# FishYuLi/BalancedGroupSoftmax

Measured on AMD Instinct MI355X. Metric: img/s fwd+bwd R50-FPN+BAGS 1333x800, 512 RoI (BASELINE metric: img/s/GPU fwd+bwd R50-FPN+BAGS 1333x800, 512 RoI; GroupSoftmax us/RoI), higher is better.
Workload: dtype f32 (conv/linear products on the bf16 MFMA from exact 3-way bf16 splits, fp32 accumulate: fp32-faithful)

## Files before the change

balancedgroupsoftmax_amd/backbone.py:

```python
import contextlib

import torch
import torch.nn as nn

from . import functional as BF
from .ops import OFFSET_PITCH, DeformConv
from .registry import BACKBONES, NECKS


def _trainable(*modules):
    return torch.is_grad_enabled() and any(
        p.requires_grad for m in modules if m is not None for p in m.parameters())


def _fold_conv_bn(conv, bn, pad_cin_to=None):
    w = conv.weight
    cbias = getattr(conv, 'bias', None)
    if w.is_cuda:
        ctx = contextlib.nullcontext() if _trainable(conv, bn) else torch.no_grad()
        with ctx:
            if bn is not None:
                return BF.fold_conv_bn(w, cbias, bn.weight, bn.bias, bn.running_mean,
                                       bn.running_var, bn.eps, cin_padded=pad_cin_to)
            return BF.fold_conv_bn(w, cbias, cin_padded=pad_cin_to)
    ctx = contextlib.nullcontext() if _trainable(conv, bn) else torch.no_grad()
    with ctx:
        w = conv.weight.float()
        cout = w.shape[0]
        if bn is not None:
            scale = bn.weight.float() / torch.sqrt(bn.running_var.float() + bn.eps)
            shift = bn.bias.float() - bn.running_mean.float() * scale
            w = w * scale.view(-1, 1, 1, 1)
            b = shift if cbias is None else shift + cbias.float() * scale
        else:
            b = cbias.float() if cbias is not None else w.new_zeros(cout)
        w = w.permute(0, 2, 3, 1)
        if pad_cin_to is not None and w.shape[3] < pad_cin_to:
            w = torch.nn.functional.pad(w, (0, pad_cin_to - w.shape[3]))
        return w.contiguous(), b.contiguous()


def _tensor_slots(mods):
    slots, dicts, moddicts = [], [], []
    stack = list(mods)[::-1]
    while stack:
        m = stack.pop()
        for d in (m._parameters, m._buffers):
            dicts.append(d)
            for k in d:
                slots.append((d, k))
        dicts.append(m._modules)
        moddicts.append(m._modules)
        stack.extend(m._modules.values())
    return slots, dicts, moddicts


class _FoldCache(object):

    def __init__(self):
        self.key = None
        self.data = None
        self.mods = None
        self.slots = None
        self.count = -1
        self.fence = None

    def _list(self, mods):
        self.mods = tuple(id(m) for m in mods)
        self.slots, self.dicts, self.moddicts = _tensor_slots(mods)
        self.count = sum(len(d) for d in self.dicts)
        self.subs = self._sub_ids()
        self.key = None

    def _sub_ids(self):
        return [id(v) for d in self.moddicts for v in d.values()]

    def get(self, module, build):
        mods = module if isinstance(module, tuple) else (module,)
        if self.slots is None or self.mods != tuple(id(m) for m in mods) or \
                self.count != sum(len(d) for d in self.dicts) or self.subs != self._sub_ids():
            self._list(mods)
        try:
            tensors = [d[k] for d, k in self.slots]
        except KeyError:
            self._list(mods)
            tensors = [d[k] for d, k in self.slots]
        grad = torch.is_grad_enabled()
        key = []
        for t in tensors:
            if t is None:
                continue
            if grad and t.requires_grad:
                return build()
            key.append((id(t), t._version, t.data_ptr()))
        if key != self.key:
            self.data = build()
            self.key = key
            self.fence = BF.CacheFence() if any(t is not None and t.is_cuda for t in tensors) else None
        elif self.fence is not None:
            self.fence.wait()
            if self.fence.event is None:
                self.fence = None
        return self.data


def cached_fold(conv, bn=None, pad_cin_to=None):
    cache = conv.__dict__.get('_bgs_fold_cache')
    if cache is None:
        cache = conv.__dict__['_bgs_fold_cache'] = _FoldCache()
    mods = (conv, bn) if bn is not None else (conv,)
    return cache.get(mods, lambda: _fold_conv_bn(conv, bn, pad_cin_to=pad_cin_to))


class Bottleneck(nn.Module):
    expansion = 4

    def __init__(self, inplanes, planes, stride=1, downsample=False, groups=1, base_width=4, dcn=None):
        super().__init__()
        width = planes if groups == 1 else (planes * base_width // 64) * groups
        self.groups, self.width = groups, width
        self.conv1 = nn.Conv2d(inplanes, width, 1, stride=1, bias=False)
        self.bn1 = nn.BatchNorm2d(width)
        self.with_dcn = dcn is not None and not dcn.get('fallback_on_stride', False)
        if dcn is not None and dcn.get('modulated', False):
            raise NotImplementedError('modulated')
        if self.with_dcn:
            self.dcn_groups = dcn.get('groups', 1)
            self.conv2_offset = nn.Conv2d(width, dcn.get('deformable_groups', 1) * 18, 3, stride=stride,
                                          padding=1)
            self.conv2 = DeformConv(width, width, kernel_size=3, stride=stride, padding=1, dilation=1,
                                    groups=self.dcn_groups,
                                    deformable_groups=dcn.get('deformable_groups', 1), bias=False)
        else:
            self.conv2 = nn.Conv2d(width, width, 3, stride=stride, padding=1, groups=groups, bias=False)
        self.bn2 = nn.BatchNorm2d(width)
        self.conv3 = nn.Conv2d(width, planes * 4, 1, bias=False)
        self.bn3 = nn.BatchNorm2d(planes * 4)
        self.stride = stride
        self.downsample = None
        if downsample:
            self.downsample = nn.Sequential(
                nn.Conv2d(inplanes, planes * 4, 1, stride=stride, bias=False),
                nn.BatchNorm2d(planes * 4))
        self._cache = _FoldCache()

    def folded(self):
        return self._cache.get(self, self._build_fold)

    def _build_fold(self):
        f = dict(c1=_fold_conv_bn(self.conv1, self.bn1), c2=_fold_conv_bn(self.conv2, self.bn2),
                 c3=_fold_conv_bn(self.conv3, self.bn3))
        if self.downsample is not None:
            f['ds'] = _fold_conv_bn(self.downsample[0], self.downsample[1])
        if self.with_dcn:
            ow, ob = _fold_conv_bn(self.conv2_offset, None)
            padc = OFFSET_PITCH - ow.shape[0]
            f['off'] = (torch.nn.functional.pad(ow, (0, 0, 0, 0, 0, 0, 0, padc)).contiguous(),
                        torch.nn.functional.pad(ob, (0, padc)).contiguous())
        return f

    def run_bf16_storage(self, x, f):
        if self.with_dcn:
            raise NotImplementedError('Bottleneck.run_bf16_storage: a dcn block has no bf16-storage kernel '
                                      '(the deformable conv is fp32 only)')
        identity, fk = x, None
        if 'ds' in f:
            if x.is_cuda and BF.shortcut_fork_enabled():
                with BF.forked(x.device) as fk:
                    identity = BF.conv2d_nhwc(x, f['ds'][0], f['ds'][1], stride=self.stride)
            else:
                identity = BF.conv2d_nhwc(x, f['ds'][0], f['ds'][1], stride=self.stride)
        out = BF.conv2d_nhwc(x, f['c1'][0], f['c1'][1], relu=True)
        if self.groups > 1:
            out = BF.grouped_conv3x3_nhwc(out, f['c2'][0], f['c2'][1], self.groups, stride=self.stride,
                                          relu=True)
        else:
            out = BF.conv2d_nhwc(out, f['c2'][0], f['c2'][1], stride=self.stride, pad=1, relu=True)
        if fk is not None:
            fk.join()
        return BF.conv2d_nhwc(out, f['c3'][0], f['c3'][1], relu=True, residual=identity)

    def run(self, x, f, next_c1=None, h=None):
        if h is not None and (x.dtype == torch.bfloat16 or self.groups > 1 or self.with_dcn or
                              (torch.is_grad_enabled() and x.requires_grad)):
            raise RuntimeError('Bottleneck.run: a precomputed conv1 output is for the frozen fp32 block only')
        if x.dtype == torch.bfloat16:
            return self.run_bf16_storage(x, f)
        tagged = bool(getattr(x, '_bgs_consumers_mask', False))
        fuse = BF.fork_fusion_enabled() and torch.is_grad_enabled() and x.requires_grad
        if tagged and not fuse:
            raise RuntimeError("Bottleneck.run: x is a relu='consumers' block output but fork fusion is off")
        out_relu = 'consumers' if BF.fork_fusion_enabled() else True
        xin = x
        identity = x
        fk = None
        sc_tail = ('ds' in f and not fuse and self.groups == 1 and not self.with_dcn and x.is_cuda and
                   not (torch.is_grad_enabled() and any(t.requires_grad for k in ('c1', 'c2', 'c3', 'ds') for t in f[k]
                                                        if t is not None)) and
                   BF.fused_c3_shortcut_eligible(x, tuple(x.shape[:3]) + (f['c1'][0].shape[0],), f['c2'][0], f['c3'][0],
                                                 self.stride, f['ds'][0], f['ds'][1], self.stride))
        if sc_tail:
            identity = None
        elif 'ds' in f and not fuse and x.is_cuda and BF.shortcut_fork_enabled() and \
                not (torch.is_grad_enabled() and any(t.requires_grad for t in f['ds'] if t is not None)):
            with BF.forked(x.device) as fk:
                identity = BF.conv2d_nhwc(x, f['ds'][0], f['ds'][1], stride=self.stride)
        elif 'ds' in f:
            if fuse:
                identity, xin = BF.conv2d_autograd(x, f['ds'][0], f['ds'][1], stride=self.stride,
                                                   mask_input=tagged, passthrough=True)
            else:
                identity = BF.conv2d_autograd(x, f['ds'][0], f['ds'][1], stride=self.stride)
        first_pt = fuse and 'ds' not in f
        first_mask = tagged and 'ds' not in f
        if self.groups > 1 or self.with_dcn:
            out = BF.conv2d_autograd(xin, f['c1'][0], f['c1'][1], relu=True, mask_input=first_mask,
                                     passthrough=first_pt)
            if first_pt:
                out, identity = out
            if self.with_dcn:
                off = BF.conv2d_autograd(out, f['off'][0], f['off'][1], stride=self.stride, pad=1)
                out = BF.deform_conv3x3_nhwc(out, off, f['c2'][0], f['c2'][1], self.dcn_groups,
                                             stride=self.stride, relu=True)
            else:
                out = BF.grouped_conv3x3_nhwc(out, f['c2'][0], f['c2'][1], self.groups,
                                              stride=self.stride, relu=True)
            if fk is not None:
                fk.join()
            return BF.conv2d_autograd(out, f['c3'][0], f['c3'][1], relu=out_relu, residual=identity)
        if h is not None:
            out = h
        else:
            out = BF.conv2d_autograd(xin, f['c1'][0], f['c1'][1], relu='consumers', mask_input=first_mask,
                                     passthrough=first_pt)
            if first_pt:
                out, identity = out
        if sc_tail:
            if BF.fused_c3_eligible(out, f['c2'][0], f['c3'][0], self.stride, None):
                nc = next_c1 if next_c1 is not None and next_c1[0].shape[0] == 64 and BF.fused_c3_next_eligible(
                    out, f['c2'][0], f['c3'][0], self.stride, None, next_c1[0], next_c1[1]) else (None, None)
                return BF.conv3x3_c3_sc_fused_nhwc(out, f['c2'][0], f['c2'][1], f['c3'][0], f['c3'][1], x, f['ds'][0],
                                                   f['ds'][1], nc[0], nc[1], relu3=True)
            identity = BF.conv2d_nhwc(x, f['ds'][0], f['ds'][1], stride=self.stride)
        if not fuse and BF.fused_c3_eligible(out, f['c2'][0], f['c3'][0], self.stride, identity):
            if fk is not None:
                fk.join()
            if next_c1 is not None and BF.fused_c3_next_eligible(out, f['c2'][0], f['c3'][0], self.stride, identity,
                                                                 next_c1[0], next_c1[1]):
                return BF.conv3x3_c3_next_fused_nhwc(out, f['c2'][0], f['c2'][1], f['c3'][0], f['c3'][1], next_c1[0],
                                                     next_c1[1], residual=identity, relu3=True)
            return BF.conv3x3_c3_fused_nhwc(out, f['c2'][0], f['c2'][1], f['c3'][0], f['c3'][1], residual=identity,
                                            relu3=True)
        out = BF.conv2d_autograd(out, f['c2'][0], f['c2'][1], stride=self.stride, pad=1,
                                 relu='consumers', mask_input=True)
        if fk is not None:
            fk.join()
        return BF.conv2d_autograd(out, f['c3'][0], f['c3'][1], relu=out_relu, residual=identity,
                                  mask_input=True)


@BACKBONES.register_module
class ResNet(nn.Module):
    arch_settings = {50: (3, 4, 6, 3), 101: (3, 4, 23, 3), 152: (3, 8, 36, 3)}

    def __init__(self, depth, num_stages=4, strides=(1, 2, 2, 2), dilations=(1, 1, 1, 1),
                 out_indices=(0, 1, 2, 3), style='pytorch', frozen_stages=-1, conv_cfg=None,
                 norm_cfg=dict(type='BN', requires_grad=True), norm_eval=True, dcn=None,
                 stage_with_dcn=(False, False, False, False), gcb=None,
                 stage_with_gcb=(False, False, False, False), gen_attention=None,
                 stage_with_gen_attention=((), (), (), ()), with_cp=False,
                 zero_init_residual=True, groups=1, base_width=4):
        super().__init__()
        if depth not in self.arch_settings:
            raise KeyError('invalid depth {} for resnet (bottleneck depths only)'.format(depth))
        if dcn:
            raise NotImplementedError('dcn (deformable convolution, gs_htc_dconv_* config) has no '
                                      'kernel in this build')
        if style != 'pytorch' or tuple(dilations) != (1, 1, 1, 1) or gcb or gen_attention:
            raise NotImplementedError('only the plain pytorch-style trunk of the BAGS configs')
        if norm_cfg.get('type', 'BN') != 'BN' or not norm_eval:
            raise NotImplementedError('BatchNorm in eval mode only (norm_eval=True is what every '
                                      'BAGS config uses); it is folded into the convs')
        self.depth, self.num_stages = depth, num_stages
        self.out_indices, self.frozen_stages, self.norm_eval = out_indices, frozen_stages, norm_eval
        self.conv1 = nn.Conv2d(3, 64, 7, stride=2, padding=3, bias=False)
        self.bn1 = nn.BatchNorm2d(64)
        blocks = self.arch_settings[depth][:num_stages]
        inplanes = 64
        self.res_layers = []
        for i, nb in enumerate(blocks):
            planes = 64 * 2 ** i
            layers = []
            for j in range(nb):
                stride = strides[i] if j == 0 else 1
                layers.append(Bottleneck(inplanes, planes, stride,
                                         downsample=(j == 0 and (stride != 1 or
                                                                 inplanes != planes * 4)),
                                         groups=groups, base_width=base_width))
                inplanes = planes * 4
            name = 'layer{}'.format(i + 1)
            self.add_module(name, nn.Sequential(*layers))
            self.res_layers.append(name)
        self.feat_dim = inplanes
        self._cache = _FoldCache()
        self._stem_split = _FoldCache()
        self._freeze_stages()

    def _freeze_stages(self):
        if self.frozen_stages >= 0:
            for m in (self.conv1, self.bn1):
                for p in m.parameters():
                    p.requires_grad = False
        for i in range(1, self.frozen_stages + 1):
            for p in getattr(self, 'layer{}'.format(i)).parameters():
                p.requires_grad = False

    def init_weights(self, pretrained=None):
        if isinstance(pretrained, str):
            if '://' in pretrained:
                import warnings
                warnings.warn('pretrained=%r is a model-zoo URL and there is no network here: the '
                              'backbone keeps its RANDOM initialisation (frozen stages included). '
                              'Pass a local checkpoint path, or load a state_dict explicitly '
                              '(checkpoint.load_checkpoint / load_from).' % (pretrained,),
                              RuntimeWarning, stacklevel=2)
            else:
                from .checkpoint import load_checkpoint
                load_checkpoint(self, pretrained, strict=False)
                return
        elif pretrained is not None:
            raise TypeError('pretrained must be a str or None')
        for m in self.modules():
            if isinstance(m, nn.Conv2d):
                nn.init.kaiming_normal_(m.weight, mode='fan_out', nonlinearity='relu')
            elif isinstance(m, nn.BatchNorm2d):
                nn.init.constant_(m.weight, 1)
                nn.init.constant_(m.bias, 0)
        for m in self.modules():
            if isinstance(m, Bottleneck):
                nn.init.constant_(m.bn3.weight, 0)
                if hasattr(m, 'conv2_offset'):
                    nn.init.constant_(m.conv2_offset.weight, 0)
                    nn.init.constant_(m.conv2_offset.bias, 0)

    def _build_stem(self):
        return _fold_conv_bn(self.conv1, self.bn1, pad_cin_to=4)

    @staticmethod
    def to_nhwc4(img):
        if img.is_cuda and not (torch.is_grad_enabled() and img.requires_grad):
            return BF.nchw_to_nhwc4(img)
        x = img.float().permute(0, 2, 3, 1)
        return torch.nn.functional.pad(x, (0, 4 - x.shape[3])).contiguous()

    def forward(self, img):
        return self.forward_partial(img, -1, len(self.res_layers) - 1)[1]

    def forward_partial(self, x, first, last, outs=()):
        outs = list(outs)
        if first < 0:
            x = self._forward_stem(x)
            first = 0
        chain = [(i, blk) for i in range(first, last + 1) for blk in getattr(self, self.res_layers[i])]
        h, f = None, None
        for k, (i, blk) in enumerate(chain):
            nxt = chain[k + 1][1] if k + 1 < len(chain) else None
            fn = None
            if nxt is not None and blk.width == 64 and blk.stride == 1 and blk.groups == 1 and not blk.with_dcn \
                    and nxt.groups == 1 and not nxt.with_dcn and not _trainable(nxt):
                fn = nxt.folded()
            r = blk.run(x, f if f is not None else blk.folded(), next_c1=None if fn is None else fn['c1'], h=h)
            x, h = r if isinstance(r, tuple) else (r, None)
            f = fn
            if k + 1 < len(chain) and chain[k + 1][0] == i:
                continue
            if i in self.out_indices:
                outs.append(BF.relu_gate(x))
        return x, tuple(outs)

    def _forward_stem(self, img):
        stem = self._cache.get((self.conv1, self.bn1), self._build_stem)
        frozen_stem = not (torch.is_grad_enabled() and (img.requires_grad or stem[0].requires_grad or
                                                        stem[1].requires_grad))
        if img.is_cuda and frozen_stem and img.shape[1] == 3 and tuple(stem[0].shape[:3]) == (64, 7, 7) \
                and BF.stem_fused_enabled():
            ws = self._stem_split.get((self.conv1, self.bn1),
                                      lambda: BF.stem_fused_split_weights(stem[0].detach()))
            x = BF.stem_fused(img, ws, stem[1].detach())
        else:
            x = self.to_nhwc4(img)
            x = BF.conv2d_autograd(x, stem[0], stem[1], stride=2, pad=3, relu=True)
            storage = (BF.bf16_storage_active() and not x.requires_grad and
                       not _trainable(*[getattr(self, n) for n in self.res_layers]))
            x = BF.maxpool3x3s2_nhwc(x, out_dtype=torch.bfloat16 if storage else torch.float32)
        return x

    def train(self, mode=True):
        super().train(mode)
        self._freeze_stages()
        if mode and self.norm_eval:
            for m in self.modules():
                if isinstance(m, nn.BatchNorm2d):
                    m.eval()
        return self


@BACKBONES.register_module
class ResNeXt(ResNet):

    def __init__(self, groups=1, base_width=4, **kwargs):
        super().__init__(groups=groups, base_width=base_width, **kwargs)
        self.groups, self.base_width = groups, base_width


class ConvModule(nn.Module):

    def __init__(self, cin, cout, k, padding=0):
        super().__init__()
        self.conv = nn.Conv2d(cin, cout, k, padding=padding)
        self.padding = padding


@NECKS.register_module
class FPN(nn.Module):

    def __init__(self, in_channels, out_channels, num_outs, start_level=0, end_level=-1,
                 add_extra_convs=False, extra_convs_on_inputs=True,
                 relu_before_extra_convs=False, no_norm_on_lateral=False, conv_cfg=None,
                 norm_cfg=None, activation=None):
        super().__init__()
        assert isinstance(in_channels, list)
        if add_extra_convs or norm_cfg is not None or activation is not None or start_level != 0 \
                or end_level != -1:
            raise NotImplementedError('FPN variant outside the BAGS configs')
        self.in_channels, self.out_channels, self.num_outs = in_channels, out_channels, num_outs
        self.num_ins = len(in_channels)
        self.lateral_convs = nn.ModuleList(ConvModule(c, out_channels, 1) for c in in_channels)
        self.fpn_convs = nn.ModuleList(ConvModule(out_channels, out_channels, 3, padding=1)
                                       for _ in in_channels)
        self._cache = _FoldCache()

    def init_weights(self):
        for m in self.modules():
            if isinstance(m, nn.Conv2d):
                nn.init.xavier_uniform_(m.weight)
                nn.init.constant_(m.bias, 0)

    def _build_fold(self):
        return dict(lat=[_fold_conv_bn(m.conv, None) for m in self.lateral_convs],
                    out=[_fold_conv_bn(m.conv, None) for m in self.fpn_convs])

    def forward(self, inputs):
        assert len(inputs) == self.num_ins
        f = self._cache.get(self, self._build_fold)
        n = self.num_ins
        if inputs[0].dtype != torch.float32 and torch.is_grad_enabled() and _trainable(self):
            inputs = [t.float() for t in inputs]
        lat = [None] * n
        gate = [bool(getattr(t, '_bgs_consumers_mask', False)) for t in inputs]
        lat[n - 1] = BF.conv2d_autograd(inputs[n - 1], *f['lat'][n - 1], out_dtype=torch.float32,
                                        mask_input=gate[n - 1])
        if n > 1 and lat[n - 1].is_cuda and BF.level_fork_enabled():
            outs, fk = [None] * n, None
            for i in range(n - 1, 0, -1):
                with BF.forked(lat[i].device) as fk:
                    outs[i] = BF.conv2d_autograd(lat[i], *f['out'][i], pad=1)
                    if i == n - 1:
                        extra = []
                        for _ in range(self.num_outs - n):
                            extra.append((extra[-1] if extra else outs[i])[:, ::2, ::2, :].contiguous())
                lat[i - 1] = BF.conv2d_autograd(inputs[i - 1], *f['lat'][i - 1], residual=lat[i],
                                                residual_mode=2, out_dtype=torch.float32, mask_input=gate[i - 1])
            outs[0] = BF.conv2d_autograd(lat[0], *f['out'][0], pad=1)
            fk.join()
            return tuple(outs + extra)
        for i in range(n - 2, -1, -1):
            lat[i] = BF.conv2d_autograd(inputs[i], *f['lat'][i], residual=lat[i + 1],
                                        residual_mode=2, out_dtype=torch.float32, mask_input=gate[i])
        outs = [BF.conv2d_autograd(lat[i], *f['out'][i], pad=1) for i in range(n)]
        for _ in range(self.num_outs - n):
            outs.append(outs[-1][:, ::2, ::2, :].contiguous())
        return tuple(outs)
```

balancedgroupsoftmax_amd/capi.py:

```python
import ctypes
import os

_PKG = os.path.dirname(os.path.abspath(__file__))

c_i64p = ctypes.c_void_p
c_f32p = ctypes.c_void_p
c_ptr = ctypes.c_void_p

BGS_OK = 0
BGS_MAX_BINS = 16


class BgsLibraryError(RuntimeError):
    pass


class BgsCallError(RuntimeError):
    def __init__(self, fn, code, text):
        super().__init__('%s failed with code %d: %s' % (fn, code, text))
        self.code = code


SIGNATURES = {
    'bgs_version': (ctypes.c_int, []),
    'bgs_error_string': (ctypes.c_char_p, [ctypes.c_int]),
    'bgs_selftest_wave_reduce': (ctypes.c_int, [c_f32p, c_f32p, c_ptr]),
    'bgs_selftest_mfma_peak': (ctypes.c_int, [ctypes.c_int, ctypes.c_int, c_f32p, c_ptr]),
    'bgs_selftest_mfma_peak_bf16': (ctypes.c_int, [ctypes.c_int, ctypes.c_int, ctypes.c_int, c_f32p, c_ptr]),
    'bgs_gs_prepare': (ctypes.c_int, [c_i64p, c_i64p, c_f32p, ctypes.c_int, c_f32p, ctypes.c_int,
                                      ctypes.c_int, ctypes.c_int, ctypes.c_double,
                                      ctypes.c_uint64, c_ptr, c_i64p, c_f32p, c_f32p, c_ptr]),
    'bgs_gs_loss_workspace_bytes': (ctypes.c_size_t, [ctypes.c_int, ctypes.c_int]),
    'bgs_gs_loss_fwd_bwd': (ctypes.c_int, [c_f32p, c_ptr, c_i64p, c_f32p, c_f32p,
                                           ctypes.c_int, ctypes.c_int, ctypes.c_int,
                                           c_f32p, c_f32p, c_ptr, c_ptr]),
    'bgs_gs_head_loss_fused': (ctypes.c_int, [c_f32p, c_i64p, c_i64p, c_f32p, c_ptr, ctypes.c_int,
                                              ctypes.c_int, ctypes.c_int, ctypes.c_int,
                                              ctypes.c_double, ctypes.c_uint64, c_ptr, c_f32p,
                                              c_f32p, c_f32p, c_ptr, c_f32p, c_ptr, c_ptr]),
    'bgs_gs_head_step': (ctypes.c_int, [c_f32p, c_i64p, c_i64p, c_ptr, c_f32p, c_ptr, c_ptr, ctypes.c_int,
                                        ctypes.c_int, ctypes.c_int, ctypes.c_int, ctypes.c_double,
                                        ctypes.c_uint64, c_ptr, c_f32p, c_f32p, c_f32p, ctypes.c_int,
                                        ctypes.c_float, ctypes.c_float, c_f32p, c_f32p, c_f32p, c_f32p,
                                        c_f32p, c_ptr, c_f32p, c_ptr, c_ptr]),
    'bgs_gs_head_debug_timestamps': (None, [c_ptr]),
    'bgs_gs_head_tuning': (None, [ctypes.c_int]),
    'bgs_gs_head_variant': (None, [ctypes.c_int]),
    'bgs_gs_head_variant_used': (ctypes.c_int, [ctypes.c_int]),
    'bgs_sgd_clip_workspace_bytes': (ctypes.c_size_t, [c_ptr, ctypes.c_int]),
    'bgs_sgd_clip_step': (ctypes.c_int, [c_ptr, c_ptr, c_ptr, c_ptr, ctypes.c_int] + [ctypes.c_float] * 5
                          + [c_ptr, ctypes.c_size_t, c_ptr, c_ptr]),
    'bgs_gs_class_bin_mask': (ctypes.c_int, [c_i64p, ctypes.c_int, ctypes.c_int, c_ptr, c_ptr]),
    'bgs_gs_head_step_scale_grad': (ctypes.c_int, [c_f32p, c_f32p, c_ptr, c_f32p, c_f32p, ctypes.c_int,
                                                   ctypes.c_int, ctypes.c_int, ctypes.c_int, c_ptr]),
    'bgs_gs_loss_reduce': (ctypes.c_int, [c_ptr, ctypes.c_int, ctypes.c_int, c_f32p, c_ptr]),
    'bgs_gs_scale_grad': (ctypes.c_int, [c_f32p, c_i64p, c_f32p, ctypes.c_int, ctypes.c_int,
                                         ctypes.c_int, c_ptr]),
    'bgs_gs_merge_score': (ctypes.c_int, [c_f32p, c_i64p, c_ptr, ctypes.c_int, ctypes.c_int,
                                          ctypes.c_int, ctypes.c_int, c_f32p, c_ptr]),
    'bgs_bbox_loss_workspace_bytes': (ctypes.c_size_t, [ctypes.c_int]),
    'bgs_bbox_smooth_l1_fwd_bwd': (ctypes.c_int, [c_f32p, c_i64p, c_f32p, c_f32p, ctypes.c_int,
                                                  ctypes.c_int, ctypes.c_float, ctypes.c_float,
                                                  ctypes.c_float, c_f32p, c_f32p, c_ptr, c_ptr]),
    'bgs_fc_reg_gather': (ctypes.c_int, [c_f32p, c_f32p, c_f32p, c_i64p, ctypes.c_int, ctypes.c_int,
                                         ctypes.c_int, c_f32p, c_ptr]),
    'bgs_conv2d_nhwc_f32': (ctypes.c_int, [c_f32p, c_f32p, c_f32p, c_f32p, c_f32p] + [ctypes.c_int] * 11
                            + [c_ptr]),
    'bgs_conv2d_workspace_bytes': (ctypes.c_size_t, [ctypes.c_longlong, ctypes.c_int]),
    'bgs_conv2d_nhwc_f32_ws': (ctypes.c_int, [c_f32p, c_f32p, c_f32p, c_f32p, c_f32p]
                               + [ctypes.c_int] * 11 + [c_ptr, ctypes.c_size_t, c_ptr]),
    'bgs_conv2d_dgrad_nhwc_f32_ws': (ctypes.c_int, [c_f32p, c_f32p, c_f32p, c_f32p, c_f32p]
                                     + [ctypes.c_int] * 10 + [c_ptr, ctypes.c_size_t, c_ptr]),
    'bgs_conv2d_dgrad_nhwc_f32': (ctypes.c_int, [c_f32p, c_f32p, c_f32p, c_f32p, c_f32p]
                                  + [ctypes.c_int] * 10 + [c_ptr]),
    'bgs_conv2d_wgrad_workspace_bytes': (ctypes.c_size_t, [ctypes.c_int] * 9),
    'bgs_conv2d_wgrad_nhwc_f32': (ctypes.c_int, [c_f32p, c_f32p, c_f32p, c_f32p]
                                  + [ctypes.c_int] * 10 + [c_ptr, c_ptr]),
    'bgs_fold_conv_bn_fwd': (ctypes.c_int, [c_f32p] * 6 + [ctypes.c_float] + [ctypes.c_int] * 5
                             + [c_f32p, c_f32p, c_ptr]),
    'bgs_fold_conv_bn_bwd': (ctypes.c_int, [c_f32p] * 7 + [ctypes.c_float] + [ctypes.c_int] * 5
                             + [c_f32p] * 4 + [c_ptr]),
    'bgs_conv2d_wgrad_bfx_workspace_bytes': (ctypes.c_size_t, [ctypes.c_int] * 9),
    'bgs_conv2d_wgrad_nhwc_f32_bfx': (ctypes.c_int, [c_f32p, c_f32p, c_f32p, c_f32p]
                                      + [ctypes.c_int] * 11 + [c_ptr, c_ptr]),
    'bgs_conv2d_wgrad_bfx_enable': (None, [ctypes.c_int]),
    'bgs_conv3x3_halo_nhwc_f32': (ctypes.c_int, [c_f32p, c_f32p, c_f32p, c_f32p] + [ctypes.c_int] * 6
                                  + [c_ptr]),
    'bgs_conv_bfx_weight_bytes': (ctypes.c_size_t, [ctypes.c_int, ctypes.c_int]),
    'bgs_conv_bfx_split_weights': (ctypes.c_int, [c_f32p, c_ptr, ctypes.c_int, ctypes.c_int, c_ptr]),
    'bgs_conv_dgrad_parity_enable': (None, [ctypes.c_int]),
    'bgs_conv_bfx_split_weights_dgrad': (ctypes.c_int, [c_f32p, c_ptr] + [ctypes.c_int] * 4 + [c_ptr]),
    'bgs_conv_bfx_workspace_bytes': (ctypes.c_size_t, [ctypes.c_longlong, ctypes.c_int, ctypes.c_int]),
    'bgs_conv2d_nhwc_f32_bfx_ws': (ctypes.c_int, [c_f32p, c_ptr, c_f32p, c_f32p, c_f32p]
                                   + [ctypes.c_int] * 12 + [c_ptr, ctypes.c_size_t, c_ptr]),
    'bgs_conv2d_dgrad_nhwc_f32_bfx_ws': (ctypes.c_int, [c_f32p, c_ptr, c_f32p, c_f32p, c_f32p]
                                         + [ctypes.c_int] * 11 + [c_ptr, ctypes.c_size_t, c_ptr]),
    'bgs_conv3x3_halo_bfx_workspace_bytes': (ctypes.c_size_t, [ctypes.c_int] * 5),
    'bgs_conv3x3_c3_fused_nhwc_f32_bfx': (ctypes.c_int, [c_f32p, c_ptr, c_f32p, c_ptr, c_f32p, c_f32p, c_f32p]
                                          + [ctypes.c_int] * 6 + [c_ptr]),
    'bgs_conv3x3_c3_fused_eligible': (ctypes.c_int, [ctypes.c_int] * 5),
    'bgs_conv3x3_c3_next_fused_nhwc_f32_bfx': (ctypes.c_int,
                                               [c_f32p, c_ptr, c_f32p, c_ptr, c_f32p, c_f32p, c_f32p, c_ptr, c_f32p,
                                                c_f32p] + [ctypes.c_int] * 7 + [c_ptr]),
    'bgs_conv3x3_c3_next_eligible': (ctypes.c_int, [ctypes.c_int] * 6),
    'bgs_conv3x3_c3_sc_fused_nhwc_f32_bfx': (ctypes.c_int,
                                             [c_f32p, c_ptr, c_f32p, c_ptr, c_f32p, c_f32p, c_ptr, c_f32p, c_f32p, c_ptr,
                                              c_f32p, c_f32p] + [ctypes.c_int] * 8 + [c_ptr]),
    'bgs_conv3x3_c3_sc_eligible': (ctypes.c_int, [ctypes.c_int] * 7),
    'bgs_conv3x3_halo_nhwc_f32_bfx': (ctypes.c_int, [c_f32p, c_ptr, c_f32p, c_f32p]
                                      + [ctypes.c_int] * 7 + [c_ptr, ctypes.c_size_t, c_ptr]),
    'bgs_conv3x3_halo_nhwc_f32_bfx_ex': (ctypes.c_int, [c_f32p, c_ptr, c_f32p, c_f32p, c_f32p]
                                         + [ctypes.c_int] * 7 + [c_ptr, ctypes.c_size_t, c_ptr]),
    'bgs_conv3x3_planes_head_nhwc_f32_bfx': (ctypes.c_int, [c_f32p, c_ptr, c_f32p, c_ptr, c_f32p, c_f32p]
                                             + [ctypes.c_int] * 7 + [c_ptr]),
    'bgs_conv3x3_planes_head_eligible': (ctypes.c_int, [ctypes.c_int] * 6),
    'bgs_gs_loss_tuning': (None, [ctypes.c_int]),
    'bgs_gs_loss_wavepriv_min_rows': (None, [ctypes.c_int]),
    'bgs_gs_merge_tuning': (None, [ctypes.c_int, ctypes.c_int]),
    'bgs_conv_bfx_wide_tuning': (None, [ctypes.c_int] * 3),
    'bgs_conv_bfx_wide_last_launch': (ctypes.c_int, []),
    'bgs_conv1x1_planes_enable': (None, [ctypes.c_int]),
    'bgs_conv1x1_planes_last_launch': (ctypes.c_int, []),
    'bgs_conv3x3_planes_enable': (None, [ctypes.c_int]),
    'bgs_conv3x3_planes_last_launch': (ctypes.c_int, []),
    'bgs_conv1x1_bres_enable': (None, [ctypes.c_int]),
    'bgs_conv1x1_bres_last_launch': (ctypes.c_int, []),
    'bgs_launch_census': (ctypes.c_int, [ctypes.c_int, ctypes.c_int]),
    'bgs_conv_bfx_tuning': (None, [ctypes.c_int] * 2),
    'bgs_conv_bfx_last_launch': (ctypes.c_int, [c_ptr, c_ptr]),
    'bgs_conv_tuning': (None, [ctypes.c_int] * 4),
    'bgs_conv_last_launch': (ctypes.c_int, [c_ptr, c_ptr, c_ptr, c_ptr]),
    'bgs_conv3x3_halo_bfx_tuning': (None, [ctypes.c_int] * 2),
    'bgs_conv3x3_halo_bfx_last_launch': (ctypes.c_int, [c_ptr, c_ptr]),
    'bgs_conv3x3_halo_bfx_last_wide': (ctypes.c_int, [c_ptr, c_ptr]),
    'bgs_conv3x3_halo_bfx_wide': (ctypes.c_int, [ctypes.c_int]),
    'bgs_grouped_conv3x3_nhwc_f32': (ctypes.c_int, [c_f32p, c_f32p, c_f32p, c_f32p] + [ctypes.c_int] * 7
                                     + [c_ptr]),
    'bgs_grouped_conv3x3_nhwc_bf16ops': (ctypes.c_int, [c_f32p, c_f32p, c_f32p, c_f32p] + [ctypes.c_int] * 7
                                         + [c_ptr]),
    'bgs_grouped_conv3x3_dgrad_nhwc_f32': (ctypes.c_int, [c_f32p, c_f32p, c_f32p] + [ctypes.c_int] * 6
                                           + [c_ptr]),
    'bgs_grouped_conv3x3_wgrad_workspace_bytes': (ctypes.c_size_t, [ctypes.c_int] * 6),
    'bgs_grouped_conv3x3_wgrad_nhwc_f32': (ctypes.c_int, [c_f32p, c_f32p, c_f32p, c_f32p]
                                           + [ctypes.c_int] * 7 + [c_ptr, c_ptr]),
    'bgs_deform_conv3x3_nhwc_f32': (ctypes.c_int, [c_f32p] * 5 + [ctypes.c_int] * 9 + [c_ptr]),
    'bgs_deform_conv3x3_dgrad_nhwc_f32': (ctypes.c_int, [c_f32p] * 6 + [ctypes.c_int] * 8 + [c_ptr]),
    'bgs_deform_conv3x3_wgrad_workspace_bytes': (ctypes.c_size_t, [ctypes.c_int] * 6),
    'bgs_deform_conv3x3_wgrad_nhwc_f32': (ctypes.c_int, [c_f32p] * 5 + [ctypes.c_int] * 9 + [c_ptr, c_ptr]),
    'bgs_sigmoid_focal_workspace_bytes': (ctypes.c_size_t, []),
    'bgs_sigmoid_focal_fwd': (ctypes.c_int, [c_f32p, ctypes.c_longlong, c_i64p, ctypes.c_int, ctypes.c_int,
                                             ctypes.c_float, ctypes.c_float, ctypes.c_int, c_f32p, c_ptr]),
    'bgs_sigmoid_focal_bwd': (ctypes.c_int, [c_f32p, ctypes.c_longlong, c_i64p, c_f32p, ctypes.c_int, ctypes.c_int,
                                             ctypes.c_float, ctypes.c_float, ctypes.c_int, c_f32p, c_ptr]),
    'bgs_sigmoid_focal_fwd_bwd': (ctypes.c_int, [c_f32p, ctypes.c_longlong, c_i64p, c_f32p, c_f32p, ctypes.c_int,
                                                 ctypes.c_int, ctypes.c_float, ctypes.c_float, ctypes.c_int, c_f32p,
                                                 ctypes.c_float, c_f32p, c_f32p, c_ptr, c_ptr]),
    'bgs_maxpool3x3s2_bwd_nhwc_f32': (ctypes.c_int, [c_f32p, c_f32p, c_f32p] + [ctypes.c_int] * 4 + [c_ptr]),
    'bgs_maxpool3x3s2_nhwc_f32': (ctypes.c_int, [c_f32p, c_f32p] + [ctypes.c_int] * 4 + [c_ptr]),
    'bgs_nchw_to_nhwc4_f32': (ctypes.c_int, [c_f32p, c_f32p] + [ctypes.c_int] * 4 + [c_ptr]),
    'bgs_conv2d_nhwc_bf16s': (ctypes.c_int, [c_ptr, c_ptr, c_f32p, c_ptr, ctypes.c_int, ctypes.c_int, c_ptr]
                              + [ctypes.c_int] * 11 + [c_ptr]),
    'bgs_grouped_conv3x3_nhwc_bf16s': (ctypes.c_int, [c_ptr, c_f32p, c_f32p, c_ptr] + [ctypes.c_int] * 7
                                       + [c_ptr]),
    'bgs_maxpool3x3s2_nhwc_f32_to_bf16': (ctypes.c_int, [c_f32p, c_ptr] + [ctypes.c_int] * 4 + [c_ptr]),
    'bgs_conv_bf16s_tuning': (None, [ctypes.c_int]),
    'bgs_roi_align_nhwc_fwd': (ctypes.c_int, [c_ptr, c_ptr, c_ptr, c_ptr, ctypes.c_int,
                                              ctypes.c_int, ctypes.c_float, c_f32p, ctypes.c_int,
                                              ctypes.c_int, ctypes.c_int, ctypes.c_int,
                                              ctypes.c_int, c_f32p, c_ptr, c_ptr]),
    'bgs_roi_align_nhwc_bwd': (ctypes.c_int, [c_ptr, c_ptr, c_ptr, c_ptr, ctypes.c_int,
                                              ctypes.c_int, ctypes.c_float, c_f32p, ctypes.c_int,
                                              ctypes.c_int, ctypes.c_int, ctypes.c_int,
                                              ctypes.c_int, c_f32p, c_ptr]),
    'bgs_roi_align_nhwc_fwd_f16': (ctypes.c_int, [c_ptr, c_ptr, c_ptr, c_ptr, ctypes.c_int,
                                                  ctypes.c_int, ctypes.c_float, c_f32p, ctypes.c_int,
                                                  ctypes.c_int, ctypes.c_int, ctypes.c_int,
                                                  ctypes.c_int, c_ptr, c_ptr, c_ptr]),
    'bgs_roi_align_nhwc_bwd_f16': (ctypes.c_int, [c_ptr, c_ptr, c_ptr, c_ptr, ctypes.c_int,
                                                  ctypes.c_int, ctypes.c_float, c_f32p, ctypes.c_int,
                                                  ctypes.c_int, ctypes.c_int, ctypes.c_int,
                                                  ctypes.c_int, c_ptr, c_ptr]),
    'bgs_roi_align_nhwc_fwd_ex': (ctypes.c_int, [c_ptr, c_ptr, c_ptr, c_ptr, ctypes.c_int,
                                                 ctypes.c_int, ctypes.c_float, c_f32p, ctypes.c_int,
                                                 ctypes.c_int, ctypes.c_int, ctypes.c_int,
                                                 ctypes.c_int, ctypes.c_int, ctypes.c_int, c_f32p,
                                                 c_ptr, c_ptr]),
    'bgs_roi_align_nhwc_bwd_ex': (ctypes.c_int, [c_ptr, c_ptr, c_ptr, c_ptr, ctypes.c_int,
                                                 ctypes.c_int, ctypes.c_float, c_f32p, ctypes.c_int,
                                                 ctypes.c_int, ctypes.c_int, ctypes.c_int,
                                                 ctypes.c_int, ctypes.c_int, c_f32p, c_ptr]),
    'bgs_resize_bilinear_nhwc_f32': (ctypes.c_int, [c_f32p, c_f32p] + [ctypes.c_int] * 7 + [c_ptr]),
    'bgs_resize_bilinear_nhwc_bwd_f32': (ctypes.c_int, [c_f32p, c_f32p] + [ctypes.c_int] * 7
                                         + [c_ptr]),
    'bgs_mask_target': (ctypes.c_int, [c_ptr, c_ptr, ctypes.c_int, ctypes.c_int, ctypes.c_int, c_f32p,
                                       ctypes.c_int, c_ptr, c_ptr, ctypes.c_int, ctypes.c_int, c_f32p,
                                       c_ptr]),
    'bgs_stem_fused_weight_bytes': (ctypes.c_size_t, []),
    'bgs_stem_fused_split_weights': (ctypes.c_int, [c_f32p, ctypes.c_int, c_ptr, c_ptr]),
    'bgs_stem_conv7x7s2_relu_maxpool_nchw_f32': (ctypes.c_int, [c_f32p, c_ptr, c_f32p, c_f32p, ctypes.c_int,
                                                                ctypes.c_int, ctypes.c_int, c_ptr]),
    'bgs_mask_paste_u8': (ctypes.c_int, [c_f32p, c_f32p, ctypes.c_int, ctypes.c_int, ctypes.c_int, ctypes.c_float,
                                         ctypes.c_float, ctypes.c_int, ctypes.c_int, c_ptr, c_ptr]),
    'bgs_mask_rle_workspace_bytes': (ctypes.c_size_t, [ctypes.c_int, ctypes.c_int]),
    'bgs_mask_rle_count': (ctypes.c_int, [c_f32p, c_f32p, ctypes.c_int, ctypes.c_int, ctypes.c_int, c_ptr, c_f32p,
                                          ctypes.c_float, ctypes.c_int, ctypes.c_int, c_ptr, ctypes.c_size_t, c_ptr,
                                          c_ptr]),
    'bgs_mask_rle_write': (ctypes.c_int, [c_f32p, c_f32p, ctypes.c_int, ctypes.c_int, ctypes.c_int, c_ptr, c_f32p,
                                          ctypes.c_float, ctypes.c_int, ctypes.c_int, c_ptr, ctypes.c_size_t, c_ptr,
                                          ctypes.c_longlong, c_ptr, c_ptr, c_ptr]),
    'bgs_rle_to_string': (ctypes.c_int, [c_ptr, c_ptr, ctypes.c_int, c_ptr, ctypes.c_longlong, c_ptr]),
    'bgs_rle_from_string': (ctypes.c_int, [c_ptr, c_ptr, ctypes.c_int, c_ptr, ctypes.c_longlong, c_ptr]),
    'bgs_lvis_box_iou': (ctypes.c_int, [c_ptr] * 5 + [ctypes.c_int] + [ctypes.c_longlong] * 3 + [c_ptr, c_ptr]),
    'bgs_lvis_rle_iou': (ctypes.c_int, [c_ptr] * 7 + [ctypes.c_int] + [ctypes.c_longlong] * 3 + [c_ptr, c_ptr]),
    'bgs_lvis_match_workspace_bytes': (ctypes.c_size_t, [ctypes.c_longlong, ctypes.c_int, ctypes.c_int]),
    'bgs_lvis_match': (ctypes.c_int, [c_ptr] * 4 + [ctypes.c_int] + [ctypes.c_longlong] * 2 + [c_ptr] * 4
                       + [c_ptr, ctypes.c_int, c_ptr, ctypes.c_int, c_ptr, ctypes.c_size_t] + [c_ptr] * 4 + [c_ptr]),
    'bgs_lvis_accumulate': (ctypes.c_int, [c_ptr] * 5 + [ctypes.c_int] + [ctypes.c_longlong] * 2
                            + [ctypes.c_int, ctypes.c_int, c_ptr, ctypes.c_int, c_ptr, c_ptr, c_ptr]),
    'bgs_recall_match_lds_bytes': (ctypes.c_size_t, [ctypes.c_int, ctypes.c_int]),
    'bgs_recall_match': (ctypes.c_int, [c_ptr] * 5 + [c_ptr, ctypes.c_int, c_ptr, ctypes.c_int]
                         + [ctypes.c_int, ctypes.c_int, ctypes.c_longlong, ctypes.c_longlong, ctypes.c_int,
                            ctypes.c_int, c_ptr, c_ptr, c_ptr]),
    'bgs_poly_rle_edge_points': (ctypes.c_int, [c_ptr, c_ptr, c_ptr, ctypes.c_longlong, ctypes.c_int, c_ptr, c_ptr]),
    'bgs_poly_rle_crossings': (ctypes.c_int, [c_ptr] * 4 + [ctypes.c_longlong, ctypes.c_int, ctypes.c_int, c_ptr, c_ptr,
                                              ctypes.c_longlong, c_ptr, c_ptr, c_ptr]),
    'bgs_poly_rle_events_from_transitions': (ctypes.c_int, [c_ptr] * 4 + [ctypes.c_int, ctypes.c_longlong, c_ptr,
                                                            c_ptr]),
    'bgs_poly_rle_events_from_runs': (ctypes.c_int, [c_ptr] * 3 + [ctypes.c_int, ctypes.c_longlong, c_ptr, c_ptr]),
    'bgs_poly_rle_resolve': (ctypes.c_int, [c_ptr] * 3 + [ctypes.c_int, ctypes.c_int] + [c_ptr] * 4
                             + [ctypes.c_int, ctypes.c_longlong] + [c_ptr] * 4),
    'bgs_poly_rle_write': (ctypes.c_int, [c_ptr] * 4 + [ctypes.c_int] + [c_ptr] * 4
                           + [ctypes.c_longlong, c_ptr, ctypes.c_longlong, c_ptr, c_ptr]),
    'bgs_mask_gt_logits': (ctypes.c_int, [c_f32p, c_f32p, c_f32p, c_ptr, ctypes.c_int, ctypes.c_int,
                                          ctypes.c_int, ctypes.c_int, c_f32p, c_ptr]),
    'bgs_mask_bce_partials': (ctypes.c_int, [ctypes.c_int]),
    'bgs_mask_bce': (ctypes.c_int, [c_f32p, c_f32p, c_f32p, c_ptr, c_f32p, c_ptr, c_f32p,
                                    ctypes.c_int, ctypes.c_int, ctypes.c_int, ctypes.c_int, c_f32p,
                                    c_f32p, c_f32p, c_f32p, c_ptr]),
    'bgs_topk_workspace_bytes': (ctypes.c_size_t, [ctypes.c_int, ctypes.c_int]),
    'bgs_topk_sorted_f32': (ctypes.c_int, [c_ptr, c_ptr, c_ptr, c_ptr, c_ptr, ctypes.c_int,
                                           ctypes.c_int, c_f32p, c_ptr, c_ptr, c_ptr]),
    'bgs_nms_workspace_bytes': (ctypes.c_size_t, [ctypes.c_int, ctypes.c_int]),
    'bgs_nms_batched': (ctypes.c_int, [c_f32p, c_ptr, ctypes.c_int, ctypes.c_int, ctypes.c_float,
                                       ctypes.c_int, ctypes.c_int, c_ptr, c_ptr, c_ptr, c_ptr]),
    'bgs_nms_merge_select': (ctypes.c_int, [c_f32p, c_ptr, c_ptr] + [ctypes.c_int] * 4 + [c_f32p, c_ptr, c_ptr]),
    'bgs_nms_gather': (ctypes.c_int, [c_f32p, c_ptr, c_ptr, ctypes.c_int, ctypes.c_int, c_f32p, c_f32p, c_ptr]),
    'bgs_soft_nms_batched': (ctypes.c_int, [c_f32p, c_ptr, ctypes.c_int, ctypes.c_int, ctypes.c_float, ctypes.c_int,
                                            ctypes.c_float, ctypes.c_float, c_ptr, c_f32p, c_ptr, c_ptr]),
    'bgs_det_candidates': (ctypes.c_int, [c_f32p, c_f32p, c_ptr, c_f32p] + [ctypes.c_int] * 4
                           + [ctypes.c_float, ctypes.c_int, c_f32p, c_ptr, c_ptr, c_ptr]),
    'bgs_det_select': (ctypes.c_int, [c_f32p, c_ptr, c_ptr, c_f32p, c_ptr] + [ctypes.c_int] * 4
                       + [c_f32p, c_ptr, c_ptr, c_ptr, c_ptr]),
    'bgs_gather_boxes': (ctypes.c_int, [c_f32p, c_ptr, c_f32p, ctypes.c_int, ctypes.c_int, ctypes.c_int, c_f32p,
                                        c_ptr, c_ptr]),
    'bgs_aug_map_boxes': (ctypes.c_int, [c_ptr, c_ptr] + [ctypes.c_int] * 4 + [c_ptr, c_ptr, c_ptr, ctypes.c_int,
                                                                               ctypes.c_int, c_f32p, c_f32p, c_ptr,
                                                                               c_ptr]),
    'bgs_aug_merge_bboxes': (ctypes.c_int, [c_ptr, c_ptr] + [ctypes.c_int] * 4 + [c_ptr, c_ptr, c_ptr, c_ptr, c_f32p,
                                                                                  c_f32p, c_ptr]),
    'bgs_aug_merge_masks': (ctypes.c_int, [c_ptr, c_ptr, ctypes.c_int, ctypes.c_int, ctypes.c_int, c_f32p, c_ptr]),
    'bgs_img_prep_u8': (ctypes.c_int, [c_ptr, c_ptr, ctypes.c_int, ctypes.c_int, c_f32p, ctypes.c_int, c_f32p,
                                       ctypes.c_int, ctypes.c_int, c_ptr]),
    'bgs_gt_mask_prep_u8': (ctypes.c_int, [c_ptr, c_ptr, ctypes.c_int, c_ptr, c_ptr, ctypes.c_longlong, c_ptr,
                                           ctypes.c_int, ctypes.c_int, c_ptr]),
    'bgs_gt_seg_prep_u8': (ctypes.c_int, [c_ptr, c_ptr, ctypes.c_int, c_ptr, ctypes.c_int, ctypes.c_int, c_ptr]),
    'bgs_iou_assign_workspace_bytes': (ctypes.c_size_t, [ctypes.c_int] * 3),
    'bgs_iou_assign': (ctypes.c_int, [c_f32p, ctypes.c_longlong, ctypes.c_int, c_ptr, c_f32p, c_ptr,
                                      ctypes.c_int, ctypes.c_int, ctypes.c_float, ctypes.c_float,
# ... 120 lines not shown
```

balancedgroupsoftmax_amd/csrc/bottleneck_tail_planes.hip:

```cpp
#include <stdlib.h>

#include <initializer_list>

#include "conv_args.h"
#include "bfx_split.h"

using namespace bgs_conv;

namespace {

struct TailArgs {
  const float* x;
  const __bf16* ws2;
  const float* bias2;
  const __bf16* ws3;
  const float* bias3;
  const float* res;
  float* y;
  int N, H, W, relu3;
  int tiles_y, tiles_x, tiles, chunk;
};

struct TailNextArgs {
  TailArgs t;
  const __bf16* ws1n;
  const float* bias1n;
  float* h;
};
template <class A> struct TailScArgs {
  A a;
  const float* x0;
  const __bf16* wssc;
  const float* bias_sc;
};
template <int NEXT, bool SC = false> struct TailArgsOf { typedef TailNextArgs type; };
template <> struct TailArgsOf<0, false> { typedef TailArgs type; };
template <int NEXT> struct TailArgsOf<NEXT, true> { typedef TailScArgs<typename TailArgsOf<NEXT>::type> type; };
__device__ __forceinline__ const TailArgs& tail_base(const TailArgs& a) { return a; }
__device__ __forceinline__ const TailArgs& tail_base(const TailNextArgs& a) { return a.t; }
template <class A> __device__ __forceinline__ const TailArgs& tail_base(const TailScArgs<A>& a) { return tail_base(a.a); }
template <class A> __device__ __forceinline__ const A& tail_inner(const A& a) { return a; }
template <class A> __device__ __forceinline__ const A& tail_inner(const TailScArgs<A>& a) { return a.a; }

constexpr int kOob = 0x7f000000;

__device__ __forceinline__ void load_x0_half(const float* x0, const TailArgs& g, int n, int ty, int tx, int tid, int a,
                                             f32x4& q0, f32x4& q1) {
  const __amdgpu_buffer_rsrc_t x0_rsrc = __builtin_amdgcn_make_buffer_rsrc(
      const_cast<float*>(x0), 0, (int)((size_t)g.N * g.H * g.W * 64 * 4), 0x00020000);
  f32x4 q[2];
#pragma unroll
  for (int j = 0; j < 2; ++j) {
    const int m = a * 32 + (tid >> 4) + 16 * j;
    const int ho = ty * 8 + (m >> 3), wo = tx * 8 + (m & 7);
    const int off = ho < g.H && wo < g.W ? (((n * g.H + ho) * g.W + wo) * 64 + (tid & 15) * 4) * 4 : kOob;
    q[j] = __builtin_bit_cast(f32x4, __builtin_amdgcn_raw_buffer_load_b128(x0_rsrc, off, 0, 0));
  }
  q0 = q[0];
  q1 = q[1];
}

__device__ __forceinline__ void load_sc_filter(const __bf16* wssc, int lane_off, int t, bf16x8 (&dst)[3]) {
  const __amdgpu_buffer_rsrc_t bs_rsrc = __builtin_amdgcn_make_buffer_rsrc(const_cast<__bf16*>(wssc), 0, 3 * 4 * 256 * 32, 0x00020000);
#pragma unroll
  for (int s = 0; s < 3; ++s)
    dst[s] = __builtin_bit_cast(bf16x8, __builtin_amdgcn_raw_buffer_load_b128(bs_rsrc, lane_off, ((s * 4 + (t & 3)) * 256 + 32 * (t >> 2)) * 32, 0));
}

template <int NEXT, bool SC = false>
__global__ __launch_bounds__(kThreads, 3) void bottleneck_tail_planes_kernel(typename TailArgsOf<NEXT, SC>::type ga) {
  static_assert(NEXT == 0 || NEXT == 64 || NEXT == 128, "width of the next block's conv1");
  static_assert(!SC || NEXT != 128, "a block with a stride-1 projection shortcut (layer1.0) is never in front of a 128-wide conv1");
  const TailArgs& g = tail_base(ga);
  const auto& gn = tail_inner(ga);
  constexpr int NS = 3, CM = 64, CO3 = 256, KC2 = 36, KC3 = 4;
  constexpr int PW = 10, PS = 12, PSLOTS = PW * PS;
  constexpr int AQ = PW * PW * 16, AQT = (AQ + kThreads - 1) / kThreads;
  constexpr int KS = PSLOTS * 32, PL = 4 * KS;
  constexpr int KCN = CO3 / 16, KCH = KCN / 2, KSN = 64 * 32 + 32, PLN = KCH * KSN;
  constexpr int LD4 = CO3 + 8;
  constexpr int SC_OFF = 32 * LD4 * 4, KSC = 32 * 32 + 32, PLSC = KC3 * KSC;
  constexpr int LDS_BASE = NEXT ? NS * PLN : NS * PL;
  constexpr int LDS_BYTES = SC && SC_OFF + NS * PLSC > LDS_BASE ? SC_OFF + NS * PLSC : LDS_BASE;
  static_assert(64 * (NEXT + 8) * 4 <= LDS_BYTES, "the h transpose tile overlays the planes");
  static_assert(NS * PL <= LDS_BYTES && 3 * LDS_BYTES <= 160 * 1024, "three workgroups per CU");
  constexpr int LD2 = CM + 4, S2_BYTES = 64 * LD2 * 4;
  constexpr int Y_OFF = 18 * 1024;
  constexpr int P3_CH = 64 * 32, P3_PL = KC3 * P3_CH;
  static_assert(S2_BYTES <= Y_OFF && Y_OFF + NS * P3_PL <= LDS_BYTES && 32 * LD4 * 4 <= LDS_BYTES, "overlays");
  __shared__ __attribute__((aligned(1024))) unsigned char lds[LDS_BYTES];

  const int tid = threadIdx.x, lane = tid & 63;
  const int wave = bgs::uniform(tid >> 6);
  const int wm = wave >> 1, wn = wave & 1;
  const int frow = lane & 31, fk = lane >> 5;
  const int vtile = (int)((blockIdx.x & 7) * g.chunk + (blockIdx.x >> 3));
  if (vtile >= g.tiles) return;
  const int per_img = g.tiles_y * g.tiles_x;
  const int n = vtile / per_img, trem = vtile - n * per_img;
  const int ty = trem / g.tiles_x, tx = trem - ty * g.tiles_x;
  const int h0 = ty * 8 - 1, w0 = tx * 8 - 1;

  const __amdgpu_buffer_rsrc_t x_rsrc = __builtin_amdgcn_make_buffer_rsrc(
      const_cast<float*>(g.x), 0, (int)((size_t)g.N * g.H * g.W * CM * 4), 0x00020000);
  f32x4 ra[AQT];
  int a_dst[AQT];
#pragma unroll
  for (int i = 0; i < AQT; ++i) {
    const int q = tid + kThreads * i;
    const bool use = q < AQ;
    const int pix = use ? q >> 4 : 0, kq = q & 15;
    const int ppy = pix / PW, ppx = pix - ppy * PW;
    const int hi = h0 + ppy, wi = w0 + ppx;
    const bool in = use && hi >= 0 && hi < g.H && wi >= 0 && wi < g.W;
    const int off = in ? (((n * g.H + hi) * g.W + wi) * CM + kq * 4) * 4 : kOob;
    ra[i] = __builtin_bit_cast(f32x4, __builtin_amdgcn_raw_buffer_load_b128(x_rsrc, off, 0, 0));
    const int quad = kq & 3;
    a_dst[i] = use ? (kq >> 2) * KS + (ppy * PS + ppx) * 32 + (((quad >> 1) ^ (ppy & 1)) << 4) + (quad & 1) * 8 : -1;
  }

  f32x4 rx[SC ? 4 : 1];
  if constexpr (SC) load_x0_half(ga.x0, g, n, ty, tx, tid, 0, rx[0], rx[1]);

  const __amdgpu_buffer_rsrc_t b2_rsrc = __builtin_amdgcn_make_buffer_rsrc(
      const_cast<__bf16*>(g.ws2), 0, NS * KC2 * CM * 32, 0x00020000);
  const int b2_lane = ((wn * 32 + frow) * 16 + fk * 8) * 2;
  auto load_b2 = [&](int kc, bf16x8 (&dst)[NS]) {
#pragma unroll
    for (int s = 0; s < NS; ++s)
      dst[s] = __builtin_bit_cast(bf16x8, __builtin_amdgcn_raw_buffer_load_b128(b2_rsrc, b2_lane, (s * KC2 + kc) * CM * 32, 0));
  };
  bf16x8 fbA[NS], fbB[NS];
  load_b2(0, fbA);

#pragma unroll
  for (int i = 0; i < AQT; ++i) {
    if (a_dst[i] < 0) continue;
    u32x2 hh, mm, ll;
    split3(ra[i], hh, mm, ll);
    unsigned char* d = lds + a_dst[i];
    *reinterpret_cast<u32x2*>(d) = hh;
    *reinterpret_cast<u32x2*>(d + PL) = mm;
    *reinterpret_cast<u32x2*>(d + 2 * PL) = ll;
  }
  __syncthreads();

  int a_frag[2];
  {
    const int m = wm * 32 + frow;
    const int py = m >> 3, px = m & 7;
#pragma unroll
    for (int par = 0; par < 2; ++par) a_frag[par] = (py * PS + px) * 32 + ((fk ^ ((py + par) & 1)) << 4);
  }
  f32x16 acc2;
#pragma unroll
  for (int r = 0; r < 16; ++r) acc2[r] = 0.f;
#pragma unroll
  for (int t = 0; t < KC2; ++t) {
    const int c16 = t / 9, tap = t % 9, dy = tap / 3, dx = tap % 3;
    const int t1 = t + 1;
    const int kc_next = t1 < KC2 ? (t1 % 9) * 4 + t1 / 9 : 0;
    if (t & 1) load_b2(kc_next, fbA);
    else load_b2(kc_next, fbB);
    __builtin_amdgcn_sched_barrier(0);
    const bf16x8 (&fb)[NS] = (t & 1) ? fbB : fbA;
    bf16x8 fa[NS];
#pragma unroll
    for (int s = 0; s < NS; ++s)
      fa[s] = *reinterpret_cast<const bf16x8*>(lds + s * PL + c16 * KS + a_frag[dy & 1] + (dy * PS + dx) * 32);
#pragma unroll
    for (int tt = NS - 1; tt >= 0; --tt)
#pragma unroll
      for (int i = 0; i <= tt; ++i) acc2 = __builtin_amdgcn_mfma_f32_32x32x16_bf16(fa[i], fb[tt - i], acc2, 0, 0, 0);
    __builtin_amdgcn_sched_barrier(0);
  }

  const __amdgpu_buffer_rsrc_t b3_rsrc = __builtin_amdgcn_make_buffer_rsrc(
      const_cast<__bf16*>(g.ws3), 0, NS * KC3 * CO3 * 32, 0x00020000);
  const int b3_lane = ((wave * 64 + frow) * 16 + fk * 8) * 2;
  auto load_b3 = [&](int kc, bf16x8 (&dst)[NS][2]) {
#pragma unroll
    for (int s = 0; s < NS; ++s)
#pragma unroll
      for (int b = 0; b < 2; ++b)
        dst[s][b] = __builtin_bit_cast(bf16x8, __builtin_amdgcn_raw_buffer_load_b128(b3_rsrc, b3_lane, ((s * KC3 + kc) * CO3 + 32 * b) * 32, 0));
  };
  bf16x8 f3a[NS][2], f3b[NS][2];
  load_b3(0, f3a);
  bf16x8 fsa[NS], fsb[NS];

  __syncthreads();
  float* scratch = reinterpret_cast<float*>(lds);
#pragma unroll
  for (int r = 0; r < 16; ++r) {
    const int i = wm * 32 + (r & 3) + 8 * (r >> 2) + 4 * (lane >> 5);
    scratch[i * LD2 + wn * 32 + (lane & 31)] = acc2[r];
  }
  __syncthreads();
  {
    const int c4 = (tid & 15) * 4, r0 = tid >> 4;
    f32x4 bias2 = {0.f, 0.f, 0.f, 0.f};
    if (g.bias2) bias2 = *reinterpret_cast<const f32x4*>(g.bias2 + c4);
    const int kc2 = c4 >> 4, kq2 = (c4 & 15) >> 2;
#pragma unroll
    for (int ps = 0; ps < 4; ++ps) {
      const int i = r0 + ps * 16;
      f32x4 v = *reinterpret_cast<const f32x4*>(scratch + i * LD2 + c4);
      v += bias2;
#pragma unroll
      for (int t = 0; t < 4; ++t) v[t] = fmaxf(v[t], 0.f);
      u32x2 hh, mm, ll;
      split3(v, hh, mm, ll);
      unsigned char* d = lds + Y_OFF + kc2 * P3_CH + i * 32 + (((kq2 >> 1) ^ ((i >> 3) & 1)) << 4) + (kq2 & 1) * 8;
      *reinterpret_cast<u32x2*>(d) = hh;
      *reinterpret_cast<u32x2*>(d + P3_PL) = mm;
      *reinterpret_cast<u32x2*>(d + 2 * P3_PL) = ll;
    }
  }
  __syncthreads();

  int a3_frag[2];
#pragma unroll
  for (int a = 0; a < 2; ++a) {
    const int m = a * 32 + frow;
// ... 22 lines not shown
    const bf16x8 (&fb3)[NS][2] = (kc & 1) ? f3b : f3a;
    bf16x8 fa3[NS][2];
#pragma unroll
    for (int s = 0; s < NS; ++s)
#pragma unroll
      for (int a = 0; a < 2; ++a) fa3[s][a] = *reinterpret_cast<const bf16x8*>(lds + a3_frag[a] + kc * P3_CH + s * P3_PL);
#pragma unroll
    for (int tt = NS - 1; tt >= 0; --tt)
#pragma unroll
      for (int i = 0; i <= tt; ++i)
#pragma unroll
        for (int a = 0; a < 2; ++a)
#pragma unroll
          for (int b = 0; b < 2; ++b)
            acc3[a][b] = __builtin_amdgcn_mfma_f32_32x32x16_bf16(fa3[i][a], fb3[tt - i][b], acc3[a][b], 0, 0, 0);
    __builtin_amdgcn_sched_barrier(0);
  }
  __syncthreads();

  const int e4 = (tid & 63) * 4, er0 = tid >> 6;
  f32x4 bias3 = {0.f, 0.f, 0.f, 0.f};
  if (g.bias3) bias3 = *reinterpret_cast<const f32x4*>(g.bias3 + e4);
  const int out_bytes = (int)((size_t)g.N * g.H * g.W * CO3 * 4);
  const __amdgpu_buffer_rsrc_t res_rsrc = __builtin_amdgcn_make_buffer_rsrc(
      const_cast<float*>(g.res ? g.res : g.x), 0, g.res ? out_bytes : 0, 0x00020000);
  const __amdgpu_buffer_rsrc_t y_rsrc = __builtin_amdgcn_make_buffer_rsrc(g.y, 0, out_bytes, 0x00020000);
  f32x4 vn[NEXT ? 2 : 1][NEXT ? 8 : 1];
  if constexpr (SC) {
    const int kcw = (tid & 15) >> 2, kqw = tid & 3;
    auto write_planes = [&](int a) {
#pragma unroll
      for (int j = 0; j < 2; ++j) {
        const int i = (tid >> 4) + 16 * j;
        u32x2 hh, mm, ll;
        split3(rx[2 * a + j], hh, mm, ll);
        unsigned char* d = lds + SC_OFF + kcw * KSC + i * 32 + (((kqw >> 1) ^ ((i >> 3) & 1)) << 4) + (kqw & 1) * 8;
        *reinterpret_cast<u32x2*>(d) = hh;
        *reinterpret_cast<u32x2*>(d + PLSC) = mm;
        *reinterpret_cast<u32x2*>(d + 2 * PLSC) = ll;
      }
    };
    const int as_frag = SC_OFF + frow * 32 + ((fk ^ ((frow >> 3) & 1)) << 4);
    float b3v[2] = {0.f, 0.f}, bsv[2] = {0.f, 0.f};
#pragma unroll
    for (int b = 0; b < 2; ++b) {
      if (g.bias3) b3v[b] = g.bias3[wave * 64 + b * 32 + (lane & 31)];
      if (ga.bias_sc) bsv[b] = ga.bias_sc[wave * 64 + b * 32 + (lane & 31)];
    }
    write_planes(0);
#pragma unroll
    for (int a = 0; a < 2; ++a) {
      __syncthreads();
#pragma unroll
      for (int b = 0; b < 2; ++b) {
        f32x16 accs;
#pragma unroll
        for (int r = 0; r < 16; ++r) accs[r] = 0.f;
#pragma unroll
        for (int kc = 0; kc < KC3; ++kc) {
          const int t = b * KC3 + kc;
          if (t + 1 < 2 * KC3) {
            if (t & 1) load_sc_filter(ga.wssc, b3_lane, t + 1, fsa);
            else load_sc_filter(ga.wssc, b3_lane, t + 1, fsb);
          }
          __builtin_amdgcn_sched_barrier(0);
          const bf16x8 (&fbs)[NS] = (t & 1) ? fsb : fsa;
          bf16x8 fas[NS];
#pragma unroll
          for (int s = 0; s < NS; ++s) fas[s] = *reinterpret_cast<const bf16x8*>(lds + as_frag + kc * KSC + s * PLSC);
#pragma unroll
          for (int tt = NS - 1; tt >= 0; --tt)
#pragma unroll
            for (int i = 0; i <= tt; ++i) accs = __builtin_amdgcn_mfma_f32_32x32x16_bf16(fas[i], fbs[tt - i], accs, 0, 0, 0);
          __builtin_amdgcn_sched_barrier(0);
        }
#pragma unroll
        for (int r = 0; r < 16; ++r) {
          const int i = (r & 3) + 8 * (r >> 2) + 4 * (lane >> 5);
          const float rsc = accs[r] + bsv[b];
          scratch[i * LD4 + wave * 64 + b * 32 + (lane & 31)] = (acc3[a][b][r] + b3v[b]) + rsc;
        }
      }
      __syncthreads();
      if (a == 0) {
        load_sc_filter(ga.wssc, b3_lane, 0, fsa);
        write_planes(1);
      }
#pragma unroll
      for (int ps = 0; ps < 8; ++ps) {
        const int i = er0 + ps * 4;
        const int m = a * 32 + i;
        const int ho = ty * 8 + (m >> 3), wo = tx * 8 + (m & 7);
        f32x4 v = *reinterpret_cast<const f32x4*>(scratch + i * LD4 + e4);
        if (g.relu3) {
#pragma unroll
          for (int t = 0; t < 4; ++t) v[t] = fmaxf(v[t], 0.f);
        }
        if (ho < g.H && wo < g.W)
          __builtin_amdgcn_raw_buffer_store_b128(__builtin_bit_cast(u32x4, v), y_rsrc, (((n * g.H + ho) * g.W + wo) * CO3 + e4) * 4, 0, 0);
        if constexpr (NEXT > 0) vn[a][ps] = v;
      }
    }
    if constexpr (NEXT > 0) __syncthreads();
  } else {
#pragma unroll
  for (int a = 0; a < 2; ++a) {
    f32x4 rs[8];
#pragma unroll
    for (int ps = 0; ps < 8; ++ps) {
      const int m = a * 32 + er0 + ps * 4;
      const int ho = min(ty * 8 + (m >> 3), g.H - 1), wo = min(tx * 8 + (m & 7), g.W - 1);
      rs[ps] = __builtin_bit_cast(f32x4, __builtin_amdgcn_raw_buffer_load_b128(res_rsrc, (((n * g.H + ho) * g.W + wo) * CO3 + e4) * 4, 0, 0));
    }
#pragma unroll
    for (int b = 0; b < 2; ++b)
#pragma unroll
      for (int r = 0; r < 16; ++r) {
        const int i = (r & 3) + 8 * (r >> 2) + 4 * (lane >> 5);
        scratch[i * LD4 + wave * 64 + b * 32 + (lane & 31)] = acc3[a][b][r];
      }
    __syncthreads();
#pragma unroll
    for (int ps = 0; ps < 8; ++ps) {
      const int i = er0 + ps * 4;
      const int m = a * 32 + i;
      const int ho = ty * 8 + (m >> 3), wo = tx * 8 + (m & 7);
      f32x4 v = *reinterpret_cast<const f32x4*>(scratch + i * LD4 + e4);
      v += bias3;
      v += rs[ps];
      if (g.relu3) {
#pragma unroll
        for (int t = 0; t < 4; ++t) v[t] = fmaxf(v[t], 0.f);
      }
      if (ho < g.H && wo < g.W)
        __builtin_amdgcn_raw_buffer_store_b128(__builtin_bit_cast(u32x4, v), y_rsrc, (((n * g.H + ho) * g.W + wo) * CO3 + e4) * 4, 0, 0);
      if constexpr (NEXT > 0) vn[a][ps] = v;
    }
    __syncthreads();
  }
  }

  if constexpr (NEXT > 0) {
    constexpr int LDH = NEXT + 8, NA = NEXT == 128 ? 2 : 1;
    const int a0 = NEXT == 128 ? 0 : (wave >> 1);
    const int tn = NEXT == 128 ? wave : (wave & 1);
    const __amdgpu_buffer_rsrc_t bn_rsrc = __builtin_amdgcn_make_buffer_rsrc(
        const_cast<__bf16*>(gn.ws1n), 0, NS * KCN * NEXT * 32, 0x00020000);
    const int bn_lane = ((tn * 32 + frow) * 16 + fk * 8) * 2;
    auto load_bn = [&](int kc, bf16x8 (&dst)[NS]) {
#pragma unroll
      for (int s = 0; s < NS; ++s)
        dst[s] = __builtin_bit_cast(bf16x8, __builtin_amdgcn_raw_buffer_load_b128(bn_rsrc, bn_lane, (s * KCN + kc) * NEXT * 32, 0));
    };
    bf16x8 fn[3][NS];
    load_bn(0, fn[0]);
    load_bn(1, fn[1]);
    f32x4 vs[2][8];
#pragma unroll
    for (int ps = 0; ps < 8; ++ps) {
      const u32x4 lo = __builtin_bit_cast(u32x4, vn[0][ps]), hi = __builtin_bit_cast(u32x4, vn[1][ps]);
      u32x4 slo, shi;
#pragma unroll
      for (int t = 0; t < 4; ++t) {
        const unsigned a0 = lo[t], a1 = hi[t];
        const auto sw = __builtin_amdgcn_permlane32_swap(a0, a1, false, false);
        slo[t] = sw[0];
        shi[t] = sw[1];
      }
      vs[0][ps] = __builtin_bit_cast(f32x4, slo);
      vs[1][ps] = __builtin_bit_cast(f32x4, shi);
    }
    const int kcl = (lane & 31) >> 2, kqn = lane & 3;
    int an_frag[NA];
#pragma unroll
    for (int a = 0; a < NA; ++a) {
      const int m = (a0 + a) * 32 + frow;
      an_frag[a] = m * 32 + ((fk ^ ((m >> 3) & 1)) << 4);
    }
    f32x16 accn[NA];
#pragma unroll
    for (int a = 0; a < NA; ++a)
#pragma unroll
      for (int r = 0; r < 16; ++r) accn[a][r] = 0.f;
#pragma unroll
    for (int c = 0; c < 2; ++c) {
#pragma unroll
      for (int ps = 0; ps < 8; ++ps) {
        const int i = (lane >> 5) * 32 + er0 + ps * 4;
        u32x2 hh, mm, ll;
        split3(vs[c][ps], hh, mm, ll);
        unsigned char* d = lds + kcl * KSN + i * 32 + (((kqn >> 1) ^ ((i >> 3) & 1)) << 4) + (kqn & 1) * 8;
        *reinterpret_cast<u32x2*>(d) = hh;
        *reinterpret_cast<u32x2*>(d + PLN) = mm;
        *reinterpret_cast<u32x2*>(d + 2 * PLN) = ll;
      }
      __syncthreads();
#pragma unroll
      for (int k8 = 0; k8 < KCH; ++k8) {
        const int kc = c * KCH + k8;
        if (kc + 2 < KCN) load_bn(kc + 2, fn[(kc + 2) % 3]);
        __builtin_amdgcn_sched_barrier(0);
        const bf16x8 (&fbn)[NS] = fn[kc % 3];
        bf16x8 fan[NS][NA];
#pragma unroll
        for (int s = 0; s < NS; ++s)
#pragma unroll
          for (int a = 0; a < NA; ++a) fan[s][a] = *reinterpret_cast<const bf16x8*>(lds + s * PLN + k8 * KSN + an_frag[a]);
#pragma unroll
        for (int tt = NS - 1; tt >= 0; --tt)
#pragma unroll
          for (int i = 0; i <= tt; ++i)
#pragma unroll
            for (int a = 0; a < NA; ++a)
              accn[a] = __builtin_amdgcn_mfma_f32_32x32x16_bf16(fan[i][a], fbn[tt - i], accn[a], 0, 0, 0);
        __builtin_amdgcn_sched_barrier(0);
      }
      __syncthreads();
    }
#pragma unroll
    for (int a = 0; a < NA; ++a)
#pragma unroll
      for (int r = 0; r < 16; ++r) {
        const int i = (a0 + a) * 32 + (r & 3) + 8 * (r >> 2) + 4 * (lane >> 5);
        scratch[i * LDH + tn * 32 + (lane & 31)] = accn[a][r];
      }
    __syncthreads();
    constexpr int TPRN = NEXT / 4, RPPN = kThreads / TPRN, EPN = 64 / RPPN;
    const int n4 = (tid % TPRN) * 4, nr0 = tid / TPRN;
    f32x4 biasn = {0.f, 0.f, 0.f, 0.f};
    if (gn.bias1n) biasn = *reinterpret_cast<const f32x4*>(gn.bias1n + n4);
    const __amdgpu_buffer_rsrc_t h_rsrc =
        __builtin_amdgcn_make_buffer_rsrc(gn.h, 0, (int)((size_t)g.N * g.H * g.W * NEXT * 4), 0x00020000);
#pragma unroll
    for (int ps = 0; ps < EPN; ++ps) {
      const int m = nr0 + ps * RPPN;
      const int ho = ty * 8 + (m >> 3), wo = tx * 8 + (m & 7);
      f32x4 v = *reinterpret_cast<const f32x4*>(scratch + m * LDH + n4);
      v += biasn;
#pragma unroll
      for (int t = 0; t < 4; ++t) v[t] = fmaxf(v[t], 0.f);
      if (ho < g.H && wo < g.W)
        __builtin_amdgcn_raw_buffer_store_b128(__builtin_bit_cast(u32x4, v), h_rsrc, (((n * g.H + ho) * g.W + wo) * NEXT + n4) * 4, 0, 0);
    }
  }
}

}


static int tail_eligible(int N, int H, int W, int Cmid, int Cout3) {
  if (N <= 0 || H <= 0 || W <= 0 || Cmid != 64 || Cout3 != 256) return 0;
  const long long lim = kOob / (256 * 4);
  const long long nh = (long long)N * H;
  return nh < lim && nh * W < lim ? 1 : 0;
}

template <class... P> static bool aligned16(P... ptr) { return ((... | (uintptr_t)ptr) % 16) == 0; }

static TailArgs tail_args(const float* x, const void* w2split, const float* bias2, const void* w3split,
                          const float* bias3, const float* residual, float* y, int N, int H, int W, int relu3) {
  TailArgs g;
  g.x = x;
  g.ws2 = reinterpret_cast<const __bf16*>(w2split);
  g.bias2 = bias2;
  g.ws3 = reinterpret_cast<const __bf16*>(w3split);
  g.bias3 = bias3;
  g.res = residual;
  g.y = y;
  g.N = N; g.H = H; g.W = W; g.relu3 = relu3;
  g.tiles_y = (H + 7) / 8;
  g.tiles_x = (W + 7) / 8;
  g.tiles = N * g.tiles_y * g.tiles_x;
  g.chunk = (g.tiles + 7) / 8;
  return g;
}

static TailNextArgs tail_next_args(const TailArgs& g, const void* w1n_split, const float* bias1n, float* h) {
  TailNextArgs a;
  a.t = g;
  a.ws1n = reinterpret_cast<const __bf16*>(w1n_split);
  a.bias1n = bias1n;
  a.h = h;
  return a;
}

template <int NEXT, bool SC>
static int tail_launch(const typename TailArgsOf<NEXT, SC>::type& a, int chunk, bgs_stream_t stream,
                       std::initializer_list<int> own_slots = {}) {
  hipLaunchKernelGGL((bottleneck_tail_planes_kernel<NEXT, SC>), dim3((unsigned)(8 * chunk)), dim3(kThreads), 0,
                     (hipStream_t)stream, a);
  bgs_internal_census_bump(BGS_CENSUS_FUSED_C3);
  for (int slot : own_slots) bgs_internal_census_bump(slot);
  return hipGetLastError() == hipSuccess ? BGS_OK : BGS_ERR_LAUNCH;
}

extern "C" int bgs_conv3x3_c3_fused_eligible(int N, int H, int W, int Cmid, int Cout3) {
  return tail_eligible(N, H, W, Cmid, Cout3);
}

extern "C" int bgs_conv3x3_c3_fused_nhwc_f32_bfx(const float* x, const void* w2split, const float* bias2,
                                                 const void* w3split, const float* bias3, const float* residual,
                                                 float* y, int N, int H, int W, int Cmid, int Cout3, int relu3,
                                                 bgs_stream_t stream) {
  if (N <= 0 || H <= 0 || W <= 0 || !x || !w2split || !w3split || !y) return BGS_ERR_INVALID_ARG;
  if (!tail_eligible(N, H, W, Cmid, Cout3)) return BGS_ERR_UNSUPPORTED;
  if (!aligned16(x, w2split, w3split, y, residual, bias2, bias3)) return BGS_ERR_UNSUPPORTED;
  const TailArgs g = tail_args(x, w2split, bias2, w3split, bias3, residual, y, N, H, W, relu3);
  return tail_launch<0, false>(g, g.chunk, stream);
}

extern "C" int bgs_conv3x3_c3_next_eligible(int N, int H, int W, int Cmid, int Cout3, int Cnext) {
  return (Cnext == 64 || Cnext == 128) ? tail_eligible(N, H, W, Cmid, Cout3) : 0;
}

extern "C" int bgs_conv3x3_c3_next_fused_nhwc_f32_bfx(const float* x, const void* w2split, const float* bias2,
                                                      const void* w3split, const float* bias3, const float* residual,
                                                      float* y, const void* w1n_split, const float* bias1n, float* h,
                                                      int N, int H, int W, int Cmid, int Cout3, int relu3, int Cnext,
                                                      bgs_stream_t stream) {
  if (N <= 0 || H <= 0 || W <= 0 || !x || !w2split || !w3split || !y || !w1n_split || !h) return BGS_ERR_INVALID_ARG;
  if (!bgs_conv3x3_c3_next_eligible(N, H, W, Cmid, Cout3, Cnext)) return BGS_ERR_UNSUPPORTED;
  if (!aligned16(x, w2split, w3split, y, residual, bias2, bias3, w1n_split, bias1n, h)) return BGS_ERR_UNSUPPORTED;
  const TailArgs g = tail_args(x, w2split, bias2, w3split, bias3, residual, y, N, H, W, relu3);
  const TailNextArgs a = tail_next_args(g, w1n_split, bias1n, h);
  return Cnext == 64 ? tail_launch<64, false>(a, g.chunk, stream, {BGS_CENSUS_FUSED_C3_NEXT})
                     : tail_launch<128, false>(a, g.chunk, stream, {BGS_CENSUS_FUSED_C3_NEXT});
}

extern "C" int bgs_conv3x3_c3_sc_eligible(int N, int H, int W, int Cin0, int Cmid, int Cout3, int Cnext) {
  return (Cin0 == 64 && (Cnext == 0 || Cnext == 64)) ? tail_eligible(N, H, W, Cmid, Cout3) : 0;
}

extern "C" int bgs_conv3x3_c3_sc_fused_nhwc_f32_bfx(const float* x, const void* w2split, const float* bias2,
                                                    const void* w3split, const float* bias3, const float* x0,
                                                    const void* wsc_split, const float* bias_sc, float* y,
                                                    const void* w1n_split, const float* bias1n, float* h, int N, int H,
                                                    int W, int Cin0, int Cmid, int Cout3, int relu3, int Cnext,
                                                    bgs_stream_t stream) {
  if (N <= 0 || H <= 0 || W <= 0 || !x || !w2split || !w3split || !x0 || !wsc_split || !y) return BGS_ERR_INVALID_ARG;
  if (Cnext != 0 && (!w1n_split || !h)) return BGS_ERR_INVALID_ARG;
  if (!bgs_conv3x3_c3_sc_eligible(N, H, W, Cin0, Cmid, Cout3, Cnext)) return BGS_ERR_UNSUPPORTED;
  if (!aligned16(x, w2split, w3split, y, x0, wsc_split, bias2, bias3, bias_sc)) return BGS_ERR_UNSUPPORTED;
  if (Cnext != 0 && !aligned16(w1n_split, bias1n, h)) return BGS_ERR_UNSUPPORTED;
  const TailArgs g = tail_args(x, w2split, bias2, w3split, bias3, nullptr, y, N, H, W, relu3);
  const __bf16* wssc = reinterpret_cast<const __bf16*>(wsc_split);
  if (Cnext == 64) {
    const TailScArgs<TailNextArgs> a = {tail_next_args(g, w1n_split, bias1n, h), x0, wssc, bias_sc};
    return tail_launch<64, true>(a, g.chunk, stream, {BGS_CENSUS_FUSED_C3_SHORTCUT, BGS_CENSUS_FUSED_C3_NEXT});
  }
  const TailScArgs<TailArgs> a = {g, x0, wssc, bias_sc};
  return tail_launch<0, true>(a, g.chunk, stream, {BGS_CENSUS_FUSED_C3_SHORTCUT});
}
```

balancedgroupsoftmax_amd/csrc/conv3x3_planes.hip:

```cpp
#include <stdlib.h>

#include <type_traits>

#ifndef BGS_P3_A_AUX
#define BGS_P3_A_AUX 0
#endif
#ifndef BGS_P3_Y_AUX
#define BGS_P3_Y_AUX 0
#endif
#ifndef BGS_P3_PRIO
#define BGS_P3_PRIO 0
#endif
#ifndef BGS_P3_ABL
#define BGS_P3_ABL 0
#endif
#include "bfx_internal.h"
#include "bfx_split.h"

using namespace bgs_conv;

namespace {

struct Planes3Args {
  ConvArgs c;
  const __bf16* ws;
  int KC;
  int tiles_y, tiles_x;
};

constexpr int kOob = 0x7f000000;

struct Planes3HeadArgs {
  Planes3Args g;
  const __bf16* hs;
  const float* hbias;
  float* hy;
  int CH;
};

template <bool HEAD>
struct Planes3ArgsOf { typedef Planes3Args type; };
template <>
struct Planes3ArgsOf<true> { typedef Planes3HeadArgs type; };
__device__ __forceinline__ const Planes3Args& planes3_base(const Planes3Args& a) { return a; }
__device__ __forceinline__ const Planes3Args& planes3_base(const Planes3HeadArgs& a) { return a.g; }

template <int NB, bool HEAD = false>
__global__ __launch_bounds__(kThreads, 3) void conv3x3_planes_bfx_kernel(typename Planes3ArgsOf<HEAD>::type ga) {
  const Planes3Args& g = planes3_base(ga);
  const ConvArgs& p = g.c;
  constexpr int NS = 3, KCH = 2;
  constexpr int TW = 8, PW = 10, PS = 12, PSLOTS = PW * PS;
  constexpr int AQ = PW * PW * 8;
  constexpr int KS = PSLOTS * 32, PL = KCH * KS, BUF = NS * PL;
  constexpr int CO = 128 * NB, LD4 = CO + 8;
  constexpr int LDS_BYTES = 2 * BUF;
  static_assert(PL % 512 == 0 && 3 * LDS_BYTES <= 160 * 1024, "three workgroups per CU");
  static_assert(32 * LD4 * 4 <= LDS_BYTES, "epilogue tile overlays the operand buffers");
  __shared__ __attribute__((aligned(1024))) unsigned char lds[LDS_BYTES];

  const int tid = threadIdx.x, lane = tid & 63;
  const int wave = bgs::uniform(tid >> 6);
  const int frow = lane & 31, fk = lane >> 5;
  const int vtile = (int)((blockIdx.x & 7) * p.chunk + (blockIdx.x >> 3));
  if (vtile >= p.tiles_m * p.tiles_n) return;
  const int tm = vtile / p.tiles_n, tn = vtile - tm * p.tiles_n;
  const int per_img = g.tiles_y * g.tiles_x;
  const int n = tm / per_img, trem = tm - n * per_img;
  const int ty = trem / g.tiles_x, tx = trem - ty * g.tiles_x;
  const int h0 = ty * 8 - 1, w0 = tx * 8 - 1;
  const int n0 = tn * CO;
  const int cch16 = p.Cin >> 4, nchunks = p.Cin >> 5;

  const __amdgpu_buffer_rsrc_t x_rsrc = __builtin_amdgcn_make_buffer_rsrc(
      const_cast<float*>(p.x), 0, (int)((size_t)p.N * p.H * p.W * p.Cin * 4), 0x00020000);
  int a_off[4], a_dst[4];
#pragma unroll
  for (int i = 0; i < 4; ++i) {
    const int q = tid + kThreads * i;
    const bool use = q < AQ;
    const int pix = use ? q >> 3 : 0, kq = q & 7;
    const int ppy = pix / PW, ppx = pix - ppy * PW;
    const int hi = h0 + ppy, wi = w0 + ppx;
    const bool in = use && hi >= 0 && hi < p.H && wi >= 0 && wi < p.W;
    a_off[i] = in ? (((n * p.H + hi) * p.W + wi) * p.Cin + kq * 4) * 4 : kOob;
    const int quad = kq & 3;
    a_dst[i] = use ? (kq >> 2) * KS + (ppy * PS + ppx) * 32 + (((quad >> 1) ^ (ppy & 1)) << 4) + (quad & 1) * 8 : -1;
  }
  f32x4 ra[4];
  auto load_a = [&](int chunk) {
#pragma unroll
    for (int i = 0; i < 4; ++i)
      ra[i] = __builtin_bit_cast(f32x4, __builtin_amdgcn_raw_buffer_load_b128(x_rsrc, a_off[i], chunk * 128, BGS_P3_A_AUX));
  };
  auto store_a = [&](int buf) {
#pragma unroll
    for (int i = 0; i < 4; ++i) {
      if (a_dst[i] < 0) continue;
      u32x2 hh, mm, ll;
      split3(ra[i], hh, mm, ll);
      unsigned char* d = lds + buf * BUF + a_dst[i];
      *reinterpret_cast<u32x2*>(d) = hh;
      *reinterpret_cast<u32x2*>(d + PL) = mm;
      *reinterpret_cast<u32x2*>(d + 2 * PL) = ll;
    }
  };

  const __amdgpu_buffer_rsrc_t b_rsrc = __builtin_amdgcn_make_buffer_rsrc(
      const_cast<__bf16*>(g.ws), 0, (int)((size_t)NS * g.KC * p.Cout * 32), 0x00020000);
  const int b_lane = ((n0 + wave * 32 * NB + frow) * 16 + fk * 8) * 2;
  const int b_plane = g.KC * p.Cout * 32;
  auto load_b = [&](int kc, bf16x8 (&dst)[NS][NB]) {
#pragma unroll
    for (int s = 0; s < NS; ++s)
#pragma unroll
      for (int b = 0; b < NB; ++b)
        dst[s][b] = __builtin_bit_cast(bf16x8, __builtin_amdgcn_raw_buffer_load_b128(
                                                   b_rsrc, b_lane, s * b_plane + (kc * p.Cout + 32 * b) * 32, 0));
  };

  int a_frag[2][2];
#pragma unroll
  for (int a = 0; a < 2; ++a) {
    const int m = a * 32 + frow;
    const int py = m >> 3, px = m & 7;
#pragma unroll
    for (int par = 0; par < 2; ++par) a_frag[a][par] = (py * PS + px) * 32 + ((fk ^ ((py + par) & 1)) << 4);
  }
  f32x16 acc[2][NB];
#pragma unroll
  for (int a = 0; a < 2; ++a)
#pragma unroll
    for (int b = 0; b < NB; ++b)
#pragma unroll
      for (int r = 0; r < 16; ++r) acc[a][b][r] = 0.f;

  bf16x8 fb0[NS][NB], fb1[NS][NB];
  load_a(0);
  load_b(0, fb0);
  for (int chunk = 0; chunk < nchunks; ++chunk) {
    const int buf = chunk & 1;
    store_a(buf);
    __syncthreads();
#pragma unroll
    for (int t = 0; t < 2 * 9; ++t) {
      const int kcs = t / 9, tap = t % 9, dy = tap / 3, dx = tap % 3;
      const int t1 = t + 1;
      const int kc_next = t1 < 18 ? (t1 % 9) * cch16 + chunk * 2 + t1 / 9 : (chunk + 1) * 2;
#if BGS_P3_ABL & 1
      if (t < 2) {
#endif
      if (t & 1) load_b(kc_next, fb0);
      else load_b(kc_next, fb1);
#if BGS_P3_ABL & 1
      }
#endif
#if BGS_P3_ABL & 2
      if (t == 0 && chunk == 0) load_a(chunk + 1);
#else
      if (t == 0) load_a(chunk + 1);
#endif
      __builtin_amdgcn_sched_barrier(0);
      const bf16x8 (&fbu)[NS][NB] = (t & 1) ? fb1 : fb0;
      bf16x8 fa[NS][2];
#pragma unroll
      for (int s = 0; s < NS; ++s)
#pragma unroll
        for (int a = 0; a < 2; ++a)
          fa[s][a] = *reinterpret_cast<const bf16x8*>(lds + buf * BUF + s * PL + kcs * KS + a_frag[a][dy & 1] +
                                                      (dy * PS + dx) * 32);
#if BGS_P3_PRIO
      __builtin_amdgcn_s_setprio(1);
#endif
#pragma unroll
      for (int tt = NS - 1; tt >= 0; --tt)
#pragma unroll
        for (int i = 0; i <= tt; ++i)
#pragma unroll
          for (int a = 0; a < 2; ++a)
#pragma unroll
            for (int b = 0; b < NB; ++b)
              acc[a][b] = __builtin_amdgcn_mfma_f32_32x32x16_bf16(fa[i][a], fbu[tt - i][b], acc[a][b], 0, 0, 0);
#if BGS_P3_PRIO
      __builtin_amdgcn_s_setprio(0);
#endif
      __builtin_amdgcn_sched_barrier(0);
    }
  }
  __syncthreads();

  float* scratch = reinterpret_cast<float*>(lds);
  constexpr int TPR = CO / 4, RPP = kThreads / TPR, EP = 32 / RPP;
  const int e4 = (tid % TPR) * 4, er0 = tid / TPR;
  f32x4 bias = {0.f, 0.f, 0.f, 0.f};
  if (p.bias) bias = *reinterpret_cast<const f32x4*>(p.bias + n0 + e4);
  if constexpr (HEAD) {
    static_assert(NB == 2, "the head form owns all 256 channels of a pixel");
    const Planes3HeadArgs& hg = ga;
    const int CH = hg.CH;
    const int kch = p.Cout >> 4;
    float cb[NB];
#pragma unroll
    for (int b = 0; b < NB; ++b) cb[b] = p.bias ? p.bias[n0 + wave * 32 * NB + b * 32 + (lane & 31)] : 0.f;
    const __amdgpu_buffer_rsrc_t h_rsrc = __builtin_amdgcn_make_buffer_rsrc(
        const_cast<__bf16*>(hg.hs), 0, (int)((size_t)NS * kch * CH * 32), 0x00020000);
    const __amdgpu_buffer_rsrc_t hy_rsrc =
        __builtin_amdgcn_make_buffer_rsrc(hg.hy, 0, (int)((size_t)p.M * CH * 4), 0x00020000);
    const int h_lane = frow < CH ? frow * 32 + fk * 16 : kOob;
    const int h_plane = kch * CH * 32;
    const float hb = (hg.hbias && frow < CH) ? hg.hbias[frow] : 0.f;
    bf16x8 hf[4][NS];
#pragma unroll
    for (int u = 0; u < 4; ++u)
#pragma unroll
      for (int s = 0; s < NS; ++s)
        hf[u][s] = __builtin_bit_cast(bf16x8, __builtin_amdgcn_raw_buffer_load_b128(
                                                  h_rsrc, h_lane, s * h_plane + (wave * 4 + u) * CH * 32, 0));
    static_assert(32 * LD4 * 4 + 2 * 16 * 64 * 4 <= LDS_BYTES, "accumulator hand-off slots behind the scratch tile");
    float* hand = scratch + 32 * LD4;
    const float* srow = scratch + frow * LD4 + wave * 64 + fk * 8;
    auto stage = [&](auto half) {
      constexpr int a = decltype(half)::value;
      __builtin_amdgcn_s_setprio(3);
#pragma unroll
      for (int b = 0; b < NB; ++b)
#pragma unroll
        for (int r = 0; r < 16; ++r) {
          const int i = (r & 3) + 8 * (r >> 2) + 4 * (lane >> 5);
          float v = acc[a][b][r];
          v += cb[b];
          if (p.relu) v = fmaxf(v, 0.f);
          scratch[i * LD4 + wave * 32 * NB + b * 32 + (lane & 31)] = v;
        }
      f32x16 hacc;
      if (wave == 0) {
#pragma unroll
        for (int r = 0; r < 16; ++r) hacc[r] = 0.f;
      } else {
#pragma unroll
        for (int r = 0; r < 16; ++r) hacc[r] = hand[(a * 16 + r) * 64 + lane];
      }
      __builtin_amdgcn_fence(__ATOMIC_RELEASE, "wavefront");
      __builtin_amdgcn_wave_barrier();
      __builtin_amdgcn_fence(__ATOMIC_ACQUIRE, "wavefront");
#pragma unroll
      for (int u = 0; u < 4; ++u) {
        const f32x4 v0 = *reinterpret_cast<const f32x4*>(srow + u * 16);
        const f32x4 v1 = *reinterpret_cast<const f32x4*>(srow + u * 16 + 4);
        u32x2 h0, m0, l0, h1, m1, l1;
        split3(v0, h0, m0, l0);
        split3(v1, h1, m1, l1);
        bf16x8 fa[NS];
        fa[0] = __builtin_bit_cast(bf16x8, u32x4{h0[0], h0[1], h1[0], h1[1]});
        fa[1] = __builtin_bit_cast(bf16x8, u32x4{m0[0], m0[1], m1[0], m1[1]});
        fa[2] = __builtin_bit_cast(bf16x8, u32x4{l0[0], l0[1], l1[0], l1[1]});
#pragma unroll
        for (int tt = NS - 1; tt >= 0; --tt)
#pragma unroll
          for (int i = 0; i <= tt; ++i)
            hacc = __builtin_amdgcn_mfma_f32_32x32x16_bf16(fa[i], hf[u][tt - i], hacc, 0, 0, 0);
      }
      __builtin_amdgcn_s_setprio(0);
      if (wave < 3) {
#pragma unroll
        for (int r = 0; r < 16; ++r) hand[(a * 16 + r) * 64 + lane] = hacc[r];
      } else if (frow < CH) {
#pragma unroll
        for (int r = 0; r < 16; ++r) {
          const int i = (r & 3) + 8 * (r >> 2) + 4 * (lane >> 5);
          const int m = a * 32 + i;
          const int ho = ty * 8 + (m >> 3), wo = tx * TW + (m & 7);
          if (ho < p.H && wo < p.W)
            __builtin_amdgcn_raw_buffer_store_b32(__builtin_bit_cast(unsigned, hacc[r] + hb), hy_rsrc,
                                                  (((n * p.H + ho) * p.W + wo) * CH + frow) * 4, 0, 0);
        }
      }
    };
#pragma unroll
    for (int s = 0; s < 5; ++s) {
      if (s - wave == 0) stage(std::integral_constant<int, 0>{});
      else if (s - wave == 1) stage(std::integral_constant<int, 1>{});
      if (s < 4) __syncthreads();
    }
    return;
  }
  const __amdgpu_buffer_rsrc_t y_rsrc =
      __builtin_amdgcn_make_buffer_rsrc(p.y, 0, (int)((size_t)p.M * p.Cout * 4), 0x00020000);
  const __amdgpu_buffer_rsrc_t mk_rsrc = __builtin_amdgcn_make_buffer_rsrc(
      const_cast<float*>(p.mask ? p.mask : p.x), 0, p.mask ? (int)((size_t)p.M * p.Cout * 4) : 0, 0x00020000);
#pragma unroll
  for (int a = 0; a < 2; ++a) {
    f32x4 mk[EP];
    if (p.mask) {
#pragma unroll
      for (int ps = 0; ps < EP; ++ps) {
        const int m = a * 32 + er0 + ps * RPP;
        const int ho = min(ty * 8 + (m >> 3), p.H - 1), wo = min(tx * TW + (m & 7), p.W - 1);
        mk[ps] = __builtin_bit_cast(f32x4, __builtin_amdgcn_raw_buffer_load_b128(
                                               mk_rsrc, (((n * p.H + ho) * p.W + wo) * p.Cout + n0 + e4) * 4, 0, 0));
      }
    }
#pragma unroll
    for (int b = 0; b < NB; ++b)
#pragma unroll
      for (int r = 0; r < 16; ++r) {
        const int i = (r & 3) + 8 * (r >> 2) + 4 * (lane >> 5);
        scratch[i * LD4 + wave * 32 * NB + b * 32 + (lane & 31)] = acc[a][b][r];
      }
    __syncthreads();
#pragma unroll
    for (int ps = 0; ps < EP; ++ps) {
      const int i = er0 + ps * RPP;
      const int m = a * 32 + i;
      const int ho = ty * 8 + (m >> 3), wo = tx * TW + (m & 7);
      f32x4 v = *reinterpret_cast<const f32x4*>(scratch + i * LD4 + e4);
      v += bias;
      if (p.relu) {
#pragma unroll
        for (int t = 0; t < 4; ++t) v[t] = fmaxf(v[t], 0.f);
      }
      if (p.mask) {
#pragma unroll
        for (int t = 0; t < 4; ++t) v[t] = mk[ps][t] > 0.f ? v[t] : 0.f;
      }
      if (ho < p.H && wo < p.W)
        __builtin_amdgcn_raw_buffer_store_b128(__builtin_bit_cast(u32x4, v), y_rsrc,
                                               (((n * p.H + ho) * p.W + wo) * p.Cout + n0 + e4) * 4, 0, BGS_P3_Y_AUX);
    }
    __syncthreads();
  }
}

template <int NB>
__global__ __launch_bounds__(kThreads, 3) void conv3x3s2_planes_bfx_kernel(Planes3Args g) {
  const ConvArgs& p = g.c;
  constexpr int NS = 3;
  constexpr int PW = 17, PS = 12, SG = 9 * PS * 32;
  constexpr int AQ = PW * PW * 4, AQT = (AQ + kThreads - 1) / kThreads;
  constexpr int PL = 4 * SG, BUF = NS * PL;
  constexpr int CO = 128 * NB, LD4 = CO + 8;
  static_assert(3 * BUF <= 160 * 1024, "three workgroups per CU");
  static_assert(32 * LD4 * 4 <= BUF, "epilogue tile overlays the operand buffer");
  __shared__ __attribute__((aligned(1024))) unsigned char lds[BUF];

  const int tid = threadIdx.x, lane = tid & 63;
  const int wave = bgs::uniform(tid >> 6);
  const int frow = lane & 31, fk = lane >> 5;
  const int vtile = (int)((blockIdx.x & 7) * p.chunk + (blockIdx.x >> 3));
  if (vtile >= p.tiles_m * p.tiles_n) return;
  const int tm = vtile / p.tiles_n, tn = vtile - tm * p.tiles_n;
  const int per_img = g.tiles_y * g.tiles_x;
  const int n = tm / per_img, trem = tm - n * per_img;
  const int ty = trem / g.tiles_x, tx = trem - ty * g.tiles_x;
  const int h0 = ty * 16 - 1, w0 = tx * 16 - 1;
  const int n0 = tn * CO;
  const int cch16 = p.Cin >> 4;

  const __amdgpu_buffer_rsrc_t x_rsrc = __builtin_amdgcn_make_buffer_rsrc(
      const_cast<float*>(p.x), 0, (int)((size_t)p.N * p.H * p.W * p.Cin * 4), 0x00020000);
  int a_off[AQT], a_dst[AQT];
#pragma unroll
  for (int i = 0; i < AQT; ++i) {
    const int q = tid + kThreads * i;
    const bool use = q < AQ;
    const int pix = use ? q >> 2 : 0, quad = q & 3;
    const int ppy = pix / PW, ppx = pix - ppy * PW;
    const int hi = h0 + ppy, wi = w0 + ppx;
    const bool in = use && hi >= 0 && hi < p.H && wi >= 0 && wi < p.W;
    a_off[i] = in ? (((n * p.H + hi) * p.W + wi) * p.Cin + quad * 4) * 4 : kOob;
    const int iy = ppy >> 1, ix = ppx >> 1;
    a_dst[i] = use ? ((ppy & 1) * 2 + (ppx & 1)) * SG + (iy * PS + ix) * 32 + (((quad >> 1) ^ (iy & 1)) << 4) + (quad & 1) * 8 : -1;
  }
  f32x4 ra[AQT];
  auto load_a = [&](int chunk) {
#pragma unroll
    for (int i = 0; i < AQT; ++i)
      ra[i] = __builtin_bit_cast(f32x4, __builtin_amdgcn_raw_buffer_load_b128(x_rsrc, a_off[i], chunk * 64, 0));
  };
  auto store_a = [&]() {
#pragma unroll
    for (int i = 0; i < AQT; ++i) {
      if (a_dst[i] < 0) continue;
      u32x2 hh, mm, ll;
      split3(ra[i], hh, mm, ll);
      unsigned char* d = lds + a_dst[i];
      *reinterpret_cast<u32x2*>(d) = hh;
      *reinterpret_cast<u32x2*>(d + PL) = mm;
      *reinterpret_cast<u32x2*>(d + 2 * PL) = ll;
    }
  };

  const __amdgpu_buffer_rsrc_t b_rsrc = __builtin_amdgcn_make_buffer_rsrc(
      const_cast<__bf16*>(g.ws), 0, (int)((size_t)NS * g.KC * p.Cout * 32), 0x00020000);
  const int b_lane = ((n0 + wave * 32 * NB + frow) * 16 + fk * 8) * 2;
  const int b_plane = g.KC * p.Cout * 32;
  auto load_b = [&](int kc, bf16x8 (&dst)[NS][NB]) {
#pragma unroll
    for (int s = 0; s < NS; ++s)
#pragma unroll
      for (int b = 0; b < NB; ++b)
        dst[s][b] = __builtin_bit_cast(bf16x8, __builtin_amdgcn_raw_buffer_load_b128(
                                                   b_rsrc, b_lane, s * b_plane + (kc * p.Cout + 32 * b) * 32, 0));
  };

  int a_frag[2][2];
#pragma unroll
  for (int a = 0; a < 2; ++a) {
    const int m = a * 32 + frow;
    const int py = m >> 3, px = m & 7;
#pragma unroll
    for (int par = 0; par < 2; ++par) a_frag[a][par] = (py * PS + px) * 32 + ((fk ^ ((py + par) & 1)) << 4);
  }
  f32x16 acc[2][NB];
#pragma unroll
  for (int a = 0; a < 2; ++a)
#pragma unroll
    for (int b = 0; b < NB; ++b)
#pragma unroll
      for (int r = 0; r < 16; ++r) acc[a][b][r] = 0.f;

  bf16x8 fb0[NS][NB], fb1[NS][NB];
  load_a(0);
  load_b(0, fb0);
  for (int c2 = 0; c2 < cch16; c2 += 2) {
#pragma unroll
    for (int t = 0; t < 18; ++t) {
      const int chunk = c2 + t / 9, tap = t % 9, dy = tap / 3, dx = tap % 3;
      if (tap == 0) {
        __syncthreads();
        store_a();
        __syncthreads();
      }
      const int kc_next = tap < 8 ? (tap + 1) * cch16 + chunk : chunk + 1;
      if (t & 1) load_b(kc_next, fb0);
      else load_b(kc_next, fb1);
      if (tap == 0) load_a(chunk + 1);
      __builtin_amdgcn_sched_barrier(0);
      const bf16x8 (&fbu)[NS][NB] = (t & 1) ? fb1 : fb0;
      bf16x8 fa[NS][2];
#pragma unroll
      for (int s = 0; s < NS; ++s)
#pragma unroll
        for (int a = 0; a < 2; ++a)
          fa[s][a] = *reinterpret_cast<const bf16x8*>(lds + s * PL + ((dy & 1) * 2 + (dx & 1)) * SG + a_frag[a][dy >> 1] +
                                                      ((dy >> 1) * PS + (dx >> 1)) * 32);
#pragma unroll
      for (int tt = NS - 1; tt >= 0; --tt)
#pragma unroll
        for (int i = 0; i <= tt; ++i)
#pragma unroll
          for (int a = 0; a < 2; ++a)
#pragma unroll
            for (int b = 0; b < NB; ++b)
              acc[a][b] = __builtin_amdgcn_mfma_f32_32x32x16_bf16(fa[i][a], fbu[tt - i][b], acc[a][b], 0, 0, 0);
      __builtin_amdgcn_sched_barrier(0);
    }
  }
  __syncthreads();

  float* scratch = reinterpret_cast<float*>(lds);
  constexpr int TPR = CO / 4, RPP = kThreads / TPR, EP = 32 / RPP;
  const int e4 = (tid % TPR) * 4, er0 = tid / TPR;
  f32x4 bias = {0.f, 0.f, 0.f, 0.f};
  if (p.bias) bias = *reinterpret_cast<const f32x4*>(p.bias + n0 + e4);
  const __amdgpu_buffer_rsrc_t y_rsrc =
      __builtin_amdgcn_make_buffer_rsrc(p.y, 0, (int)((size_t)p.M * p.Cout * 4), 0x00020000);
#pragma unroll
  for (int a = 0; a < 2; ++a) {
#pragma unroll
    for (int b = 0; b < NB; ++b)
#pragma unroll
      for (int r = 0; r < 16; ++r) {
        const int i = (r & 3) + 8 * (r >> 2) + 4 * (lane >> 5);
        scratch[i * LD4 + wave * 32 * NB + b * 32 + (lane & 31)] = acc[a][b][r];
      }
    __syncthreads();
#pragma unroll
    for (int ps = 0; ps < EP; ++ps) {
      const int i = er0 + ps * RPP;
      const int m = a * 32 + i;
      const int ho = ty * 8 + (m >> 3), wo = tx * 8 + (m & 7);
      f32x4 v = *reinterpret_cast<const f32x4*>(scratch + i * LD4 + e4);
      v += bias;
      if (p.relu) {
#pragma unroll
        for (int t = 0; t < 4; ++t) v[t] = fmaxf(v[t], 0.f);
      }
      if (ho < p.Ho && wo < p.Wo)
        __builtin_amdgcn_raw_buffer_store_b128(__builtin_bit_cast(u32x4, v), y_rsrc,
                                               (((n * p.Ho + ho) * p.Wo + wo) * p.Cout + n0 + e4) * 4, 0, 0);
    }
    __syncthreads();
  }
}

int g_planes3_mode = -1;
int g_planes3_last = 0;

}

extern "C" void bgs_conv3x3_planes_enable(int mode) { g_planes3_mode = mode < 0 ? -1 : (mode > 2 ? 2 : mode); }
extern "C" int bgs_conv3x3_planes_last_launch(void) { return g_planes3_last; }
void bgs_internal_conv3x3_planes_clear_last() { g_planes3_last = 0; }

static int planes3_rule(int N, int H, int W, int Cout) {
  int mode = g_planes3_mode;
  if (mode < 0) {
    const char* e = getenv("BGS_BFX_PLANES3");
    mode = e ? atoi(e) : 1;
    if (mode < 0 || mode > 2) mode = 1;
  }
  if (mode == 0) return 0;
  const int tiles_y = (H + 7) / 8, tiles_x = (W + 7) / 8;
  const long long tiles_px = (long long)N * tiles_y * tiles_x;
  static int nb_env = -1;
  if (nb_env < 0) {
    const char* e = getenv("BGS_BFX_PLANES3_NB");
    nb_env = e ? atoi(e) : 0;
  }
  int nb = (Cout & 255) ? 1 : 2;
  if (nb == 2 && (nb_env == 1 || (nb_env == 0 && tiles_px * (Cout / 256) <= 768))) nb = 1;
  const long long wgs = tiles_px * (Cout / (128 * nb));
  if (mode == 1 && wgs < 256) return 0;
  return nb;
}

int bgs_internal_conv3x3_planes(const bgs_conv::ConvArgs& pc, const void* wsplit, int KC, hipStream_t st) {
  const ConvArgs& p = pc;
  if (p.R != 3 || p.S != 3 || p.stride != 1 || p.pad != 1 || p.rowmap || p.res_mode != 0) return -1;
  if ((p.Cin & 31) || (p.Cout & 127) || KC != 9 * (p.Cin / 16)) return -1;
  if (((uintptr_t)p.x | (uintptr_t)p.y | (uintptr_t)p.bias | (uintptr_t)p.mask | (uintptr_t)wsplit) & 15) return -1;
  const long long lim = kOob;
  if ((long long)p.N * p.H * p.W * p.Cin * 4 >= lim || (long long)p.M * p.Cout * 4 >= lim || (long long)3 * KC * p.Cout * 32 >= lim) return -1;
  const int tiles_y = (p.H + 7) / 8, tiles_x = (p.W + 7) / 8;
  const long long tiles_px = (long long)p.N * tiles_y * tiles_x;
  const int nb = planes3_rule(p.N, p.H, p.W, p.Cout);
  if (nb == 0) return -1;
  const long long wgs = tiles_px * (p.Cout / (128 * nb));
  {
  }
  Planes3Args g;
  g.c = p;
  g.ws = reinterpret_cast<const __bf16*>(wsplit);
  g.KC = KC;
  g.tiles_y = tiles_y;
  g.tiles_x = tiles_x;
  g.c.tiles_m = (int)tiles_px;
  g.c.tiles_n = p.Cout / (128 * nb);
  g.c.chunk = (int)((wgs + 7) / 8);
  g.c.partial = nullptr;
  const dim3 grid((unsigned)(8 * g.c.chunk)), block(kThreads);
  if (nb == 2) hipLaunchKernelGGL((conv3x3_planes_bfx_kernel<2>), grid, block, 0, st, g);
  else hipLaunchKernelGGL((conv3x3_planes_bfx_kernel<1>), grid, block, 0, st, g);
  g_planes3_last = nb;
  bgs_internal_census_bump(BGS_CENSUS_PLANES_3X3);
  return hipGetLastError() == hipSuccess ? BGS_OK : BGS_ERR_LAUNCH;
}

extern "C" int bgs_conv3x3_planes_head_eligible(int N, int H, int W, int Cin, int Cout, int Chead) {
  if (N <= 0 || H <= 0 || W <= 0 || Cout != 256 || Cin <= 0 || (Cin & 31) || Chead <= 0 || Chead > 32) return 0;
  if (!bgs_internal_halo_hooks_default()) return 0;
  if (planes3_rule(N, H, W, Cout) != 2) return 0;
  return bgs_internal_bfx_unsliced((long long)N * H * W, Chead, Cout / 16) ? 1 : 0;
}

extern "C" int bgs_conv3x3_planes_head_nhwc_f32_bfx(const float* x, const void* wsplit, const float* bias,
                                                    const void* hsplit, const float* hbias, float* y, int N, int H,
                                                    int W, int Cin, int Cout, int relu, int Chead,
                                                    bgs_stream_t stream) {
  if (N <= 0 || H <= 0 || W <= 0 || Cin <= 0 || Cout <= 0 || Chead <= 0) return BGS_ERR_INVALID_ARG;
  if (!x || !wsplit || !hsplit || !y) return BGS_ERR_INVALID_ARG;
  if (Cout != 256 || (Cin & 31) || Chead > 32) return BGS_ERR_UNSUPPORTED;
  if (((uintptr_t)x | (uintptr_t)wsplit | (uintptr_t)hsplit) & 15) return BGS_ERR_UNSUPPORTED;
  if (((uintptr_t)bias & 15) || (((uintptr_t)hbias | (uintptr_t)y) & 3)) return BGS_ERR_UNSUPPORTED;
  const long long M = (long long)N * H * W, lim = kOob;
  const int KC = 9 * (Cin / 16);
  if (M * Cin * 4 >= lim || M * Chead * 4 >= lim || (long long)3 * KC * Cout * 32 >= lim) return BGS_ERR_UNSUPPORTED;
  Planes3HeadArgs a;
  Planes3Args& g = a.g;
  ConvArgs& p = g.c;
  p = ConvArgs();
  p.x = x; p.w = nullptr; p.bias = bias; p.res = nullptr; p.mask = nullptr; p.y = nullptr;
  p.N = N; p.H = H; p.W = W; p.Cin = Cin; p.Cout = Cout; p.R = 3; p.S = 3; p.stride = 1; p.pad = 1;
  p.Ho = H; p.Wo = W; p.M = (int)M; p.K = 9 * Cin; p.relu = relu; p.res_mode = 0;
  p.partial = nullptr; p.kt_per_split = 0;
  g.ws = reinterpret_cast<const __bf16*>(wsplit);
  g.KC = KC;
  g.tiles_y = (H + 7) / 8;
  g.tiles_x = (W + 7) / 8;
  p.tiles_m = N * g.tiles_y * g.tiles_x;
  p.tiles_n = 1;
  p.chunk = (p.tiles_m + 7) / 8;
  a.hs = reinterpret_cast<const __bf16*>(hsplit);
  a.hbias = hbias;
  a.hy = y;
  a.CH = Chead;
  hipLaunchKernelGGL((conv3x3_planes_bfx_kernel<2, true>), dim3((unsigned)(8 * p.chunk)), dim3(kThreads), 0,
                     (hipStream_t)stream, a);
  g_planes3_last = 2;
  bgs_internal_census_bump(BGS_CENSUS_PLANES_3X3);
  bgs_internal_census_bump(BGS_CENSUS_PLANES_3X3_HEAD);
  return hipGetLastError() == hipSuccess ? BGS_OK : BGS_ERR_LAUNCH;
}

int bgs_internal_conv3x3s2_planes(const bgs_conv::ConvArgs& pc, const void* wsplit, int KC, hipStream_t st) {
  int mode = g_planes3_mode;
  if (mode < 0) {
    const char* e = getenv("BGS_BFX_PLANES3");
    mode = e ? atoi(e) : 1;
    if (mode < 0 || mode > 2) mode = 1;
  }
  static int s2_env = -1;
  if (s2_env < 0) {
    const char* e = getenv("BGS_BFX_PLANES3_S2");
    s2_env = e ? atoi(e) : 1;
  }
  if (mode == 0 || !s2_env) return -1;
  const ConvArgs& p = pc;
  if (p.R != 3 || p.S != 3 || p.stride != 2 || p.pad != 1 || p.mask || p.rowmap || p.res_mode != 0) return -1;
  if ((p.Cin & 31) || (p.Cout & 127) || KC != 9 * (p.Cin / 16)) return -1;
  if (p.Ho != (p.H - 1) / 2 + 1 || p.Wo != (p.W - 1) / 2 + 1) return -1;
  if (((uintptr_t)p.x | (uintptr_t)p.y | (uintptr_t)p.bias | (uintptr_t)wsplit) & 15) return -1;
  const long long lim = kOob;
  if ((long long)p.N * p.H * p.W * p.Cin * 4 >= lim || (long long)p.M * p.Cout * 4 >= lim || (long long)3 * KC * p.Cout * 32 >= lim) return -1;
  const int tiles_y = (p.Ho + 7) / 8, tiles_x = (p.Wo + 7) / 8;
  const long long tiles_px = (long long)p.N * tiles_y * tiles_x;
  const int nb = 1;
  const long long wgs = tiles_px * (p.Cout / (128 * nb));
  if (mode == 1 && wgs < 256) return -1;
  Planes3Args g;
  g.c = p;
  g.ws = reinterpret_cast<const __bf16*>(wsplit);
  g.KC = KC;
  g.tiles_y = tiles_y;
  g.tiles_x = tiles_x;
  g.c.tiles_m = (int)tiles_px;
  g.c.tiles_n = p.Cout / (128 * nb);
  g.c.chunk = (int)((wgs + 7) / 8);
  g.c.partial = nullptr;
  const dim3 grid((unsigned)(8 * g.c.chunk)), block(kThreads);
  hipLaunchKernelGGL((conv3x3s2_planes_bfx_kernel<1>), grid, block, 0, st, g);
  g_planes3_last = nb | 0x10;
  bgs_internal_census_bump(BGS_CENSUS_PLANES_3X3);
  return hipGetLastError() == hipSuccess ? BGS_OK : BGS_ERR_LAUNCH;
}
```

balancedgroupsoftmax_amd/functional.py:

```python
import ctypes
import itertools
import os

import torch

from . import capi

_WS = {}


def _workspace(nbytes, device):
    key = (device.index, capi.raw_stream(device))
    buf = _WS.get(key)
    if buf is None or buf.numel() < nbytes:
        buf = torch.empty(max(int(nbytes), 1 << 20), dtype=torch.uint8, device=device)
        _WS[key] = buf
    return buf


def reset_workspaces():
    _WS.clear()


_SIDE = {}
# ... 752 lines not shown
class conv_math_scope(object):

    def __init__(self, mode):
        self.mode = _checked_conv_math(mode, 'conv_math_scope')

    def __enter__(self):
        self.prev = set_conv_math(self.mode)
        return self

    def __exit__(self, *exc):
        set_conv_math(self.prev)
        return False


_BF16_STORAGE = [os.environ.get('BGS_BF16_STORAGE', '1') != '0']


def set_bf16_storage(on):
    prev = _BF16_STORAGE[0]
    _BF16_STORAGE[0] = bool(on)
    return prev


def bf16_storage_active():
    return _CONV_MATH[0] == 'bf16' and _BF16_STORAGE[0]


_FORK_FUSION = [os.environ.get('BGS_FORK_FUSION', '1') != '0']


def fork_fusion_enabled():
    return _FORK_FUSION[0]


def set_fork_fusion(on):
    prev = _FORK_FUSION[0]
    _FORK_FUSION[0] = bool(on)
    return prev


_SPLIT_CACHE = {}
_SPLIT_CACHE_MAX = 1024


class CacheFence(object):
    __slots__ = ('event', 'stream')

    def __init__(self, device=None):
        self.event = None
        self.stream = None
        if torch.cuda.is_available() and not torch.cuda.is_current_stream_capturing():
            st = torch.cuda.current_stream(device)
            self.event = torch.cuda.Event()
            self.event.record(st)
            self.stream = st.cuda_stream

    def wait(self, device=None):
        ev = self.event
        if ev is None:
            return
        if torch.cuda.is_current_stream_capturing():
            return
        if ev.query():
            self.event = None
            return
        st = torch.cuda.current_stream(device)
        if st.cuda_stream != self.stream:
            st.wait_event(ev)


def clear_split_cache():
    _SPLIT_CACHE.clear()


def bfx_split_weights(w2d, cache=True):
    _require_cuda(w2d)
    lib = capi.load()
    assert w2d.dtype == torch.float32 and w2d.dim() == 2 and w2d.is_contiguous()
    rows, K = w2d.shape
    cacheable = cache and not w2d.requires_grad
    key = w2d.data_ptr()
    if cacheable:
        hit = _SPLIT_CACHE.get(key)
        if hit is not None and hit[0] == w2d._version and hit[1] == (rows, K):
            hit[4].wait(w2d.device)
            return hit[3]
    out = torch.empty(lib.bgs_conv_bfx_weight_bytes(rows, K), dtype=torch.uint8, device=w2d.device)
    rc = lib.bgs_conv_bfx_split_weights(capi.ptr(w2d), capi.ptr(out), rows, K,
                                        capi.current_stream(w2d.device))
    capi.check('bgs_conv_bfx_split_weights', rc)
    if cacheable:
        if key not in _SPLIT_CACHE and len(_SPLIT_CACHE) >= _SPLIT_CACHE_MAX:
            _SPLIT_CACHE.pop(next(iter(_SPLIT_CACHE)))
        _SPLIT_CACHE[key] = (w2d._version, (rows, K), w2d, out, CacheFence(w2d.device))
    return out


def presplit(*weights):
    for w in weights:
        if w is not None and w.is_cuda and w.dim() == 4 and not w.requires_grad and \
                (_CONV_MATH[0] != 'f32' or bf16_storage_active()):
            bfx_split_weights(w.view(w.shape[0], -1), cache=True)


def bfx_split_weights_dgrad(w_krsc, cache=True):
    _require_cuda(w_krsc)
    lib = capi.load()
    assert w_krsc.dtype == torch.float32 and w_krsc.dim() == 4 and w_krsc.is_contiguous()
    Cout, R, S, Cin = w_krsc.shape
    cacheable = cache and not w_krsc.requires_grad
    key = (w_krsc.data_ptr(), 'dgrad')
    if cacheable:
        hit = _SPLIT_CACHE.get(key)
        if hit is not None and hit[0] == w_krsc._version and hit[1] == (Cout, R, S, Cin):
            hit[4].wait(w_krsc.device)
            return hit[3]
    out = torch.empty(lib.bgs_conv_bfx_weight_bytes(Cin, R * S * Cout), dtype=torch.uint8,
                      device=w_krsc.device)
    rc = lib.bgs_conv_bfx_split_weights_dgrad(capi.ptr(w_krsc), capi.ptr(out), Cout, R, S, Cin,
                                              capi.current_stream(w_krsc.device))
    capi.check('bgs_conv_bfx_split_weights_dgrad', rc)
    if cacheable:
        if key not in _SPLIT_CACHE and len(_SPLIT_CACHE) >= _SPLIT_CACHE_MAX:
            _SPLIT_CACHE.pop(next(iter(_SPLIT_CACHE)))
        _SPLIT_CACHE[key] = (w_krsc._version, (Cout, R, S, Cin), w_krsc, out, CacheFence(w_krsc.device))
    return out


def conv_bfx_tuning(tile=0, splitk=-1, halo_splits=-1, halo_variant=0, halo_geom=-1, halo_flags=0, halo_wide=-1):
    lib = capi.load()
    lib.bgs_conv_bfx_tuning(int(tile), int(splitk))
    lib.bgs_conv3x3_halo_bfx_tuning(int(halo_splits), int(halo_variant) | ((int(halo_geom) + 1) << 16) |
                                    (int(halo_flags) << 20) | ((int(halo_wide) + 1) << 24))


def set_halo_wide(mode):
    return capi.load().bgs_conv3x3_halo_bfx_wide(int(mode))


def conv_bfx_last_launch():
    import ctypes
    lib = capi.load()
    a, c, d, e, f, g = (ctypes.c_int() for _ in range(6))
    lib.bgs_conv_bfx_last_launch(ctypes.byref(a), ctypes.byref(c))
    lib.bgs_conv3x3_halo_bfx_last_launch(ctypes.byref(d), ctypes.byref(e))
    lib.bgs_conv3x3_halo_bfx_last_wide(ctypes.byref(f), ctypes.byref(g))
    return dict(tile=a.value & ~0x400, ring_stages=3 if a.value & 0x400 else 4, splits=c.value,
                halo_nb=d.value & 0xff, halo_variant=(d.value >> 8) & 0xff, halo_geom=d.value >> 16,
                halo_splits=e.value, halo_wide_units=f.value, halo_tail_units=g.value)


CENSUS = dict(bf16_ring8=0, grouped_lds=1, halo_bfx4=2, dma_ring64=3, gs_head_fused=4, conv1x1_bres=5,
              wgrad_bfx=6, roi_bwd_gather=7, bf16s=8, grouped_bf16s=9, bfx_wide=10, gs_scale_grad=11, halo_wide=12, stem_fused=13, fused_c3=14,
              planes_3x3=15, planes_1x1=16, planes_3x3_head=17, fused_c3_next=18, fused_c3_shortcut=19)


def launch_census(reset=False):
    lib = capi.load()
    out = {k: lib.bgs_launch_census(v, 0) for k, v in CENSUS.items()}
    if reset:
        lib.bgs_launch_census(0, 1)
    return out


def conv_tuning(tile=0, bk=0, splitk=0, noswizzle=0):
    capi.load().bgs_conv_tuning(int(tile), int(bk), int(splitk), int(noswizzle))


def conv_last_launch():
    import ctypes
    a, b, c, d = (ctypes.c_int() for _ in range(4))
    capi.load().bgs_conv_last_launch(ctypes.byref(a), ctypes.byref(b), ctypes.byref(c), ctypes.byref(d))
    return dict(tile=a.value, bk=b.value, up=c.value, splits=d.value)


def _use_halo_bfx(M, Cout):
    env = os.environ.get('BGS_CONV_HALO')
    if env == '1':
        return True
    if env == '0':
        return False
    return M >= 2000


def _use_halo_kernel(M, Cout):
    env = os.environ.get('BGS_CONV_HALO')
    if env == '1':
        return True
    if env == '0':
        return False
    return M >= 100000 and Cout % 128 == 0


_FUSED_C3 = [os.environ.get('BGS_FUSED_C3', '1') != '0']


def set_fused_c3(on):
    prev = _FUSED_C3[0]
    _FUSED_C3[0] = bool(on)
    return prev


def fused_c3_eligible(x, w2, w3, stride, residual):
    env = os.environ.get('BGS_FUSED_C3')
    on = _FUSED_C3[0] if env is None else env != '0'
    return (on and _CONV_MATH[0] == 'bf16x6' and x.is_cuda and x.dtype == torch.float32 and stride == 1
            and tuple(w2.shape[:3]) == (64, 3, 3) and w2.shape[3] == 64 and tuple(w3.shape) == (256, 1, 1, 64)
            and x.shape[3] == 64 and _use_halo_bfx(x.shape[0] * x.shape[1] * x.shape[2], 64)
            and x.shape[0] * ((x.shape[1] + 7) // 8) * ((x.shape[2] + 15) // 16) >= 700
            and not (torch.is_grad_enabled() and (x.requires_grad or w2.requires_grad or w3.requires_grad or
                                                  (residual is not None and residual.requires_grad)))
            and bool(capi.load().bgs_conv3x3_c3_fused_eligible(x.shape[0], x.shape[1], x.shape[2], 64, 256)))


def _c3_tail(x, w2_krsc, bias2, w3_krsc, bias3, residual=None, relu3=True, out=None, w1n_krsc=None, bias1n=None,
             x0=None, w_sc_krsc=None, bias_sc=None):
    _require_cuda(x, w2_krsc, bias2, w3_krsc, bias3, residual, w1n_krsc, bias1n, x0, w_sc_krsc, bias_sc)
    lib = capi.load()
    assert x.dtype == torch.float32 and x.is_contiguous() and x.dim() == 4
    N, H, W, Cmid = x.shape
    Cout3 = w3_krsc.shape[0]
    Cnext = 0 if w1n_krsc is None else w1n_krsc.shape[0]
    assert tuple(w2_krsc.shape) == (Cmid, 3, 3, Cmid) and tuple(w3_krsc.shape) == (Cout3, 1, 1, Cmid)
    if residual is not None:
        assert tuple(residual.shape) == (N, H, W, Cout3) and residual.is_contiguous() and residual.dtype == torch.float32
    y = out if out is not None else torch.empty((N, H, W, Cout3), dtype=torch.float32, device=x.device)
    w2s = bfx_split_weights(w2_krsc.view(Cmid, 9 * Cmid), cache=True)
    w3s = bfx_split_weights(w3_krsc.view(Cout3, Cmid), cache=True)
    h = w1s = None
    if Cnext:
        assert tuple(w1n_krsc.shape) == (Cnext, 1, 1, Cout3) and w1n_krsc.is_contiguous()
        h = torch.empty((N, H, W, Cnext), dtype=torch.float32, device=x.device)
        w1s = bfx_split_weights(w1n_krsc.view(Cnext, Cout3), cache=True)
    relu3 = int(bool(relu3))
    if x0 is not None:
        Cin0 = x0.shape[3]
        assert residual is None
        assert tuple(x0.shape) == (N, H, W, Cin0) and x0.is_contiguous() and x0.dtype == torch.float32
        assert tuple(w_sc_krsc.shape) == (Cout3, 1, 1, Cin0) and w_sc_krsc.is_contiguous()
        wss = bfx_split_weights(w_sc_krsc.view(Cout3, Cin0), cache=True)
        name = 'bgs_conv3x3_c3_sc_fused_nhwc_f32_bfx'
        tensors = (x, w2s, bias2, w3s, bias3, x0, wss, bias_sc, y, w1s, bias1n if Cnext else None, h)
        ints = (N, H, W, Cin0, Cmid, Cout3, relu3, Cnext)
    elif Cnext:
        name = 'bgs_conv3x3_c3_next_fused_nhwc_f32_bfx'
        tensors = (x, w2s, bias2, w3s, bias3, residual, y, w1s, bias1n, h)
        ints = (N, H, W, Cmid, Cout3, relu3, Cnext)
    else:
        name = 'bgs_conv3x3_c3_fused_nhwc_f32_bfx'
        tensors = (x, w2s, bias2, w3s, bias3, residual, y)
        ints = (N, H, W, Cmid, Cout3, relu3)
    rc = getattr(lib, name)(*[capi.ptr(t) for t in tensors], *ints, capi.current_stream(x.device))
    capi.check(name, rc)
    return y, h


def conv3x3_c3_fused_nhwc(x, w2_krsc, bias2, w3_krsc, bias3, residual=None, relu3=True, out=None):
    return _c3_tail(x, w2_krsc, bias2, w3_krsc, bias3, residual, relu3, out)[0]


def fused_c3_next_eligible(x, w2, w3, stride, residual, w1n, b1n=None, stride1n=1, pad1n=0):
    if os.environ.get('BGS_TAIL_NEXT_C1', '1') == '0':
        return False
    if w1n is None or w1n.dim() != 4 or stride1n != 1 or pad1n != 0:
        return False
    if tuple(w1n.shape[1:]) != (1, 1, 256) or w1n.shape[0] not in (64, 128) or w1n.dtype != torch.float32:
        return False
    if torch.is_grad_enabled() and (w1n.requires_grad or (b1n is not None and b1n.requires_grad)):
        return False
    if not fused_c3_eligible(x, w2, w3, stride, residual):
        return False
    N, H, W, _ = x.shape
    return bool(capi.load().bgs_conv3x3_c3_next_eligible(N, H, W, 64, 256, w1n.shape[0]))


def conv3x3_c3_next_fused_nhwc(x, w2_krsc, bias2, w3_krsc, bias3, w1n_krsc, bias1n, residual=None, relu3=True):
    return _c3_tail(x, w2_krsc, bias2, w3_krsc, bias3, residual, relu3, w1n_krsc=w1n_krsc, bias1n=bias1n)


def fused_c3_shortcut_eligible(x0, h1_shape, w2, w3, stride, w_sc, b_sc=None, stride_sc=1):
    if os.environ.get('BGS_TAIL_SHORTCUT', '1') == '0':
        return False
    if w_sc is None or w_sc.dim() != 4 or stride_sc != 1 or stride != 1:
        return False
    if tuple(w_sc.shape) != (256, 1, 1, 64) or w_sc.dtype != torch.float32 or not w_sc.is_contiguous():
        return False
    if x0.dim() != 4 or x0.shape[3] != 64 or x0.dtype != torch.float32 or not x0.is_cuda or not x0.is_contiguous():
        return False
    if tuple(h1_shape) != (x0.shape[0], x0.shape[1], x0.shape[2], 64):
        return False
    if torch.is_grad_enabled() and (x0.requires_grad or w_sc.requires_grad or (b_sc is not None and b_sc.requires_grad)):
        return False
    if not fused_c3_eligible(x0, w2, w3, stride, None):
        return False
    N, H, W, _ = x0.shape
    return bool(capi.load().bgs_conv3x3_c3_sc_eligible(N, H, W, 64, 64, 256, 0))


def conv3x3_c3_sc_fused_nhwc(x, w2_krsc, bias2, w3_krsc, bias3, x0, w_sc_krsc, bias_sc, w1n_krsc=None, bias1n=None,
                             relu3=True):
    y, h = _c3_tail(x, w2_krsc, bias2, w3_krsc, bias3, None, relu3, w1n_krsc=w1n_krsc, bias1n=bias1n, x0=x0,
                    w_sc_krsc=w_sc_krsc, bias_sc=bias_sc)
    return y if h is None else (y, h)


def rpn_head_fusion_eligible(x, w_conv, w_head):
    if os.environ.get('BGS_RPN_HEAD_FUSION', '1') == '0' or _CONV_MATH[0] != 'bf16x6':
        return False
    if not x.is_cuda or x.dtype != torch.float32 or x.dim() != 4 or w_conv.dim() != 4 or w_head.dim() != 4:
        return False
    N, H, W, Cin = x.shape
    if tuple(w_conv.shape[1:]) != (3, 3, Cin) or tuple(w_head.shape[1:]) != (1, 1, w_conv.shape[0]):
        return False
    if not _use_halo_bfx(N * H * W, w_conv.shape[0]):
        return False
    return bool(capi.load().bgs_conv3x3_planes_head_eligible(N, H, W, Cin, w_conv.shape[0], w_head.shape[0]))


def conv3x3_head_fused_nhwc(x, w_krsc, bias, hw_krsc, hbias, relu=True):
    _require_cuda(x, w_krsc, bias, hw_krsc, hbias)
    lib = capi.load()
    assert x.dtype == torch.float32 and x.is_contiguous() and x.dim() == 4
    N, H, W, Cin = x.shape
    Cout, Ch = w_krsc.shape[0], hw_krsc.shape[0]
    assert tuple(w_krsc.shape) == (Cout, 3, 3, Cin) and tuple(hw_krsc.shape) == (Ch, 1, 1, Cout)
    assert w_krsc.is_contiguous() and hw_krsc.is_contiguous()
    ws = bfx_split_weights(w_krsc.view(Cout, 9 * Cin), cache=True)
    hs = bfx_split_weights(hw_krsc.view(Ch, Cout), cache=True)
    out = torch.empty((N, H, W, Ch), dtype=torch.float32, device=x.device)
    rc = lib.bgs_conv3x3_planes_head_nhwc_f32_bfx(capi.ptr(x), capi.ptr(ws), capi.ptr(bias), capi.ptr(hs),
                                                  capi.ptr(hbias), capi.ptr(out), N, H, W, Cin, Cout,
                                                  int(bool(relu)), Ch, capi.current_stream(x.device))
    capi.check('bgs_conv3x3_planes_head_nhwc_f32_bfx', rc)
    return out


def conv2d_nhwc(x, w_krsc, bias=None, stride=1, pad=0, relu=False, residual=None,
                residual_mode=0, out=None, frozen_weight=True, out_dtype=None):
    _require_cuda(x, w_krsc, bias, residual)
    lib = capi.load()
    assert x.dtype in (torch.float32, torch.bfloat16) and w_krsc.dtype == torch.float32
    assert x.is_contiguous() and w_krsc.is_contiguous() and x.dim() == 4 and w_krsc.dim() == 4
    N, H, W, Cin = x.shape
    Cout, R, S, Cin2 = w_krsc.shape
    assert Cin == Cin2, (x.shape, w_krsc.shape)
    Ho = (H + 2 * pad - R) // stride + 1
    Wo = (W + 2 * pad - S) // stride + 1
    if residual is not None and residual_mode == 0:
        residual_mode = 1
    if residual is not None:
        exp = (N, Ho, Wo, Cout) if residual_mode == 1 else (N, Ho // 2, Wo // 2, Cout)
        assert tuple(residual.shape) == exp and residual.is_contiguous(), (residual.shape, exp)
    if x.dtype == torch.bfloat16:
        if out_dtype is None:
            out_dtype = torch.bfloat16
        assert out_dtype in (torch.float32, torch.bfloat16)
        assert residual is None or residual.dtype in (torch.float32, torch.bfloat16)
        if out is None:
            out = torch.empty((N, Ho, Wo, Cout), dtype=out_dtype, device=x.device)
        assert out.dtype == out_dtype
        wsplit = bfx_split_weights(w_krsc.view(Cout, R * S * Cin), cache=bool(frozen_weight))
        rc = lib.bgs_conv2d_nhwc_bf16s(capi.ptr(x), capi.ptr(wsplit), capi.ptr(bias), capi.ptr(residual),
                                       residual_mode if residual is not None else 0,
                                       int(residual is not None and residual.dtype == torch.bfloat16),
                                       capi.ptr(out), int(out_dtype == torch.bfloat16), N, H, W, Cin,
                                       Cout, R, S, stride, pad, int(bool(relu)),
                                       capi.current_stream(x.device))
        capi.check('bgs_conv2d_nhwc_bf16s', rc)
        return out
    assert out_dtype in (None, torch.float32), 'fp32 activations produce fp32 (bf16 out needs bf16 in)'
    assert residual is None or residual.dtype == torch.float32
    if out is None:
        out = torch.empty((N, Ho, Wo, Cout), dtype=torch.float32, device=x.device)
    halo_ok = R == 3 and S == 3 and stride == 1 and pad == 1 and residual is None and Cin % 16 == 0
    if _CONV_MATH[0] != 'f32':
        planes = 3 if _CONV_MATH[0] == 'bf16x6' else 1
        wsplit = bfx_split_weights(w_krsc.view(Cout, R * S * Cin), cache=bool(frozen_weight))
        st = capi.current_stream(x.device)
        if halo_ok and _use_halo_bfx(N * Ho * Wo, Cout):
            wsb = lib.bgs_conv3x3_halo_bfx_workspace_bytes(N, H, W, Cin, Cout)
            ws = _workspace(wsb, x.device) if wsb else None
            rc = lib.bgs_conv3x3_halo_nhwc_f32_bfx(capi.ptr(x), capi.ptr(wsplit), capi.ptr(bias),
                                                   capi.ptr(out), N, H, W, Cin, Cout,
                                                   int(bool(relu)), planes, capi.ptr(ws), wsb, st)
            capi.check('bgs_conv3x3_halo_nhwc_f32_bfx', rc)
            return out
        wsb = lib.bgs_conv_bfx_workspace_bytes(N * Ho * Wo, Cout, R * S * Cin)
        ws = _workspace(wsb, x.device) if wsb else None
        rc = lib.bgs_conv2d_nhwc_f32_bfx_ws(capi.ptr(x), capi.ptr(wsplit), capi.ptr(bias),
                                            capi.ptr(residual), capi.ptr(out), N, H, W, Cin, Cout,
                                            R, S, stride, pad, int(bool(relu)), residual_mode,
                                            planes, capi.ptr(ws), wsb, st)
        capi.check('bgs_conv2d_nhwc_f32_bfx_ws', rc)
        return out
    if halo_ok and _use_halo_kernel(N * Ho * Wo, Cout):
        rc = lib.bgs_conv3x3_halo_nhwc_f32(capi.ptr(x), capi.ptr(w_krsc), capi.ptr(bias),
                                           capi.ptr(out), N, H, W, Cin, Cout, int(bool(relu)),
                                           capi.current_stream(x.device))
        capi.check('bgs_conv3x3_halo_nhwc_f32', rc)
        return out
    wsb = lib.bgs_conv2d_workspace_bytes(N * Ho * Wo, Cout)
    ws = _workspace(wsb, x.device) if wsb else None
    rc = lib.bgs_conv2d_nhwc_f32_ws(capi.ptr(x), capi.ptr(w_krsc), capi.ptr(bias),
                                    capi.ptr(residual), capi.ptr(out), N, H, W, Cin, Cout, R, S,
                                    stride, pad, int(bool(relu)), residual_mode, capi.ptr(ws),
                                    wsb, capi.current_stream(x.device))
    capi.check('bgs_conv2d_nhwc_f32_ws', rc)
    return out


def dgrad_filter(w_krsc):
    return w_krsc.detach().permute(3, 1, 2, 0).flip(1, 2).contiguous()


def conv2d_dgrad_nhwc(dy, w_krsc, in_hw, stride=1, pad=0, residual=None, residual_mode=0,
                      mask=None, wt=None, frozen_weight=False):
    _require_cuda(dy, w_krsc, residual, mask)
    lib = capi.load()
    assert dy.dtype == torch.float32 and dy.is_contiguous() and dy.dim() == 4
    Cout, R, S, Cin = w_krsc.shape
    N, Ho, Wo, Cout2 = dy.shape
    H, W = in_hw
    assert Cout == Cout2 and Ho == (H + 2 * pad - R) // stride + 1 and \
        Wo == (W + 2 * pad - S) // stride + 1, (dy.shape, w_krsc.shape, in_hw)
    if Cout % 4 != 0:
        padc = 4 - Cout % 4
        dy = torch.nn.functional.pad(dy, (0, padc))
        w_krsc = torch.nn.functional.pad(w_krsc.detach(), (0, 0, 0, 0, 0, 0, 0, padc))
        Cout += padc
        wt = None
    wt_is_temp = wt is None
    fused_split = wt is None and _CONV_MATH[0] != 'f32' and os.environ.get('BGS_DGRAD_FUSED_SPLIT', '1') != '0'
    if wt is None and not fused_split:
        wt = dgrad_filter(w_krsc)
    if residual is not None and residual_mode == 0:
        residual_mode = 1
    if residual is not None:
        exp = (N, H, W, Cin) if residual_mode == 1 else (N, 2 * H, 2 * W, Cin)
        assert tuple(residual.shape) == exp and residual.is_contiguous(), (residual.shape, exp)
    if mask is not None:
        assert tuple(mask.shape) == (N, H, W, Cin) and mask.is_contiguous()
    dx = torch.empty((N, H, W, Cin), dtype=torch.float32, device=dy.device)
    if _CONV_MATH[0] != 'f32':
        if fused_split:
            wt_split = bfx_split_weights_dgrad(w_krsc.detach().contiguous(), cache=bool(frozen_weight))
        else:
            wt_split = bfx_split_weights(wt.view(Cin, R * S * Cout), cache=not wt_is_temp)
        if R == 3 and S == 3 and stride == 1 and pad == 1 and residual is None and Cout % 16 == 0 \
                and _use_halo_bfx(N * H * W, Cin) and os.environ.get('BGS_DGRAD_HALO', '1') != '0':
            wsb = lib.bgs_conv3x3_halo_bfx_workspace_bytes(N, H, W, Cout, Cin)
            ws = _workspace(wsb, dy.device) if wsb else None
            rc = lib.bgs_conv3x3_halo_nhwc_f32_bfx_ex(
                capi.ptr(dy), capi.ptr(wt_split), None, capi.ptr(mask), capi.ptr(dx), N, H, W, Cout,
                Cin, 0, 3 if _CONV_MATH[0] == 'bf16x6' else 1, capi.ptr(ws), wsb,
                capi.current_stream(dy.device))
# ... 1902 lines not shown
```

balancedgroupsoftmax_amd/train.py:

```python
from collections import OrderedDict

import torch
import torch.distributed as dist


def _scalar(v):
    return v if v.dim() == 0 else v.mean()


def _total(vals):
    vals = [v.reshape(()) for v in vals]
    if len(vals) == 1:
        return vals[0]
    return torch.stack(vals).sum()


_SEGMENT_MATS = {}


def _segment_matrix(lengths, device):
    key = (lengths, str(device))
    m = _SEGMENT_MATS.get(key)
    if m is None:
        n = sum(l for l, _ in lengths)
# ... 246 lines not shown


def _fused_sgd_eligible(optimizer, params, grad_clip):
    import os
    if os.environ.get('BGS_FUSED_SGD', '1') == '0' or type(optimizer) is not torch.optim.SGD:
        return False
    if len(optimizer.param_groups) != 1:
        return False
    g = optimizer.param_groups[0]
    if g.get('dampening', 0) != 0 or g.get('nesterov', False) or g.get('maximize', False):
        return False
    if grad_clip is not None and float(grad_clip.get('norm_type', 2)) != 2.0:
        return False
    return all(p.is_cuda and p.dtype == torch.float32 and p.is_contiguous() for p in params)


class FusedClipSGD(object):

    def __init__(self, optimizer, params, grad_clip=None):
        self.optimizer = optimizer
        self.params = list(params)
        self.max_norm = float(grad_clip['max_norm']) if grad_clip is not None else 0.0
        self.total_norm = None
        self._ws = None

    def step(self, grad_scale=1.0):
        import ctypes
        from . import capi
        lib = capi.load()
        group = self.optimizer.param_groups[0]
        ps = [p for p in self.params if p.grad is not None]
        if not ps:
            return
        dev = ps[0].device
        bufs = []
        for p in ps:
            st = self.optimizer.state[p]
            if st.get('momentum_buffer') is None:
                st['momentum_buffer'] = torch.zeros_like(p, memory_format=torch.contiguous_format)
            bufs.append(st['momentum_buffer'])
            if not p.grad.is_contiguous():
                p.grad = p.grad.contiguous()
        n = len(ps)
        arr = ctypes.c_void_p * n
        numel = (ctypes.c_longlong * n)(*[p.numel() for p in ps])
        wsb = lib.bgs_sgd_clip_workspace_bytes(numel, n)
        if self._ws is None or self._ws.numel() < wsb or self._ws.device != dev:
            self._ws = torch.empty(max(wsb, 1 << 16), dtype=torch.uint8, device=dev)
            self.total_norm = torch.zeros(1, dtype=torch.float32, device=dev)
        rc = lib.bgs_sgd_clip_step(arr(*[p.data_ptr() for p in ps]), arr(*[p.grad.data_ptr() for p in ps]),
                                   arr(*[b.data_ptr() for b in bufs]), numel, n, self.max_norm,
                                   float(grad_scale), float(group['lr']), float(group.get('momentum', 0.0)),
                                   float(group.get('weight_decay', 0.0)), capi.ptr(self._ws),
                                   self._ws.numel(), capi.ptr(self.total_norm), capi.current_stream(dev))
        capi.check('bgs_sgd_clip_step', rc)
        _bump_versions(ps)


def _bump_versions(tensors):
    try:
        torch.autograd.graph.increment_version(tensors)
    except (AttributeError, TypeError):
        for t in tensors:
            torch._C._increment_version(t)


class DistOptimizerStep(object):

    def __init__(self, params, optimizer, grad_clip=None, world_size=1, overlap=None,
                 bucket_bytes=32 << 20):
        self.params = list(params)
        self.optimizer = optimizer
        self.grad_clip = grad_clip
        self.world_size = world_size
        nbytes = sum(p.numel() * p.element_size() for p in self.params)
        if overlap is None:
            overlap = world_size > 1 and nbytes > bucket_bytes
        self.overlap = OverlappedGradExchange(self.params, world_size, bucket_bytes) \
            if (overlap and world_size > 1) else None
        self.fused = FusedClipSGD(optimizer, self.params, grad_clip) \
            if _fused_sgd_eligible(optimizer, self.params, grad_clip) else None

    def _clip_and_step(self, loss_scale=1.0):
        if self.fused is not None:
            self.fused.step(1.0 / loss_scale if loss_scale != 1.0 else 1.0)
            return
        if loss_scale != 1.0:
            grads = [p.grad for p in self.params if p.grad is not None]
            if grads:
                torch._foreach_div_(grads, float(loss_scale))
        if self.grad_clip is not None:
            torch.nn.utils.clip_grad_norm_(self.params, self.grad_clip['max_norm'],
                                           self.grad_clip.get('norm_type', 2))
        self.optimizer.step()

    def exchange_and_update(self):
        if self.overlap is not None:
            self.overlap.finish()
        else:
            allreduce_grads(self.params, self.world_size)
        self._clip_and_step()

    def __call__(self, loss):
        self.optimizer.zero_grad(set_to_none=False)
        backward_unit(loss)
        self.exchange_and_update()


class TrunkPipeline(object):

    def __init__(self, model, depth=2, lane=3, inference=False):
        if not inference and not model.trunk_is_frozen():
            raise ValueError('TrunkPipeline needs a frozen backbone / neck (selectp = 1 or 3); with a trainable trunk '
                             'the next batch\'s features depend on this step\'s update')
        bb = model.backbone
        nst = len(getattr(bb, 'res_layers', ()))
        split = model.with_neck and hasattr(bb, 'forward_partial') and nst >= 2
        if depth >= 3 and not split:
            depth = 2
        depth = max(2, min(int(depth), nst + 2 if split else 2))
        if depth == 2:
            self.stages = [model.extract_feat]
        elif depth == 3:
            self.stages = [bb, model.neck]
        else:
            k = depth - 2
            cuts = [(nst * g + k - 1) // k for g in range(k + 1)]
            self.stages = []
            for g in range(k):
                first, last = cuts[g], cuts[g + 1] - 1

                def piece(st, first=first, last=last, final=(g == k - 1)):
                    if first == 0:
                        r = bb.forward_partial(st, -1, last)
                    else:
                        r = bb.forward_partial(st[0], first, last, st[1])
                    return r[1] if final else r
                self.stages.append(piece)
            self.stages.append(model.neck)
        self.model = model
        self.depth = depth
        self.lane = lane
        self._slots = [None] * len(self.stages)
        self._device = next(model.parameters()).device

    @staticmethod
    def _record(obj, stream):
        if torch.is_tensor(obj):
            if obj.is_cuda:
                obj.record_stream(stream)
        elif isinstance(obj, (tuple, list)):
            for o in obj:
                TrunkPipeline._record(o, stream)

    def _launch(self, j, inp, producer):
        from . import functional as BF
        with torch.no_grad():
            with BF.forked(self._device, lane=self.lane + j) as fk:
                if producer is not None:
                    producer.join()
                self._record(inp, fk.side)
                out = self.stages[j](inp)
        return fk, out

    def push(self, img):
        from . import functional as BF
        if img is not None:
            self._device = img.device
        elif all(s is None for s in self._slots):
            return
        if not BF._PIPELINE_ACTIVE[0]:
            BF._PIPELINE_ACTIVE[0] = id(self)
            self._wide_prev = BF.set_halo_wide(1)
            if self._wide_prev >= 0:
                BF.set_halo_wide(self._wide_prev)
        n = len(self.stages)
        assert self._slots[n - 1] is None, 'take() the finished features first'
        for j in range(n - 1, 0, -1):
            if self._slots[j - 1] is not None:
                fk, out = self._slots[j - 1]
                self._slots[j] = self._launch(j, out, fk)
                self._slots[j - 1] = None
        if img is not None:
            self._slots[0] = self._launch(0, img, None)
        elif all(s is None for s in self._slots):
            self._deactivate()

    def prefetch(self, img):
        self.push(img)

    def take(self):
        from . import functional as BF
        n = len(self.stages)
        assert self._slots[n - 1] is not None, 'push() %d batches first' % n
        fk, feats = self._slots[n - 1]
        fk.join()
        self._record(feats, torch.cuda.current_stream(self._device))
        self._slots[n - 1] = None
        if all(s is None for s in self._slots):
            self._deactivate()
        return feats

    def __del__(self):
        try:
            self._deactivate()
        except Exception:
            pass

    def _deactivate(self):
        from . import functional as BF
        if BF._PIPELINE_ACTIVE[0] == id(self):
            BF._PIPELINE_ACTIVE[0] = 0
            if getattr(self, '_wide_prev', 0) < 0:
                BF.set_halo_wide(-1)

    def drain(self):
        from . import functional as BF
        for j, s in enumerate(self._slots):
            if s is not None:
                s[0].join()
                self._slots[j] = None
        self._deactivate()


def backward_unit(loss):
    if loss.is_cuda and loss.dtype == torch.float32 and loss.numel() == 1:
        from . import functional as BF
        loss.backward(BF.unit_gradient(loss.device).reshape(loss.shape))
    else:
        loss.backward()


def wrap_fp16_model(model, math='bf16'):
    from . import functional as BF
    assert math in ('bf16',), math
    unwrap_fp16_model(model)
    model._conv_math = math
    stack = []

    def _enter(_m, _args, _kwargs=None):
        stack.append(BF.set_conv_math(model._conv_math))

    def _exit(_m, _args, _out):
        if stack:
            BF.set_conv_math(stack.pop())

    model._conv_math_hooks = (model.register_forward_pre_hook(_enter),
                              model.register_forward_hook(_exit, always_call=True))
    return BF.conv_math()


class fp16_scope(object):

    def __init__(self, model):
        self.math = getattr(model, '_conv_math', None)
        self._prev = []

    def __enter__(self):
        from . import functional as BF
        self._prev.append(BF.set_conv_math(self.math) if self.math else None)
        return self

    def __exit__(self, *exc):
        from . import functional as BF
        prev = self._prev.pop()
        if prev is not None:
            BF.set_conv_math(prev)
        return False


def unwrap_fp16_model(model):
    for h in getattr(model, '_conv_math_hooks', ()):
        h.remove()
    model._conv_math_hooks = ()
    model._conv_math = None


class Fp16OptimizerStep(DistOptimizerStep):

    def __init__(self, params, optimizer, grad_clip=None, world_size=1, loss_scale=512.0, **kw):
        super().__init__(params, optimizer, grad_clip=grad_clip, world_size=world_size, **kw)
        self.loss_scale = float(loss_scale)

    def exchange_and_update(self):
        if self.overlap is not None:
            self.overlap.finish()
        else:
            allreduce_grads(self.params, self.world_size)
        self._clip_and_step(self.loss_scale)

    def __call__(self, loss):
        self.optimizer.zero_grad(set_to_none=False)
        (loss * self.loss_scale).backward()
        self.exchange_and_update()
```

include/bgs.h:

```cpp
#ifndef BGS_H_
#define BGS_H_

#include <stddef.h>
#include <stdint.h>

#ifdef __cplusplus
extern "C" {
#endif

#define BGS_OK 0
#define BGS_ERR_INVALID_ARG 1
#define BGS_ERR_UNSUPPORTED 2
#define BGS_ERR_LAUNCH 3

#define BGS_MAX_BINS 16

typedef void* bgs_stream_t;

int bgs_version(void);
const char* bgs_error_string(int code);



int bgs_gs_prepare(const int64_t* labels, const int64_t* label2binlabel,
                   const float* cls_weight, int cls_weight_stride, const float* row_weights,
                   int N, int C, int B, double others_sample_ratio, uint64_t seed,
                   const uint64_t* seed_offset, int32_t* bin_labels_out, float* weights_out, float* avg_out,
                   bgs_stream_t stream);

size_t bgs_gs_loss_workspace_bytes(int N, int B);
int bgs_gs_loss_fwd_bwd(const float* logits, const int32_t* bin_labels,
                        const int64_t* host_pred_slice,
                        const float* weights, const float* avg,
                        int N, int B, int W,
                        float* loss_out, float* dlogits, void* workspace,
                        bgs_stream_t stream);

int bgs_gs_head_loss_fused(const float* logits, const int64_t* labels, const int64_t* label2binlabel,
                           const float* row_weights, const int64_t* host_pred_slice, int N, int C,
                           int B, int W, double others_sample_ratio, uint64_t seed,
                           const uint64_t* seed_offset, float* loss_out, float* dlogits,
                           float* avg_out, int32_t* bin_labels_out, float* weights_out,
                           void* workspace, bgs_stream_t stream);
int bgs_gs_head_step(const float* logits, const int64_t* labels, const int64_t* label2binlabel,
                     const uint16_t* class_bin_mask, const float* row_weights,
                     const int64_t* host_pred_slice, const float* host_bin_loss_weight, int N, int C,
                     int B, int W, double others_sample_ratio, uint64_t seed, uint64_t* draw_counter,
                     const float* bbox_pred, const float* bbox_targets, const float* bbox_weights,
                     int num_reg_classes, float beta, float box_loss_weight, float* loss_out,
                     float* total_out, float* dlogits, float* dbbox_pred, float* avg_out,
                     int32_t* bin_labels_out, float* weights_out, void* workspace,
                     bgs_stream_t stream);
int bgs_gs_class_bin_mask(const int64_t* label2binlabel, int C, int B, uint16_t* out,
                          bgs_stream_t stream);
int bgs_gs_head_step_scale_grad(float* dlogits, float* dbbox_pred, const int64_t* host_pred_slice,
                                const float* grad_terms, const float* grad_total, int N, int B, int W,
                                int num_reg_classes, bgs_stream_t stream);
int bgs_gs_loss_reduce(const void* workspace, int N, int B, float* loss_out, bgs_stream_t stream);

int bgs_gs_scale_grad(float* dlogits, const int64_t* host_pred_slice, const float* g,
                      int N, int B, int W, bgs_stream_t stream);

int bgs_gs_merge_score(const float* logits, const int64_t* host_pred_slice,
                       const int32_t* cls2col,
                       int N, int C, int B, int W, float* scores_out, bgs_stream_t stream);

size_t bgs_bbox_loss_workspace_bytes(int N);
int bgs_bbox_smooth_l1_fwd_bwd(const float* bbox_pred, const int64_t* labels,
                               const float* bbox_targets, const float* bbox_weights,
                               int N, int R, float beta, float avg_factor, float loss_weight,
                               float* loss_out, float* dbbox_pred, void* workspace,
                               bgs_stream_t stream);

int bgs_fc_reg_gather(const float* x, const float* w, const float* bias, const int64_t* labels,
                      int K, int C, int R, float* y, bgs_stream_t stream);

int bgs_conv2d_nhwc_f32(const float* x, const float* w, const float* bias, const float* residual,
                        float* y, int N, int H, int W, int Cin, int Cout, int R, int S,
                        int stride, int pad, int relu, int residual_mode, bgs_stream_t stream);

size_t bgs_conv2d_workspace_bytes(long long M, int Cout);
int bgs_conv2d_nhwc_f32_ws(const float* x, const float* w, const float* bias, const float* residual,
                           float* y, int N, int H, int W, int Cin, int Cout, int R, int S,
                           int stride, int pad, int relu, int residual_mode, void* workspace,
                           size_t workspace_bytes, bgs_stream_t stream);
int bgs_conv2d_dgrad_nhwc_f32_ws(const float* dy, const float* wt, const float* residual,
                                 const float* mask, float* dx, int N, int H, int W, int Cin,
                                 int Cout, int R, int S, int stride, int pad, int residual_mode,
                                 void* workspace, size_t workspace_bytes, bgs_stream_t stream);

int bgs_conv2d_dgrad_nhwc_f32(const float* dy, const float* wt, const float* residual,
                              const float* mask, float* dx, int N, int H, int W, int Cin,
                              int Cout, int R, int S, int stride, int pad, int residual_mode,
                              bgs_stream_t stream);
size_t bgs_conv2d_wgrad_workspace_bytes(int N, int H, int W, int Cin, int Cout, int R, int S,
                                        int stride, int pad);
int bgs_conv2d_wgrad_nhwc_f32(const float* x, const float* dy, float* dw, float* db, int N, int H,
                              int W, int Cin, int Cout, int R, int S, int stride, int pad,
                              int accumulate, void* workspace, bgs_stream_t stream);
size_t bgs_conv2d_wgrad_bfx_workspace_bytes(int N, int H, int W, int Cin, int Cout, int R, int S,
                                            int stride, int pad);
int bgs_conv2d_wgrad_nhwc_f32_bfx(const float* x, const float* dy, float* dw, float* db, int N, int H,
                                  int W, int Cin, int Cout, int R, int S, int stride, int pad,
                                  int accumulate, int planes, void* workspace, bgs_stream_t stream);

int bgs_fold_conv_bn_fwd(const float* w, const float* conv_bias, const float* gamma,
                         const float* beta, const float* mean, const float* var, float eps, int Cout,
                         int Cin, int R, int S, int cin_padded, float* wf, float* bf,
                         bgs_stream_t stream);
int bgs_fold_conv_bn_bwd(const float* dwf, const float* dbf, const float* w, const float* conv_bias,
                         const float* gamma, const float* mean, const float* var, float eps, int Cout,
                         int Cin, int R, int S, int cin_padded, float* dw, float* dconv_bias,
                         float* dgamma, float* dbeta, bgs_stream_t stream);


int bgs_conv3x3_halo_nhwc_f32(const float* x, const float* w, const float* bias, float* y, int N,
                              int H, int W, int Cin, int Cout, int relu, bgs_stream_t stream);

size_t bgs_conv_bfx_weight_bytes(int rows, int K);
int bgs_conv_bfx_split_weights(const float* w, void* out, int rows, int K, bgs_stream_t stream);
int bgs_conv_bfx_split_weights_dgrad(const float* w, void* out, int Cout, int R, int S, int Cin,
                                     bgs_stream_t stream);
size_t bgs_conv_bfx_workspace_bytes(long long M, int Cout, int K);
int bgs_conv2d_nhwc_f32_bfx_ws(const float* x, const void* wsplit, const float* bias,
                               const float* residual, float* y, int N, int H, int W, int Cin,
                               int Cout, int R, int S, int stride, int pad, int relu,
                               int residual_mode, int planes, void* workspace,
                               size_t workspace_bytes, bgs_stream_t stream);
int bgs_conv2d_dgrad_nhwc_f32_bfx_ws(const float* dy, const void* wt_split, const float* residual,
                                     const float* mask, float* dx, int N, int H, int W, int Cin,
                                     int Cout, int R, int S, int stride, int pad,
                                     int residual_mode, int planes, void* workspace,
                                     size_t workspace_bytes, bgs_stream_t stream);
size_t bgs_conv3x3_halo_bfx_workspace_bytes(int N, int H, int W, int Cin, int Cout);
int bgs_conv3x3_halo_nhwc_f32_bfx(const float* x, const void* wsplit, const float* bias, float* y,
                                  int N, int H, int W, int Cin, int Cout, int relu, int planes,
                                  void* workspace, size_t workspace_bytes, bgs_stream_t stream);
int bgs_conv3x3_halo_nhwc_f32_bfx_ex(const float* x, const void* wsplit, const float* bias,
                                     const float* mask, float* y, int N, int H, int W, int Cin,
                                     int Cout, int relu, int planes, void* workspace,
                                     size_t workspace_bytes, bgs_stream_t stream);
int bgs_conv3x3_c3_fused_nhwc_f32_bfx(const float* x, const void* w2split, const float* bias2,
                                      const void* w3split, const float* bias3, const float* residual,
                                      float* y, int N, int H, int W, int Cmid, int Cout3, int relu3,
                                      bgs_stream_t stream);
int bgs_conv3x3_c3_fused_eligible(int N, int H, int W, int Cmid, int Cout3);
int bgs_conv3x3_c3_next_fused_nhwc_f32_bfx(const float* x, const void* w2split, const float* bias2,
                                           const void* w3split, const float* bias3, const float* residual,
                                           float* y, const void* w1n_split, const float* bias1n, float* h,
                                           int N, int H, int W, int Cmid, int Cout3, int relu3, int Cnext,
                                           bgs_stream_t stream);
int bgs_conv3x3_c3_next_eligible(int N, int H, int W, int Cmid, int Cout3, int Cnext);
int bgs_conv3x3_c3_sc_fused_nhwc_f32_bfx(const float* x, const void* w2split, const float* bias2,
                                         const void* w3split, const float* bias3, const float* x0,
                                         const void* wsc_split, const float* bias_sc, float* y,
                                         const void* w1n_split, const float* bias1n, float* h, int N, int H, int W,
                                         int Cin0, int Cmid, int Cout3, int relu3, int Cnext, bgs_stream_t stream);
int bgs_conv3x3_c3_sc_eligible(int N, int H, int W, int Cin0, int Cmid, int Cout3, int Cnext);
int bgs_conv3x3_planes_head_nhwc_f32_bfx(const float* x, const void* wsplit, const float* bias,
                                         const void* hsplit, const float* hbias, float* y, int N, int H,
                                         int W, int Cin, int Cout, int relu, int Chead, bgs_stream_t stream);
int bgs_conv3x3_planes_head_eligible(int N, int H, int W, int Cin, int Cout, int Chead);


int bgs_grouped_conv3x3_nhwc_f32(const float* x, const float* w, const float* bias, float* y,
                                 int N, int H, int W, int C, int groups, int stride, int relu,
                                 bgs_stream_t stream);

int bgs_grouped_conv3x3_nhwc_bf16ops(const float* x, const float* w, const float* bias, float* y,
                                     int N, int H, int W, int C, int groups, int stride, int relu,
                                     bgs_stream_t stream);

int bgs_conv2d_nhwc_bf16s(const void* x, const void* w_hi, const float* bias, const void* residual,
                          int residual_mode, int residual_bf16, void* y, int y_bf16, int N, int H, int W,
                          int Cin, int Cout, int R, int S, int stride, int pad, int relu,
                          bgs_stream_t stream);
int bgs_grouped_conv3x3_nhwc_bf16s(const void* x, const float* w, const float* bias, void* y, int N, int H,
                                   int W, int C, int groups, int stride, int relu, bgs_stream_t stream);
int bgs_maxpool3x3s2_nhwc_f32_to_bf16(const float* x, void* y, int N, int H, int W, int C,
                                      bgs_stream_t stream);

int bgs_grouped_conv3x3_dgrad_nhwc_f32(const float* dy, const float* wt, float* dx, int N, int H,
                                       int W, int C, int groups, int stride, bgs_stream_t stream);
size_t bgs_grouped_conv3x3_wgrad_workspace_bytes(int N, int H, int W, int C, int groups, int stride);
int bgs_grouped_conv3x3_wgrad_nhwc_f32(const float* x, const float* dy, float* dw, float* db, int N,
                                       int H, int W, int C, int groups, int stride, int accumulate,
                                       void* workspace, bgs_stream_t stream);

int bgs_deform_conv3x3_nhwc_f32(const float* x, const float* offset, const float* w, const float* bias,
                                float* y, int N, int H, int W, int C, int groups, int deformable_groups,
                                int off_pitch, int stride, int relu, bgs_stream_t stream);
int bgs_deform_conv3x3_dgrad_nhwc_f32(const float* x, const float* offset, const float* w, const float* dz,
                                      float* dx, float* doffset, int N, int H, int W, int C, int groups,
                                      int deformable_groups, int off_pitch, int stride, bgs_stream_t stream);
size_t bgs_deform_conv3x3_wgrad_workspace_bytes(int N, int H, int W, int C, int groups, int stride);
int bgs_deform_conv3x3_wgrad_nhwc_f32(const float* x, const float* offset, const float* dz, float* dw,
                                      float* db, int N, int H, int W, int C, int groups, int deformable_groups,
                                      int off_pitch, int stride, int accumulate, void* workspace,
                                      bgs_stream_t stream);

size_t bgs_sigmoid_focal_workspace_bytes(void);
int bgs_sigmoid_focal_fwd(const float* logits, long long ld, const int64_t* labels, int N, int C, float gamma,
                          float alpha, int pos_shift, float* losses, bgs_stream_t stream);
int bgs_sigmoid_focal_bwd(const float* logits, long long ld, const int64_t* labels, const float* d_losses, int N,
                          int C, float gamma, float alpha, int pos_shift, float* d_logits, bgs_stream_t stream);
int bgs_sigmoid_focal_fwd_bwd(const float* logits, long long ld, const int64_t* labels, const float* row_weights,
                              const float* cls_weight, int N, int C, float gamma, float alpha, int pos_shift,
                              const float* avg, float loss_weight, float* loss_out, float* dlogits, void* workspace,
                              bgs_stream_t stream);

int bgs_nchw_to_nhwc4_f32(const float* x, float* y, int N, int C, int H, int W, bgs_stream_t stream);

size_t bgs_stem_fused_weight_bytes(void);
int bgs_stem_fused_split_weights(const float* w, int cin_stride, void* out, bgs_stream_t stream);
int bgs_stem_conv7x7s2_relu_maxpool_nchw_f32(const float* img, const void* wsplit, const float* bias, float* out,
                                             int N, int H, int W, bgs_stream_t stream);

int bgs_maxpool3x3s2_nhwc_f32(const float* x, float* y, int N, int H, int W, int C,
                              bgs_stream_t stream);
int bgs_maxpool3x3s2_bwd_nhwc_f32(const float* x, const float* dy, float* dx, int N, int H, int W,
                                  int C, bgs_stream_t stream);

int bgs_roi_align_nhwc_fwd(const float* const* host_feats, const int* host_heights,
                           const int* host_widths, const float* host_scales, int num_levels,
                           int num_images, float finest_scale, const float* rois, int K, int C,
                           int pooled_h, int pooled_w, int sample_num, float* out,
                           int* levels_out, bgs_stream_t stream);

int bgs_roi_align_nhwc_bwd(float* const* host_dfeats, const int* host_heights,
                           const int* host_widths, const float* host_scales, int num_levels,
                           int num_images, float finest_scale, const float* rois, int K, int C,
                           int pooled_h, int pooled_w, int sample_num, const float* dout,
                           bgs_stream_t stream);

int bgs_roi_align_nhwc_fwd_f16(const void* const* host_feats, const int* host_heights,
                               const int* host_widths, const float* host_scales, int num_levels,
                               int num_images, float finest_scale, const float* rois, int K, int C,
                               int pooled_h, int pooled_w, int sample_num, void* out, int* levels_out,
                               bgs_stream_t stream);
int bgs_roi_align_nhwc_bwd_f16(float* const* host_dfeats, const int* host_heights,
                               const int* host_widths, const float* host_scales, int num_levels,
                               int num_images, float finest_scale, const float* rois, int K, int C,
                               int pooled_h, int pooled_w, int sample_num, const void* dout,
                               bgs_stream_t stream);

int bgs_roi_align_nhwc_fwd_ex(const float* const* host_feats, const int* host_heights,
                              const int* host_widths, const float* host_scales, int num_levels,
                              int num_images, float finest_scale, const float* rois, int K, int C,
                              int pooled_h, int pooled_w, int sample_num, int pool,
                              int accumulate, float* out, int* levels_out, bgs_stream_t stream);
int bgs_roi_align_nhwc_bwd_ex(float* const* host_dfeats, const int* host_heights,
                              const int* host_widths, const float* host_scales, int num_levels,
                              int num_images, float finest_scale, const float* rois, int K, int C,
                              int pooled_h, int pooled_w, int sample_num, int pool,
                              const float* dout, bgs_stream_t stream);

int bgs_resize_bilinear_nhwc_f32(const float* x, float* y, int N, int H, int W, int C, int Ho,
                                 int Wo, int align_corners, bgs_stream_t stream);
int bgs_resize_bilinear_nhwc_bwd_f32(const float* dy, float* dx, int N, int H, int W, int C,
                                     int Ho, int Wo, int align_corners, bgs_stream_t stream);

size_t bgs_topk_workspace_bytes(int P, int kmax);
int bgs_topk_sorted_f32(const float* const* host_rows, const int* host_len, const int* host_k,
                        const int* host_inner, const int* host_pitch, int P, int kmax,
                        float* out_val, long long* out_idx, void* workspace, bgs_stream_t stream);

size_t bgs_nms_workspace_bytes(int P, int nmax);
int bgs_nms_batched(const float* boxes, const int* counts, int P, int nmax, float iou_thr,
                    int iou_mode, int max_keep, int* keep, int* keep_count, void* workspace,
                    bgs_stream_t stream);

int bgs_nms_gather(const float* boxes, const int* keep, const int* keep_count, int R, int nmax,
                   float* out_boxes, float* out_scores, bgs_stream_t stream);
int bgs_gather_boxes(const float* flat, const long long* idx, const float* scores, int N, int T, int num,
                     float* props, unsigned char* valid, bgs_stream_t stream);
int bgs_nms_merge_select(const float* boxes, const int* keep, const int* keep_count, int N, int L, int nmax,
                         int num, float* props, unsigned char* valid, bgs_stream_t stream);

int bgs_soft_nms_batched(const float* dets, const int* counts, int P, int nmax, float iou_thr, int method,
                         float sigma, float min_score, int* order, float* scores, int* keep_count,
                         bgs_stream_t stream);

int bgs_det_candidates(const float* scores, const float* boxes, const unsigned char* valid,
                       const float* score_factors, int B, int n, int C, int box_cols, float score_thr, int mode,
                       float* dets, int* idx, int* counts, bgs_stream_t stream);
int bgs_det_select(const float* dets, const int* idx, const int* keep, const float* sel_scores,
                   const int* keep_count, int B, int num_problems, int n, int max_num, float* out_dets,
                   int* out_labels, int* out_count, void* workspace, bgs_stream_t stream);

int bgs_aug_map_boxes(const float* const* host_src, const unsigned char* const* host_valid, int A, int n,
                      int src_cols, int nbox, const float* host_scale, const int* host_flip, const int* host_width,
                      int back, int out_mode, float* out, float* out_scores, int* out_count, bgs_stream_t stream);
int bgs_aug_merge_bboxes(const float* const* host_boxes, const float* const* host_scores, int A, int n, int box_cols,
                         int C, const float* host_scale, const int* host_flip, const int* host_width,
                         const unsigned char* valid, float* out_boxes, float* out_scores, bgs_stream_t stream);
int bgs_aug_merge_masks(const float* const* host_masks, const int* host_flip, int M, int k, int size, float* out,
                        bgs_stream_t stream);

int bgs_img_prep_u8(const unsigned char* const* host_src, const int* host_geom, int V, int channels,
                    const float* lut, int swap_rb, float* out, int Hp, int Wp, bgs_stream_t stream);

int bgs_gt_mask_prep_u8(const int* host_desc, const int* desc, int M, const unsigned* host_prefix,
                        const unsigned* prefix, long long prefix_len, unsigned char* out, int Hp, int Wp,
                        bgs_stream_t stream);
int bgs_gt_seg_prep_u8(const int* host_desc, const int* desc, int N, unsigned char* out, int Hs, int Ws,
                       bgs_stream_t stream);

size_t bgs_iou_assign_workspace_bytes(int N, int A, int G_total);
int bgs_iou_assign(const float* boxes, long long box_img_stride, int box_stride,
                   const uint8_t* valid, const float* gt, const int* host_gt_offsets, int N, int A,
                   float pos_iou_thr, float neg_iou_lo, float neg_iou_hi, float min_pos_iou,
                   int* assigned, float* max_overlaps_out, void* workspace, bgs_stream_t stream);

size_t bgs_rpn_loss_workspace_bytes(int N, int A_total, int L);
int bgs_rpn_loss(const float* const* host_level_outs, const int* host_level_hw, int L,
// ... 161 lines not shown
```

include/bgs_tuning.h:

```cpp
#ifndef BGS_TUNING_H_
#define BGS_TUNING_H_

#include "bgs.h"

#ifdef __cplusplus
extern "C" {
#endif

int bgs_selftest_wave_reduce(const float* in, float* out, bgs_stream_t stream);
int bgs_selftest_mfma_peak(int blocks, int iters, float* out, bgs_stream_t stream);
int bgs_selftest_mfma_peak_bf16(int blocks, int iters, int random_operands, float* out, bgs_stream_t stream);

#define BGS_CENSUS_BF16_RING8 0
#define BGS_CENSUS_GROUPED_LDS 1
#define BGS_CENSUS_HALO_BFX4 2
#define BGS_CENSUS_DMA_RING64 3
#define BGS_CENSUS_GS_HEAD_FUSED 4
#define BGS_CENSUS_CONV1X1_BRES 5
#define BGS_CENSUS_WGRAD_BFX 6
#define BGS_CENSUS_ROI_BWD_GATHER 7
#define BGS_CENSUS_BF16S 8
#define BGS_CENSUS_GROUPED_BF16S 9
#define BGS_CENSUS_BFX_WIDE 10
#define BGS_CENSUS_GS_SCALE_GRAD 11
#define BGS_CENSUS_HALO_WIDE 12
#define BGS_CENSUS_STEM_FUSED 13
#define BGS_CENSUS_FUSED_C3 14
#define BGS_CENSUS_PLANES_3X3 15
#define BGS_CENSUS_PLANES_1X1 16
#define BGS_CENSUS_PLANES_3X3_HEAD 17
#define BGS_CENSUS_FUSED_C3_NEXT 18
#define BGS_CENSUS_FUSED_C3_SHORTCUT 19
#define BGS_CENSUS_FAMILIES 20
int bgs_launch_census(int family, int reset);

void bgs_gs_head_debug_timestamps(unsigned long long* buf);
void bgs_gs_head_tuning(int rows_per_workgroup);
void bgs_gs_head_variant(int variant);
int bgs_gs_head_variant_used(int N);

void bgs_conv_tuning(int tile, int bk, int splitk, int noswizzle);
int bgs_conv_last_launch(int* tile, int* bk, int* up, int* splits);
void bgs_conv_bfx_tuning(int tile, int splitk);
int bgs_conv_bfx_last_launch(int* tile, int* splits);
void bgs_conv3x3_halo_bfx_tuning(int splits, int variant);
int bgs_conv3x3_halo_bfx_last_launch(int* nb, int* splits);
int bgs_conv3x3_halo_bfx_last_wide(int* wide_units, int* tail_units);
int bgs_conv3x3_halo_bfx_wide(int mode);
void bgs_conv1x1_bres_enable(int on);
int bgs_conv1x1_bres_last_launch(void);
void bgs_conv_dgrad_parity_enable(int on);
void bgs_conv2d_wgrad_bfx_enable(int on);
void bgs_conv_bf16s_tuning(int variant);

void bgs_conv_bfx_wide_tuning(int mode, int nst, int splitk);
int bgs_conv_bfx_wide_last_launch(void);
void bgs_conv1x1_planes_enable(int mode);
int bgs_conv1x1_planes_last_launch(void);
void bgs_conv3x3_planes_enable(int mode);
int bgs_conv3x3_planes_last_launch(void);

void bgs_gs_loss_tuning(int prefetch);
void bgs_gs_loss_wavepriv_min_rows(int rows);
void bgs_gs_merge_tuning(int mode, int min_rows);

#ifdef __cplusplus
}
#endif
#endif
```

Measured before the change: 442.1.

## Fuse FPN P2 lateral into layer1 tail kernel and upsample-add into P2 3x3

The last layer1 bottleneck tail kernel now also computes the raw FPN lateral 1x1 conv on the tile it already holds in LDS. It writes the lateral output alongside the block output and the next block's conv1. The neck then skips the separate lateral conv and residual add for P2, and runs a new 3x3 kernel that folds the nearest upsample-add of the coarser lateral into its input read. This cuts kernel launches and a full-resolution fp32 round trip through memory. The costs are a shallower weight prefetch ring in the tail kernel and extra LDS staging passes. It applies only to frozen, non-trainable necks and needs the backbone to be attached to the neck.

After: 422.9. 0.957x the previous value.

```diff
diff --git a/balancedgroupsoftmax_amd/backbone.py b/balancedgroupsoftmax_amd/backbone.py
--- a/balancedgroupsoftmax_amd/backbone.py
+++ b/balancedgroupsoftmax_amd/backbone.py
@@ -38,6 +38,14 @@
         if pad_cin_to is not None and w.shape[3] < pad_cin_to:
             w = torch.nn.functional.pad(w, (0, pad_cin_to - w.shape[3]))
         return w.contiguous(), b.contiguous()
+
+
+class TrunkMaps(tuple):
+
+    def __new__(cls, maps, raw_lat0=None, raw_lat0_filter=None):
+        self = super().__new__(cls, maps)
+        self.raw_lat0, self.raw_lat0_filter = raw_lat0, raw_lat0_filter
+        return self
 
 
 def _tensor_slots(mods):
@@ -180,7 +188,7 @@
             fk.join()
         return BF.conv2d_nhwc(out, f['c3'][0], f['c3'][1], relu=True, residual=identity)
 
-    def run(self, x, f, next_c1=None, h=None):
+    def run(self, x, f, next_c1=None, h=None, lateral=None):
         if h is not None and (x.dtype == torch.bfloat16 or self.groups > 1 or self.with_dcn or
                               (torch.is_grad_enabled() and x.requires_grad)):
             raise RuntimeError('Bottleneck.run: a precomputed conv1 output is for the frozen fp32 block only')
@@ -247,6 +255,11 @@
                 fk.join()
             if next_c1 is not None and BF.fused_c3_next_eligible(out, f['c2'][0], f['c3'][0], self.stride, identity,
                                                                  next_c1[0], next_c1[1]):
+                if lateral is not None and BF.fused_c3_lateral_eligible(out, f['c2'][0], f['c3'][0], self.stride, identity,
+                                                                        next_c1[0], next_c1[1], lateral[0], lateral[1]):
+                    return BF.conv3x3_c3_next_lat_fused_nhwc(out, f['c2'][0], f['c2'][1], f['c3'][0], f['c3'][1],
+                                                             next_c1[0], next_c1[1], lateral[0], lateral[1],
+                                                             residual=identity, relu3=True)
                 return BF.conv3x3_c3_next_fused_nhwc(out, f['c2'][0], f['c2'][1], f['c3'][0], f['c3'][1], next_c1[0],
                                                      next_c1[1], residual=identity, relu3=True)
             return BF.conv3x3_c3_fused_nhwc(out, f['c2'][0], f['c2'][1], f['c3'][0], f['c3'][1], residual=identity,
@@ -304,7 +317,11 @@
         self.feat_dim = inplanes
         self._cache = _FoldCache()
         self._stem_split = _FoldCache()
+        self.lateral_hint = None
         self._freeze_stages()
+
+    def attach_neck(self, neck):
+        self.lateral_hint = getattr(neck, 'raw_lateral_fold', None)
 
     def _freeze_stages(self):
         if self.frozen_stages >= 0:
@@ -357,6 +374,7 @@
         return self.forward_partial(img, -1, len(self.res_layers) - 1)[1]
 
     def forward_partial(self, x, first, last, outs=()):
+        raw, raw_filter = getattr(outs, 'raw_lat0', None), getattr(outs, 'raw_lat0_filter', None)
         outs = list(outs)
         if first < 0:
             x = self._forward_stem(x)
@@ -369,14 +387,22 @@
             if nxt is not None and blk.width == 64 and blk.stride == 1 and blk.groups == 1 and not blk.with_dcn \
                     and nxt.groups == 1 and not nxt.with_dcn and not _trainable(nxt):
                 fn = nxt.folded()
-            r = blk.run(x, f if f is not None else blk.folded(), next_c1=None if fn is None else fn['c1'], h=h)
+            lateral = None
+            if fn is not None and i == 0 and chain[k + 1][0] == 1 and self.lateral_hint is not None \
+                    and len(self.out_indices) > 0 and self.out_indices[0] == 0:
+                lateral = self.lateral_hint()
+            r = blk.run(x, f if f is not None else blk.folded(), next_c1=None if fn is None else fn['c1'], h=h,
+                        lateral=lateral)
+            if isinstance(r, tuple) and len(r) == 3:
+                raw, raw_filter = r[2], lateral[0]
+                r = r[:2]
             x, h = r if isinstance(r, tuple) else (r, None)
             f = fn
             if k + 1 < len(chain) and chain[k + 1][0] == i:
                 continue
             if i in self.out_indices:
                 outs.append(BF.relu_gate(x))
-        return x, tuple(outs)
+        return x, (tuple(outs) if raw is None else TrunkMaps(outs, raw, raw_filter))
 
     def _forward_stem(self, img):
         stem = self._cache.get((self.conv1, self.bn1), self._build_stem)
@@ -449,6 +475,21 @@
     def _build_fold(self):
         return dict(lat=[_fold_conv_bn(m.conv, None) for m in self.lateral_convs],
                     out=[_fold_conv_bn(m.conv, None) for m in self.fpn_convs])
+
+    def raw_lateral_fold(self):
+        if self.num_ins < 2 or _trainable(self):
+            return None
+        return self._cache.get(self, self._build_fold)['lat'][0]
+
+    def _p2_fused(self, inputs, f, up):
+        raw = getattr(inputs, 'raw_lat0', None)
+        if raw is None or inputs.raw_lat0_filter is not f['lat'][0][0] or _trainable(self):
+            return None
+        if torch.is_grad_enabled() and (inputs[0].requires_grad or up.requires_grad):
+            return None
+        if tuple(raw.shape[:3]) != tuple(inputs[0].shape[:3]) or not BF.conv3x3_up_eligible(raw, up, f['out'][0][0]):
+            return None
+        return BF.conv3x3_up_nhwc(raw, up, *f['out'][0])
 
     def forward(self, inputs):
         assert len(inputs) == self.num_ins
@@ -469,15 +510,25 @@
                         extra = []
                         for _ in range(self.num_outs - n):
                             extra.append((extra[-1] if extra else outs[i])[:, ::2, ::2, :].contiguous())
+                if i == 1:
+                    outs[0] = self._p2_fused(inputs, f, lat[1])
+                    if outs[0] is not None:
+                        break
                 lat[i - 1] = BF.conv2d_autograd(inputs[i - 1], *f['lat'][i - 1], residual=lat[i],
                                                 residual_mode=2, out_dtype=torch.float32, mask_input=gate[i - 1])
-            outs[0] = BF.conv2d_autograd(lat[0], *f['out'][0], pad=1)
+            if outs[0] is None:
+                outs[0] = BF.conv2d_autograd(lat[0], *f['out'][0], pad=1)
             fk.join()
             return tuple(outs + extra)
+        p2 = None
         for i in range(n - 2, -1, -1):
+            if i == 0:
+                p2 = self._p2_fused(inputs, f, lat[1])
+                if p2 is not None:
+                    break
             lat[i] = BF.conv2d_autograd(inputs[i], *f['lat'][i], residual=lat[i + 1],
                                         residual_mode=2, out_dtype=torch.float32, mask_input=gate[i])
-        outs = [BF.conv2d_autograd(lat[i], *f['out'][i], pad=1) for i in range(n)]
+        outs = [p2 if i == 0 and p2 is not None else BF.conv2d_autograd(lat[i], *f['out'][i], pad=1) for i in range(n)]
         for _ in range(self.num_outs - n):
             outs.append(outs[-1][:, ::2, ::2, :].contiguous())
         return tuple(outs)
diff --git a/balancedgroupsoftmax_amd/capi.py b/balancedgroupsoftmax_amd/capi.py
--- a/balancedgroupsoftmax_amd/capi.py
+++ b/balancedgroupsoftmax_amd/capi.py
@@ -114,6 +114,14 @@
     'bgs_conv3x3_planes_head_nhwc_f32_bfx': (ctypes.c_int, [c_f32p, c_ptr, c_f32p, c_ptr, c_f32p, c_f32p]
                                              + [ctypes.c_int] * 7 + [c_ptr]),
     'bgs_conv3x3_planes_head_eligible': (ctypes.c_int, [ctypes.c_int] * 6),
+    'bgs_conv3x3_c3_next_lat_fused_nhwc_f32_bfx': (ctypes.c_int,
+                                                   [c_f32p, c_ptr, c_f32p, c_ptr, c_f32p, c_f32p, c_f32p, c_ptr,
+                                                    c_f32p, c_f32p, c_ptr, c_f32p, c_f32p] + [ctypes.c_int] * 8
+                                                   + [c_ptr]),
+    'bgs_conv3x3_c3_next_lat_eligible': (ctypes.c_int, [ctypes.c_int] * 7),
+    'bgs_conv3x3_planes_up_nhwc_f32_bfx': (ctypes.c_int, [c_f32p, c_f32p, c_ptr, c_f32p, c_f32p]
+                                           + [ctypes.c_int] * 6 + [c_ptr]),
+    'bgs_conv3x3_planes_up_eligible': (ctypes.c_int, [ctypes.c_int] * 5),
     'bgs_gs_loss_tuning': (None, [ctypes.c_int]),
     'bgs_gs_loss_wavepriv_min_rows': (None, [ctypes.c_int]),
     'bgs_gs_merge_tuning': (None, [ctypes.c_int, ctypes.c_int]),
diff --git a/balancedgroupsoftmax_amd/csrc/bottleneck_tail_planes.hip b/balancedgroupsoftmax_amd/csrc/bottleneck_tail_planes.hip
--- a/balancedgroupsoftmax_amd/csrc/bottleneck_tail_planes.hip
+++ b/balancedgroupsoftmax_amd/csrc/bottleneck_tail_planes.hip
@@ -33,14 +33,23 @@
   const __bf16* wssc;
   const float* bias_sc;
 };
-template <int NEXT, bool SC = false> struct TailArgsOf { typedef TailNextArgs type; };
-template <> struct TailArgsOf<0, false> { typedef TailArgs type; };
-template <int NEXT> struct TailArgsOf<NEXT, true> { typedef TailScArgs<typename TailArgsOf<NEXT>::type> type; };
+struct TailLatArgs {
+  TailNextArgs a;
+  const __bf16* wsl;
+  const float* bias_l;
+  float* lat;
+};
+template <int NEXT, bool SC = false, bool LAT = false> struct TailArgsOf { typedef TailNextArgs type; };
+template <> struct TailArgsOf<0, false, false> { typedef TailArgs type; };
+template <int NEXT> struct TailArgsOf<NEXT, true, false> { typedef TailScArgs<typename TailArgsOf<NEXT>::type> type; };
+template <> struct TailArgsOf<128, false, true> { typedef TailLatArgs type; };
 __device__ __forceinline__ const TailArgs& tail_base(const TailArgs& a) { return a; }
 __device__ __forceinline__ const TailArgs& tail_base(const TailNextArgs& a) { return a.t; }
 template <class A> __device__ __forceinline__ const TailArgs& tail_base(const TailScArgs<A>& a) { return tail_base(a.a); }
+__device__ __forceinline__ const TailArgs& tail_base(const TailLatArgs& a) { return a.a.t; }
 template <class A> __device__ __forceinline__ const A& tail_inner(const A& a) { return a; }
 template <class A> __device__ __forceinline__ const A& tail_inner(const TailScArgs<A>& a) { return a.a; }
+__device__ __forceinline__ const TailNextArgs& tail_inner(const TailLatArgs& a) { return a.a; }
 
 constexpr int kOob = 0x7f000000;
 
@@ -67,9 +76,10 @@
     dst[s] = __builtin_bit_cast(bf16x8, __builtin_amdgcn_raw_buffer_load_b128(bs_rsrc, lane_off, ((s * 4 + (t & 3)) * 256 + 32 * (t >> 2)) * 32, 0));
 }
 
-template <int NEXT, bool SC = false>
-__global__ __launch_bounds__(kThreads, 3) void bottleneck_tail_planes_kernel(typename TailArgsOf<NEXT, SC>::type ga) {
+template <int NEXT, bool SC = false, bool LAT = false>
+__global__ __launch_bounds__(kThreads, 3) void bottleneck_tail_planes_kernel(typename TailArgsOf<NEXT, SC, LAT>::type ga) {
   static_assert(NEXT == 0 || NEXT == 64 || NEXT == 128, "width of the next block's conv1");
+  static_assert(!LAT || (NEXT == 128 && !SC), "the FPN lateral reads the output of layer1's LAST block");
   static_assert(!SC || NEXT != 128, "a block with a stride-1 projection shortcut (layer1.0) is never in front of a 128-wide conv1");
   const TailArgs& g = tail_base(ga);
   const auto& gn = tail_inner(ga);
@@ -398,9 +408,10 @@
       for (int s = 0; s < NS; ++s)
         dst[s] = __builtin_bit_cast(bf16x8, __builtin_amdgcn_raw_buffer_load_b128(bn_rsrc, bn_lane, (s * KCN + kc) * NEXT * 32, 0));
     };
-    bf16x8 fn[3][NS];
+    constexpr int PF = LAT ? 2 : 3;
+    bf16x8 fn[PF][NS];
     load_bn(0, fn[0]);
-    load_bn(1, fn[1]);
+    if constexpr (PF == 3) load_bn(1, fn[1]);
     f32x4 vs[2][8];
 #pragma unroll
     for (int ps = 0; ps < 8; ++ps) {
@@ -428,8 +439,7 @@
     for (int a = 0; a < NA; ++a)
 #pragma unroll
       for (int r = 0; r < 16; ++r) accn[a][r] = 0.f;
-#pragma unroll
-    for (int c = 0; c < 2; ++c) {
+    auto stage_chunk = [&](int c) {
 #pragma unroll
       for (int ps = 0; ps < 8; ++ps) {
         const int i = (lane >> 5) * 32 + er0 + ps * 4;
@@ -440,13 +450,17 @@
         *reinterpret_cast<u32x2*>(d + PLN) = mm;
         *reinterpret_cast<u32x2*>(d + 2 * PLN) = ll;
       }
+    };
+#pragma unroll
+    for (int c = 0; c < 2; ++c) {
+      stage_chunk(c);
       __syncthreads();
 #pragma unroll
       for (int k8 = 0; k8 < KCH; ++k8) {
         const int kc = c * KCH + k8;
-        if (kc + 2 < KCN) load_bn(kc + 2, fn[(kc + 2) % 3]);
+        if (kc + PF - 1 < KCN) load_bn(kc + PF - 1, fn[(kc + PF - 1) % PF]);
         __builtin_amdgcn_sched_barrier(0);
-        const bf16x8 (&fbn)[NS] = fn[kc % 3];
+        const bf16x8 (&fbn)[NS] = fn[kc % PF];
         bf16x8 fan[NS][NA];
 #pragma unroll
         for (int s = 0; s < NS; ++s)
@@ -472,7 +486,9 @@
       }
     __syncthreads();
     constexpr int TPRN = NEXT / 4, RPPN = kThreads / TPRN, EPN = 64 / RPPN;
-    const int n4 = (tid % TPRN) * 4, nr0 = tid / TPRN;
+    int th = tid;
+    if constexpr (LAT) asm volatile("" : "+v"(th));
+    const int n4 = (th % TPRN) * 4, nr0 = th / TPRN;
     f32x4 biasn = {0.f, 0.f, 0.f, 0.f};
     if (gn.bias1n) biasn = *reinterpret_cast<const f32x4*>(gn.bias1n + n4);
     const __amdgpu_buffer_rsrc_t h_rsrc =
@@ -487,6 +503,83 @@
       for (int t = 0; t < 4; ++t) v[t] = fmaxf(v[t], 0.f);
       if (ho < g.H && wo < g.W)
         __builtin_amdgcn_raw_buffer_store_b128(__builtin_bit_cast(u32x4, v), h_rsrc, (((n * g.H + ho) * g.W + wo) * NEXT + n4) * 4, 0, 0);
+    }
+
+    if constexpr (LAT) {
+      const TailLatArgs& gl = ga;
+      const __amdgpu_buffer_rsrc_t bl_rsrc = __builtin_amdgcn_make_buffer_rsrc(
+          const_cast<__bf16*>(gl.wsl), 0, NS * KCN * CO3 * 32, 0x00020000);
+      const int bl_lane = ((wave * 32 + frow) * 16 + fk * 8) * 2;
+      auto load_bl = [&](int step, bf16x8 (&dst)[NS]) {
+        const int kc = (step >> 4) * KCH + (step & 7), pass = (step >> 3) & 1;
+#pragma unroll
+        for (int s = 0; s < NS; ++s)
+          dst[s] = __builtin_bit_cast(bf16x8, __builtin_amdgcn_raw_buffer_load_b128(bl_rsrc, bl_lane, ((s * KCN + kc) * CO3 + 128 * pass) * 32, 0));
+      };
+      bf16x8 fl[2][NS];
+      load_bl(0, fl[0]);
+      f32x16 accl[2][NA];
+#pragma unroll
+      for (int q = 0; q < 2; ++q)
+#pragma unroll
+        for (int a = 0; a < NA; ++a)
+#pragma unroll
+          for (int r = 0; r < 16; ++r) accl[q][a][r] = 0.f;
+      __syncthreads();
+#pragma unroll
+      for (int c = 0; c < 2; ++c) {
+        stage_chunk(c);
+        __syncthreads();
+#pragma unroll
+        for (int u = 0; u < 2 * KCH; ++u) {
+          const int step = c * 2 * KCH + u, pass = u / KCH, k8 = u % KCH;
+          if (step + 1 < 4 * KCH) load_bl(step + 1, fl[(step + 1) & 1]);
+          __builtin_amdgcn_sched_barrier(0);
+          const bf16x8 (&fbl)[NS] = fl[step & 1];
+          bf16x8 fal[NS][NA];
+#pragma unroll
+          for (int s = 0; s < NS; ++s)
+#pragma unroll
+            for (int a = 0; a < NA; ++a) fal[s][a] = *reinterpret_cast<const bf16x8*>(lds + s * PLN + k8 * KSN + an_frag[a]);
+#pragma unroll
+          for (int tt = NS - 1; tt >= 0; --tt)
+#pragma unroll
+            for (int i = 0; i <= tt; ++i)
+#pragma unroll
+              for (int a = 0; a < NA; ++a)
+                accl[pass][a] = __builtin_amdgcn_mfma_f32_32x32x16_bf16(fal[i][a], fbl[tt - i], accl[pass][a], 0, 0, 0);
+          __builtin_amdgcn_sched_barrier(0);
+        }
+        __syncthreads();
+      }
+      int tl = tid;
+      asm volatile("" : "+v"(tl));
+      const int e4 = (tl & 63) * 4, er0 = tl >> 6;
+      f32x4 biasl = {0.f, 0.f, 0.f, 0.f};
+      if (gl.bias_l) biasl = *reinterpret_cast<const f32x4*>(gl.bias_l + e4);
+      const __amdgpu_buffer_rsrc_t l_rsrc = __builtin_amdgcn_make_buffer_rsrc(gl.lat, 0, out_bytes, 0x00020000);
+#pragma unroll
+      for (int a = 0; a < NA; ++a) {
+#pragma unroll
+        for (int q = 0; q < 2; ++q)
+#pragma unroll
+          for (int r = 0; r < 16; ++r) {
+            const int i = (r & 3) + 8 * (r >> 2) + 4 * (lane >> 5);
+            scratch[i * LD4 + q * 128 + wave * 32 + (lane & 31)] = accl[q][a][r];
+          }
+        __syncthreads();
+#pragma unroll
+        for (int ps = 0; ps < 8; ++ps) {
+          const int i = er0 + ps * 4;
+          const int m = a * 32 + i;
+          const int ho = ty * 8 + (m >> 3), wo = tx * 8 + (m & 7);
+          f32x4 v = *reinterpret_cast<const f32x4*>(scratch + i * LD4 + e4);
+          v += biasl;
+          if (ho < g.H && wo < g.W)
+            __builtin_amdgcn_raw_buffer_store_b128(__builtin_bit_cast(u32x4, v), l_rsrc, (((n * g.H + ho) * g.W + wo) * CO3 + e4) * 4, 0, 0);
+        }
+        if (a + 1 < NA) __syncthreads();
+      }
     }
   }
 }
@@ -530,10 +623,10 @@
   return a;
 }
 
-template <int NEXT, bool SC>
-static int tail_launch(const typename TailArgsOf<NEXT, SC>::type& a, int chunk, bgs_stream_t stream,
+template <int NEXT, bool SC, bool LAT = false>
+static int tail_launch(const typename TailArgsOf<NEXT, SC, LAT>::type& a, int chunk, bgs_stream_t stream,
                        std::initializer_list<int> own_slots = {}) {
-  hipLaunchKernelGGL((bottleneck_tail_planes_kernel<NEXT, SC>), dim3((unsigned)(8 * chunk)), dim3(kThreads), 0,
+  hipLaunchKernelGGL((bottleneck_tail_planes_kernel<NEXT, SC, LAT>), dim3((unsigned)(8 * chunk)), dim3(kThreads), 0,
                      (hipStream_t)stream, a);
   bgs_internal_census_bump(BGS_CENSUS_FUSED_C3);
   for (int slot : own_slots) bgs_internal_census_bump(slot);
@@ -571,6 +664,27 @@
   const TailNextArgs a = tail_next_args(g, w1n_split, bias1n, h);
   return Cnext == 64 ? tail_launch<64, false>(a, g.chunk, stream, {BGS_CENSUS_FUSED_C3_NEXT})
                      : tail_launch<128, false>(a, g.chunk, stream, {BGS_CENSUS_FUSED_C3_NEXT});
+}
+
+extern "C" int bgs_conv3x3_c3_next_lat_eligible(int N, int H, int W, int Cmid, int Cout3, int Cnext, int Clat) {
+  return (Cnext == 128 && Clat == 256) ? tail_eligible(N, H, W, Cmid, Cout3) : 0;
+}
+
+extern "C" int bgs_conv3x3_c3_next_lat_fused_nhwc_f32_bfx(const float* x, const void* w2split, const float* bias2,
+                                                          const void* w3split, const float* bias3,
+                                                          const float* residual, float* y, const void* w1n_split,
+                                                          const float* bias1n, float* h, const void* wl_split,
+                                                          const float* bias_l, float* lat, int N, int H, int W,
+                                                          int Cmid, int Cout3, int relu3, int Cnext, int Clat,
+                                                          bgs_stream_t stream) {
+  if (N <= 0 || H <= 0 || W <= 0 || !x || !w2split || !w3split || !y || !w1n_split || !h || !wl_split || !lat)
+    return BGS_ERR_INVALID_ARG;
+  if (!bgs_conv3x3_c3_next_lat_eligible(N, H, W, Cmid, Cout3, Cnext, Clat)) return BGS_ERR_UNSUPPORTED;
+  if (!aligned16(x, w2split, w3split, y, residual, bias2, bias3, w1n_split, bias1n, h, wl_split, bias_l, lat))
+    return BGS_ERR_UNSUPPORTED;
+  const TailArgs g = tail_args(x, w2split, bias2, w3split, bias3, residual, y, N, H, W, relu3);
+  const TailLatArgs a = {tail_next_args(g, w1n_split, bias1n, h), reinterpret_cast<const __bf16*>(wl_split), bias_l, lat};
+  return tail_launch<128, false, true>(a, g.chunk, stream, {BGS_CENSUS_FUSED_C3_NEXT, BGS_CENSUS_FUSED_C3_LAT});
 }
 
 extern "C" int bgs_conv3x3_c3_sc_eligible(int N, int H, int W, int Cin0, int Cmid, int Cout3, int Cnext) {
diff --git a/balancedgroupsoftmax_amd/csrc/conv3x3_planes.hip b/balancedgroupsoftmax_amd/csrc/conv3x3_planes.hip
--- a/balancedgroupsoftmax_amd/csrc/conv3x3_planes.hip
+++ b/balancedgroupsoftmax_amd/csrc/conv3x3_planes.hip
@@ -38,15 +38,26 @@
   int CH;
 };
 
-template <bool HEAD>
+struct Planes3UpArgs {
+  Planes3Args g;
+  const float* up;
+};
+
+template <bool HEAD, bool UP = false>
 struct Planes3ArgsOf { typedef Planes3Args type; };
 template <>
-struct Planes3ArgsOf<true> { typedef Planes3HeadArgs type; };
+struct Planes3ArgsOf<true, false> { typedef Planes3HeadArgs type; };
+template <>
+struct Planes3ArgsOf<false, true> { typedef Planes3UpArgs type; };
 __device__ __forceinline__ const Planes3Args& planes3_base(const Planes3Args& a) { return a; }
 __device__ __forceinline__ const Planes3Args& planes3_base(const Planes3HeadArgs& a) { return a.g; }
-
-template <int NB, bool HEAD = false>
-__global__ __launch_bounds__(kThreads, 3) void conv3x3_planes_bfx_kernel(typename Planes3ArgsOf<HEAD>::type ga) {
+__device__ __forceinline__ const Planes3Args& planes3_base(const Planes3UpArgs& a) { return a.g; }
+template <class A> __device__ __forceinline__ const float* planes3_up(const A&) { return nullptr; }
+__device__ __forceinline__ const float* planes3_up(const Planes3UpArgs& a) { return a.up; }
+
+template <int NB, bool HEAD = false, bool UP = false>
+__global__ __launch_bounds__(kThreads, 3) void conv3x3_planes_bfx_kernel(typename Planes3ArgsOf<HEAD, UP>::type ga) {
+  static_assert(!(HEAD && UP), "the head form reads a stored map");
   const Planes3Args& g = planes3_base(ga);
   const ConvArgs& p = g.c;
   constexpr int NS = 3, KCH = 2;
@@ -74,32 +85,62 @@
 
   const __amdgpu_buffer_rsrc_t x_rsrc = __builtin_amdgcn_make_buffer_rsrc(
       const_cast<float*>(p.x), 0, (int)((size_t)p.N * p.H * p.W * p.Cin * 4), 0x00020000);
-  int a_off[4], a_dst[4];
-#pragma unroll
-  for (int i = 0; i < 4; ++i) {
-    const int q = tid + kThreads * i;
+  auto quad_geom = [&](int tl, int i, int& x_off, int& up_off, int& dst) {
+    const int q = tl + kThreads * i;
     const bool use = q < AQ;
     const int pix = use ? q >> 3 : 0, kq = q & 7;
     const int ppy = pix / PW, ppx = pix - ppy * PW;
     const int hi = h0 + ppy, wi = w0 + ppx;
     const bool in = use && hi >= 0 && hi < p.H && wi >= 0 && wi < p.W;
-    a_off[i] = in ? (((n * p.H + hi) * p.W + wi) * p.Cin + kq * 4) * 4 : kOob;
+    x_off = in ? (((n * p.H + hi) * p.W + wi) * p.Cin + kq * 4) * 4 : kOob;
+    up_off = in ? (((n * (p.H >> 1) + (hi >> 1)) * (p.W >> 1) + (wi >> 1)) * p.Cin + kq * 4) * 4 : kOob;
     const int quad = kq & 3;
-    a_dst[i] = use ? (kq >> 2) * KS + (ppy * PS + ppx) * 32 + (((quad >> 1) ^ (ppy & 1)) << 4) + (quad & 1) * 8 : -1;
+    dst = use ? (kq >> 2) * KS + (ppy * PS + ppx) * 32 + (((quad >> 1) ^ (ppy & 1)) << 4) + (quad & 1) * 8 : -1;
+  };
+  int a_off[UP ? 1 : 4], a_dst[UP ? 1 : 4];
+  if constexpr (!UP) {
+#pragma unroll
+    for (int i = 0; i < 4; ++i) {
+      int unused;
+      quad_geom(tid, i, a_off[i], unused, a_dst[i]);
+    }
   }
   f32x4 ra[4];
+  f32x4 ru[UP ? 4 : 1];
   auto load_a = [&](int chunk) {
 #pragma unroll
     for (int i = 0; i < 4; ++i)
       ra[i] = __builtin_bit_cast(f32x4, __builtin_amdgcn_raw_buffer_load_b128(x_rsrc, a_off[i], chunk * 128, BGS_P3_A_AUX));
   };
+  auto issue_up = [&](int i, int chunk) {
+    const float* upp = planes3_up(ga);
+    asm volatile("" : "+s"(upp));
+    const __amdgpu_buffer_rsrc_t u_rsrc = __builtin_amdgcn_make_buffer_rsrc(
+        const_cast<float*>(upp), 0, (int)((size_t)p.N * (p.H >> 1) * (p.W >> 1) * p.Cin * 4), 0x00020000);
+    int tl = tid;
+    asm volatile("" : "+v"(tl));
+    int xo, uo, dst;
+    quad_geom(tl, i, xo, uo, dst);
+    ra[i] = __builtin_bit_cast(f32x4, __builtin_amdgcn_raw_buffer_load_b128(x_rsrc, xo, chunk * 128, BGS_P3_A_AUX));
+    ru[i] = __builtin_bit_cast(f32x4, __builtin_amdgcn_raw_buffer_load_b128(u_rsrc, uo, chunk * 128, 0));
+  };
+  auto fold_up = [&](int i) { ra[i] += ru[i]; };
   auto store_a = [&](int buf) {
 #pragma unroll
     for (int i = 0; i < 4; ++i) {
-      if (a_dst[i] < 0) continue;
+      int dst;
+      if constexpr (UP) {
+        int tl = tid;
+        asm volatile("" : "+v"(tl));
+        int xo, uo;
+        quad_geom(tl, i, xo, uo, dst);
+      } else {
+        dst = a_dst[i];
+      }
+      if (dst < 0) continue;
       u32x2 hh, mm, ll;
       split3(ra[i], hh, mm, ll);
-      unsigned char* d = lds + buf * BUF + a_dst[i];
+      unsigned char* d = lds + buf * BUF + dst;
       *reinterpret_cast<u32x2*>(d) = hh;
       *reinterpret_cast<u32x2*>(d + PL) = mm;
       *reinterpret_cast<u32x2*>(d + 2 * PL) = ll;
@@ -136,7 +177,14 @@
       for (int r = 0; r < 16; ++r) acc[a][b][r] = 0.f;
 
   bf16x8 fb0[NS][NB], fb1[NS][NB];
-  load_a(0);
+  if constexpr (UP) {
+#pragma unroll
+    for (int i = 0; i < 4; ++i) issue_up(i, 0);
+#pragma unroll
+    for (int i = 0; i < 4; ++i) fold_up(i);
+  } else {
+    load_a(0);
+  }
   load_b(0, fb0);
   for (int chunk = 0; chunk < nchunks; ++chunk) {
     const int buf = chunk & 1;
@@ -158,7 +206,12 @@
 #if BGS_P3_ABL & 2
       if (t == 0 && chunk == 0) load_a(chunk + 1);
 #else
-      if (t == 0) load_a(chunk + 1);
+      if constexpr (UP) {
+        if (t % 4 == 0 && t >= 4) fold_up(t / 4 - 1);
+        if (t % 4 == 0 && t < 16) issue_up(t / 4, chunk + 1);
+      } else {
+        if (t == 0) load_a(chunk + 1);
+      }
 #endif
       __builtin_amdgcn_sched_barrier(0);
       const bf16x8 (&fbu)[NS][NB] = (t & 1) ? fb1 : fb0;
@@ -288,10 +341,11 @@
       __builtin_amdgcn_make_buffer_rsrc(p.y, 0, (int)((size_t)p.M * p.Cout * 4), 0x00020000);
   const __amdgpu_buffer_rsrc_t mk_rsrc = __builtin_amdgcn_make_buffer_rsrc(
       const_cast<float*>(p.mask ? p.mask : p.x), 0, p.mask ? (int)((size_t)p.M * p.Cout * 4) : 0, 0x00020000);
+  const bool masked = !UP && p.mask;
 #pragma unroll
   for (int a = 0; a < 2; ++a) {
     f32x4 mk[EP];
-    if (p.mask) {
+    if (masked) {
 #pragma unroll
       for (int ps = 0; ps < EP; ++ps) {
         const int m = a * 32 + er0 + ps * RPP;
@@ -319,7 +373,7 @@
 #pragma unroll
         for (int t = 0; t < 4; ++t) v[t] = fmaxf(v[t], 0.f);
       }
-      if (p.mask) {
+      if (masked) {
 #pragma unroll
         for (int t = 0; t < 4; ++t) v[t] = mk[ps][t] > 0.f ? v[t] : 0.f;
       }
@@ -603,6 +657,46 @@
   return hipGetLastError() == hipSuccess ? BGS_OK : BGS_ERR_LAUNCH;
 }
 
+extern "C" int bgs_conv3x3_planes_up_eligible(int N, int H, int W, int Cin, int Cout) {
+  if (N <= 0 || H <= 0 || W <= 0 || (H & 1) || (W & 1) || Cout != 256 || Cin <= 0 || (Cin & 31)) return 0;
+  if (!bgs_internal_halo_hooks_default()) return 0;
+  return planes3_rule(N, H, W, Cout) != 0 ? 1 : 0;
+}
+
+extern "C" int bgs_conv3x3_planes_up_nhwc_f32_bfx(const float* x, const float* up, const void* wsplit,
+                                                  const float* bias, float* y, int N, int H, int W, int Cin,
+                                                  int Cout, int relu, bgs_stream_t stream) {
+  if (N <= 0 || H <= 0 || W <= 0 || Cin <= 0 || Cout <= 0) return BGS_ERR_INVALID_ARG;
+  if (!x || !up || !wsplit || !y) return BGS_ERR_INVALID_ARG;
+  if (Cout != 256 || (Cin & 31) || (H & 1) || (W & 1)) return BGS_ERR_UNSUPPORTED;
+  if (((uintptr_t)x | (uintptr_t)up | (uintptr_t)wsplit | (uintptr_t)bias | (uintptr_t)y) & 15) return BGS_ERR_UNSUPPORTED;
+  const long long M = (long long)N * H * W, lim = kOob;
+  const int KC = 9 * (Cin / 16);
+  if (M * Cin * 4 >= lim || M * Cout * 4 >= lim || (long long)3 * KC * Cout * 32 >= lim) return BGS_ERR_UNSUPPORTED;
+  Planes3UpArgs a;
+  Planes3Args& g = a.g;
+  ConvArgs& p = g.c;
+  p = ConvArgs();
+  p.x = x; p.w = nullptr; p.bias = bias; p.res = nullptr; p.mask = nullptr; p.y = y;
+  p.N = N; p.H = H; p.W = W; p.Cin = Cin; p.Cout = Cout; p.R = 3; p.S = 3; p.stride = 1; p.pad = 1;
+  p.Ho = H; p.Wo = W; p.M = (int)M; p.K = 9 * Cin; p.relu = relu; p.res_mode = 0;
+  p.partial = nullptr; p.kt_per_split = 0;
+  g.ws = reinterpret_cast<const __bf16*>(wsplit);
+  g.KC = KC;
+  g.tiles_y = (H + 7) / 8;
+  g.tiles_x = (W + 7) / 8;
+  p.tiles_m = N * g.tiles_y * g.tiles_x;
+  p.tiles_n = 1;
+  p.chunk = (p.tiles_m + 7) / 8;
+  a.up = up;
+  hipLaunchKernelGGL((conv3x3_planes_bfx_kernel<2, false, true>), dim3((unsigned)(8 * p.chunk)), dim3(kThreads), 0,
+                     (hipStream_t)stream, a);
+  g_planes3_last = 2;
+  bgs_internal_census_bump(BGS_CENSUS_PLANES_3X3);
+  bgs_internal_census_bump(BGS_CENSUS_PLANES_3X3_UP);
+  return hipGetLastError() == hipSuccess ? BGS_OK : BGS_ERR_LAUNCH;
+}
+
 int bgs_internal_conv3x3s2_planes(const bgs_conv::ConvArgs& pc, const void* wsplit, int KC, hipStream_t st) {
   int mode = g_planes3_mode;
   if (mode < 0) {
diff --git a/balancedgroupsoftmax_amd/functional.py b/balancedgroupsoftmax_amd/functional.py
--- a/balancedgroupsoftmax_amd/functional.py
+++ b/balancedgroupsoftmax_amd/functional.py
@@ -928,7 +928,8 @@
 
 CENSUS = dict(bf16_ring8=0, grouped_lds=1, halo_bfx4=2, dma_ring64=3, gs_head_fused=4, conv1x1_bres=5,
               wgrad_bfx=6, roi_bwd_gather=7, bf16s=8, grouped_bf16s=9, bfx_wide=10, gs_scale_grad=11, halo_wide=12, stem_fused=13, fused_c3=14,
-              planes_3x3=15, planes_1x1=16, planes_3x3_head=17, fused_c3_next=18, fused_c3_shortcut=19)
+              planes_3x3=15, planes_1x1=16, planes_3x3_head=17, fused_c3_next=18, fused_c3_shortcut=19,
+              planes_3x3_up=20, fused_c3_lat=21)
 
 
 def launch_census(reset=False):
@@ -990,8 +991,8 @@
 
 
 def _c3_tail(x, w2_krsc, bias2, w3_krsc, bias3, residual=None, relu3=True, out=None, w1n_krsc=None, bias1n=None,
-             x0=None, w_sc_krsc=None, bias_sc=None):
-    _require_cuda(x, w2_krsc, bias2, w3_krsc, bias3, residual, w1n_krsc, bias1n, x0, w_sc_krsc, bias_sc)
+             x0=None, w_sc_krsc=None, bias_sc=None, wl_krsc=None, bias_l=None):
+    _require_cuda(x, w2_krsc, bias2, w3_krsc, bias3, residual, w1n_krsc, bias1n, x0, w_sc_krsc, bias_sc, wl_krsc, bias_l)
     lib = capi.load()
     assert x.dtype == torch.float32 and x.is_contiguous() and x.dim() == 4
     N, H, W, Cmid = x.shape
@@ -1009,7 +1010,16 @@
         h = torch.empty((N, H, W, Cnext), dtype=torch.float32, device=x.device)
         w1s = bfx_split_weights(w1n_krsc.view(Cnext, Cout3), cache=True)
     relu3 = int(bool(relu3))
-    if x0 is not None:
+    lat = None
+    if wl_krsc is not None:
+        Clat = wl_krsc.shape[0]
+        assert x0 is None and Cnext and tuple(wl_krsc.shape) == (Clat, 1, 1, Cout3) and wl_krsc.is_contiguous()
+        lat = torch.empty((N, H, W, Clat), dtype=torch.float32, device=x.device)
+        wls = bfx_split_weights(wl_krsc.view(Clat, Cout3), cache=True)
+        name = 'bgs_conv3x3_c3_next_lat_fused_nhwc_f32_bfx'
+        tensors = (x, w2s, bias2, w3s, bias3, residual, y, w1s, bias1n, h, wls, bias_l, lat)
+        ints = (N, H, W, Cmid, Cout3, relu3, Cnext, Clat)
+    elif x0 is not None:
         Cin0 = x0.shape[3]
         assert residual is None
         assert tuple(x0.shape) == (N, H, W, Cin0) and x0.is_contiguous() and x0.dtype == torch.float32
@@ -1028,7 +1038,7 @@
         ints = (N, H, W, Cmid, Cout3, relu3)
     rc = getattr(lib, name)(*[capi.ptr(t) for t in tensors], *ints, capi.current_stream(x.device))
     capi.check(name, rc)
-    return y, h
+    return y, h, lat
 
 
 def conv3x3_c3_fused_nhwc(x, w2_krsc, bias2, w3_krsc, bias3, residual=None, relu3=True, out=None):
@@ -1051,7 +1061,54 @@
 
 
 def conv3x3_c3_next_fused_nhwc(x, w2_krsc, bias2, w3_krsc, bias3, w1n_krsc, bias1n, residual=None, relu3=True):
-    return _c3_tail(x, w2_krsc, bias2, w3_krsc, bias3, residual, relu3, w1n_krsc=w1n_krsc, bias1n=bias1n)
+    return _c3_tail(x, w2_krsc, bias2, w3_krsc, bias3, residual, relu3, w1n_krsc=w1n_krsc, bias1n=bias1n)[:2]
+
+
+def fused_c3_lateral_eligible(x, w2, w3, stride, residual, w1n, b1n, wl, bl=None):
+    if wl is None or wl.dim() != 4 or tuple(wl.shape) != (256, 1, 1, 256) or wl.dtype != torch.float32 \
+            or not wl.is_contiguous() or not wl.is_cuda:
+        return False
+    if torch.is_grad_enabled() and (wl.requires_grad or (bl is not None and bl.requires_grad)):
+        return False
+    if w1n is None or w1n.shape[0] != 128 or not fused_c3_next_eligible(x, w2, w3, stride, residual, w1n, b1n):
+        return False
+    N, H, W, _ = x.shape
+    return bool(capi.load().bgs_conv3x3_c3_next_lat_eligible(N, H, W, 64, 256, 128, 256))
+
+
+def conv3x3_c3_next_lat_fused_nhwc(x, w2_krsc, bias2, w3_krsc, bias3, w1n_krsc, bias1n, wl_krsc, bias_l, residual=None,
+                                   relu3=True):
+    return _c3_tail(x, w2_krsc, bias2, w3_krsc, bias3, residual, relu3, w1n_krsc=w1n_krsc, bias1n=bias1n,
+                    wl_krsc=wl_krsc, bias_l=bias_l)
+
+
+def conv3x3_up_eligible(x, up, w_conv):
+    if _CONV_MATH[0] != 'bf16x6' or not x.is_cuda or x.dtype != torch.float32 or up.dtype != torch.float32:
+        return False
+    if x.dim() != 4 or up.dim() != 4 or w_conv.dim() != 4 or not (x.is_contiguous() and up.is_contiguous()):
+        return False
+    N, H, W, Cin = x.shape
+    if H % 2 or W % 2 or tuple(up.shape) != (N, H // 2, W // 2, Cin) or tuple(w_conv.shape[1:]) != (3, 3, Cin):
+        return False
+    if not _use_halo_bfx(N * H * W, w_conv.shape[0]):
+        return False
+    return bool(capi.load().bgs_conv3x3_planes_up_eligible(N, H, W, Cin, w_conv.shape[0]))
+
+
+def conv3x3_up_nhwc(x, up, w_krsc, bias=None, relu=False):
+    _require_cuda(x, up, w_krsc, bias)
+    lib = capi.load()
+    assert x.dtype == torch.float32 and up.dtype == torch.float32 and x.is_contiguous() and up.is_contiguous()
+    N, H, W, Cin = x.shape
+    Cout = w_krsc.shape[0]
+    assert tuple(up.shape) == (N, H // 2, W // 2, Cin) and H % 2 == 0 and W % 2 == 0, (x.shape, up.shape)
+    assert tuple(w_krsc.shape) == (Cout, 3, 3, Cin) and w_krsc.is_contiguous()
+    ws = bfx_split_weights(w_krsc.view(Cout, 9 * Cin), cache=True)
+    out = torch.empty((N, H, W, Cout), dtype=torch.float32, device=x.device)
+    rc = lib.bgs_conv3x3_planes_up_nhwc_f32_bfx(capi.ptr(x), capi.ptr(up), capi.ptr(ws), capi.ptr(bias), capi.ptr(out),
+                                                N, H, W, Cin, Cout, int(bool(relu)), capi.current_stream(x.device))
+    capi.check('bgs_conv3x3_planes_up_nhwc_f32_bfx', rc)
+    return out
 
 
 def fused_c3_shortcut_eligible(x0, h1_shape, w2, w3, stride, w_sc, b_sc=None, stride_sc=1):
@@ -1075,8 +1132,8 @@
 
 def conv3x3_c3_sc_fused_nhwc(x, w2_krsc, bias2, w3_krsc, bias3, x0, w_sc_krsc, bias_sc, w1n_krsc=None, bias1n=None,
                              relu3=True):
-    y, h = _c3_tail(x, w2_krsc, bias2, w3_krsc, bias3, None, relu3, w1n_krsc=w1n_krsc, bias1n=bias1n, x0=x0,
-                    w_sc_krsc=w_sc_krsc, bias_sc=bias_sc)
+    y, h, _ = _c3_tail(x, w2_krsc, bias2, w3_krsc, bias3, None, relu3, w1n_krsc=w1n_krsc, bias1n=bias1n, x0=x0,
+                       w_sc_krsc=w_sc_krsc, bias_sc=bias_sc)
     return y if h is None else (y, h)
 
 
diff --git a/balancedgroupsoftmax_amd/train.py b/balancedgroupsoftmax_amd/train.py
--- a/balancedgroupsoftmax_amd/train.py
+++ b/balancedgroupsoftmax_amd/train.py
@@ -422,6 +422,7 @@
         elif isinstance(obj, (tuple, list)):
             for o in obj:
                 TrunkPipeline._record(o, stream)
+            TrunkPipeline._record(getattr(obj, 'raw_lat0', None), stream)
 
     def _launch(self, j, inp, producer):
         from . import functional as BF
diff --git a/include/bgs.h b/include/bgs.h
--- a/include/bgs.h
+++ b/include/bgs.h
@@ -161,6 +161,17 @@
                                          const void* hsplit, const float* hbias, float* y, int N, int H,
                                          int W, int Cin, int Cout, int relu, int Chead, bgs_stream_t stream);
 int bgs_conv3x3_planes_head_eligible(int N, int H, int W, int Cin, int Cout, int Chead);
+int bgs_conv3x3_c3_next_lat_fused_nhwc_f32_bfx(const float* x, const void* w2split, const float* bias2,
+                                               const void* w3split, const float* bias3, const float* residual,
+                                               float* y, const void* w1n_split, const float* bias1n, float* h,
+                                               const void* wl_split, const float* bias_l, float* lat, int N, int H,
+                                               int W, int Cmid, int Cout3, int relu3, int Cnext, int Clat,
+                                               bgs_stream_t stream);
+int bgs_conv3x3_c3_next_lat_eligible(int N, int H, int W, int Cmid, int Cout3, int Cnext, int Clat);
+int bgs_conv3x3_planes_up_nhwc_f32_bfx(const float* x, const float* up, const void* wsplit, const float* bias,
+                                       float* y, int N, int H, int W, int Cin, int Cout, int relu,
+                                       bgs_stream_t stream);
+int bgs_conv3x3_planes_up_eligible(int N, int H, int W, int Cin, int Cout);
 
 
 int bgs_grouped_conv3x3_nhwc_f32(const float* x, const float* w, const float* bias, float* y,
diff --git a/include/bgs_tuning.h b/include/bgs_tuning.h
--- a/include/bgs_tuning.h
+++ b/include/bgs_tuning.h
@@ -31,7 +31,9 @@
 #define BGS_CENSUS_PLANES_3X3_HEAD 17
 #define BGS_CENSUS_FUSED_C3_NEXT 18
 #define BGS_CENSUS_FUSED_C3_SHORTCUT 19
-#define BGS_CENSUS_FAMILIES 20
+#define BGS_CENSUS_PLANES_3X3_UP 20
+#define BGS_CENSUS_FUSED_C3_LAT 21
+#define BGS_CENSUS_FAMILIES 22
 int bgs_launch_census(int family, int reset);
 
 void bgs_gs_head_debug_timestamps(unsigned long long* buf);
```
